# timweiland/DiffEqGMRFs.jl

Hardware: AMD Instinct MI355X
Metric: GMRF posterior solves/sec (mean+samples), 256^2 Darcy (higher is better)
Workload: dtype f64; 1 GPU; darcy256: n=65536, 64 blocks x 1024, nnz=1624084; 256 independent posterior(s) per GPU and step (4 stream(s) x batch 64), each factor + mean + 64 samples; mode=problems, samples_per_problem_per_rank=64, l_blocks_kept=False

## Files before the change

### diffeqgmrfs.jl_amd/_cabi.py

```python
from __future__ import annotations

import ctypes as C
import os
from typing import Optional

_HERE = os.path.dirname(os.path.abspath(__file__))
LIB_PATH = os.environ.get("GMRF_HIP_LIBRARY") or os.path.join(_HERE, "csrc", "libgmrf_hip.so")

GMRF_OK = 0
ERR_NOT_SPD, ERR_BAD_SHAPE, ERR_BAND, ERR_HIP, ERR_NO_FACTOR, ERR_NO_DEVICE, ERR_ALLOC, ERR_RCCL = -1, -2, -3, -4, -5, -6, -7, -8
SOLVE_FULL, SOLVE_FORWARD, SOLVE_BACKWARD = 0, 1, 2
VAR_EXACT, VAR_RBMC, VAR_MC = 0, 1, 2
BLOCK_L, BLOCK_C, BLOCK_LINV = 0, 1, 2
ORDER_REFERENCE, ORDER_TWISTED = 0, 1

EXPORTS = [
    "gmrf_bt_create", "gmrf_bt_destroy", "gmrf_last_error", "gmrf_version",
    "gmrf_bt_factor_csc", "gmrf_bt_factor_blocks", "gmrf_bt_refactor_values",
    "gmrf_bt_solve", "gmrf_bt_sample", "gmrf_bt_posterior", "gmrf_bt_normals", "gmrf_bt_marginal_var",
    "gmrf_bt_var_accumulate", "gmrf_bt_logdet", "gmrf_bt_get_block", "gmrf_bt_factor_buffer",
    "gmrf_bt_adopt_shape", "gmrf_bt_adopt_commit", "gmrf_bt_adopt_layout", "gmrf_bt_get_layout", "gmrf_bt_block_range",
    "gmrf_bt_set_keep_l", "gmrf_bt_storage_bytes", "gmrf_bt_set_storage", "gmrf_bt_factor_begin_csc",
    "gmrf_bt_factor_step_async", "gmrf_bt_factor_end", "gmrf_bt_stats",
    "gmrf_bt_set_profiling", "gmrf_bt_set_eager", "gmrf_bt_synchronize", "gmrf_bt_set_batch", "gmrf_bt_select_problem",
    "gmrf_bt_marginal_var_batch", "gmrf_bt_selinv", "gmrf_bt_trace_inv", "gmrf_bt_set_order", "gmrf_bt_get_order", "gmrf_bt_half_stats", "gmrf_bt_export_size", "gmrf_bt_export_factor", "gmrf_bt_import_factor",
    "gmrf_comm_unique_id", "gmrf_comm_create", "gmrf_comm_destroy", "gmrf_comm_bcast_host", "gmrf_comm_allreduce_sum",
    "gmrf_bt_bcast_blocks_async", "gmrf_bt_allgather_blocks_async", "gmrf_comm_wait", "gmrf_comm_bytes", "gmrf_streams_create", "gmrf_streams_destroy",
    "gmrf_bt_packed_size", "gmrf_bt_pack_blocks_async", "gmrf_bt_unpack_blocks_async",
    "gmrf_csr_create", "gmrf_csr_destroy", "gmrf_spmm", "gmrf_spmm_rows", "gmrf_spmm_async", "gmrf_spmm_rows_async",
    "gmrf_darcy_p1_create", "gmrf_darcy_p2_create", "gmrf_darcy_p1_destroy", "gmrf_darcy_p1_pattern", "gmrf_darcy_p1_assemble",
    "gmrf_burgers_p1_create", "gmrf_burgers_p2_create", "gmrf_burgers_p1_destroy", "gmrf_burgers_p1_pattern", "gmrf_burgers_p1_tangent",
    "gmrf_shallow_water_p1_create", "gmrf_shallow_water_p1_destroy", "gmrf_shallow_water_p1_pattern", "gmrf_shallow_water_p1_qpoints",
    "gmrf_shallow_water_p1_assemble", "gmrf_shallow_water_p1_operators",
    "gmrf_assemble_create", "gmrf_assemble_destroy", "gmrf_assemble_pattern", "gmrf_assemble_precision", "gmrf_assemble_rhs",
    "gmrf_test_gemm", "gmrf_test_gemm_rate", "gmrf_test_gemm_shapes", "gmrf_test_potrf_tile", "gmrf_test_potrf_block", "gmrf_test_tile_timing", "gmrf_test_persist_stamps", "gmrf_test_persist_aborts", "gmrf_test_persist_budget", "gmrf_test_clock_probe_start", "gmrf_test_clock_probe_finish",
    "gmrf_test_mfma_f64_rate", "gmrf_test_hbm_rate", "gmrf_test_microbench", "gmrf_test_symbolic_csc",
]


class SparseBlock(C.Structure):
    _fields_ = [("nnz", C.c_int64), ("ptr", C.c_void_p), ("idx", C.c_void_p), ("val", C.c_void_p)]


class Stats(C.Structure):
    _fields_ = [
        ("factor_ms", C.c_double), ("solve_ms", C.c_double), ("sample_ms", C.c_double),
        ("factor_flops", C.c_double), ("sweep_bytes", C.c_double), ("sweep_ms", C.c_double),
        ("n", C.c_int64), ("n_blocks", C.c_int64), ("block_size", C.c_int64),
        ("block_size_padded", C.c_int64), ("factor_bytes", C.c_int64),
        ("kernel_ms", C.c_double * 24), ("kernel_work", C.c_double * 24), ("kernel_launches", C.c_int64 * 24),
        ("sweep_bytes_streamed", C.c_double),
        ("persist_route", C.c_int32), ("persist_aborts", C.c_int32), ("persist_cus", C.c_int32), ("persist_refused", C.c_int32),
        ("sweep_persist", C.c_int32), ("sweep_persist_launches", C.c_int32),
    ]


class GmrfError(RuntimeError):
    def __init__(self, status: int, msg: str, info: int = 0):
        super().__init__(f"libgmrf_hip status {status}: {msg}")
        self.status = status
        self.info = info


class NotPositiveDefinite(GmrfError):
    """Julia's PosDefException(info): `.info` is the failing block (1-based)."""


_lib: Optional[C.CDLL] = None


def load() -> C.CDLL:
    global _lib
    if _lib is not None:
        return _lib
    if not os.path.exists(LIB_PATH):
        raise ImportError(
            f"{LIB_PATH} is missing: build it with `python -c 'import __graft_entry__ as g; g.build()'` "
            "or `make -C diffeqgmrfs.jl_amd/csrc` (the HIP library is the only compute path)")
    try:
        import torch
    except Exception:
        pass
    lib = C.CDLL(LIB_PATH)
    vp, i32, i64, u64, dbl = C.c_void_p, C.c_int32, C.c_int64, C.c_uint64, C.c_double
    P = C.POINTER
    sigs = {
        "gmrf_bt_create": [i32, vp, P(vp)],
        "gmrf_bt_destroy": [vp],
        "gmrf_version": [],
        "gmrf_bt_factor_csc": [vp, i64, i64, vp, vp, vp, i32, P(i32)],
        "gmrf_bt_factor_blocks": [vp, i64, i64, vp, vp, i32, i32, P(i32)],
        "gmrf_bt_refactor_values": [vp, vp, P(i32)],
        "gmrf_bt_solve": [vp, vp, vp, i64, i64, i64, i32],
        "gmrf_bt_sample": [vp, u64, i64, i64, vp, vp, vp, i64],
        "gmrf_bt_posterior": [vp, vp, u64, i64, i64, vp, vp, i64],
        "gmrf_bt_normals": [vp, u64, i64, i64, vp, i64],
        "gmrf_bt_marginal_var": [vp, i32, i64, u64, vp, vp],
        "gmrf_bt_var_accumulate": [vp, i32, i64, i64, u64, vp, vp],
        "gmrf_bt_logdet": [vp, P(dbl)],
        "gmrf_bt_get_block": [vp, i32, i64, vp, i64],
        "gmrf_bt_factor_buffer": [vp, i32, P(vp), P(i64)],
        "gmrf_bt_adopt_shape": [vp, i64, i64],
        "gmrf_bt_storage_bytes": [i64, i64, i64, P(i64), P(i64), P(i64)],
        "gmrf_bt_set_storage": [vp, i64, i64, i64, vp, vp, vp],
        "gmrf_bt_adopt_commit": [vp, i32],
        "gmrf_bt_adopt_layout": [vp, i64, i64, vp, i64],
        "gmrf_bt_get_layout": [vp, vp, i64, P(i64)],
        "gmrf_bt_block_range": [vp, i32, i64, i64, P(i64), P(i64), P(i64)],
        "gmrf_bt_set_keep_l": [vp, i32],
        "gmrf_comm_unique_id": [vp],
        "gmrf_comm_create": [i32, i32, i32, vp, P(vp)],
        "gmrf_comm_destroy": [vp],
        "gmrf_comm_bcast_host": [vp, vp, i64, i32],
        "gmrf_comm_allreduce_sum": [vp, vp, vp, i64],
        "gmrf_bt_bcast_blocks_async": [vp, vp, i32, i64, i64, i32],
        "gmrf_bt_allgather_blocks_async": [vp, vp, vp, i64, i64],
        "gmrf_comm_wait": [vp, vp],
        "gmrf_comm_bytes": [vp, i32, P(dbl)],
        "gmrf_bt_packed_size": [vp, i64, i64, P(i64)],
        "gmrf_bt_pack_blocks_async": [vp, i64, i64, vp],
        "gmrf_bt_unpack_blocks_async": [vp, i64, i64, vp],
        "gmrf_streams_create": [i32, i32, vp, vp],
        "gmrf_streams_destroy": [i32, i32, vp],
        "gmrf_bt_factor_begin_csc": [vp, i64, i64, vp, vp, vp, i32],
        "gmrf_bt_factor_step_async": [vp, i64, i64],
        "gmrf_bt_factor_end": [vp, P(i32)],
        "gmrf_bt_stats": [vp, P(Stats)],
        "gmrf_bt_set_order": [vp, i32, i64],
        "gmrf_bt_get_order": [vp, P(i32), P(i64)],
        "gmrf_bt_half_stats": [vp, i32, P(Stats)],
        "gmrf_bt_set_profiling": [vp, i32],
        "gmrf_bt_set_eager": [vp, i32],
        "gmrf_bt_synchronize": [vp],
        "gmrf_bt_set_batch": [vp, i64],
        "gmrf_bt_select_problem": [vp, i64],
        "gmrf_csr_create": [i32, vp, i64, i64, vp, vp, vp, i32, i32, P(vp)],
        "gmrf_bt_marginal_var_batch": [vp, i32, i64, u64, vp, vp, vp],
        "gmrf_bt_selinv": [vp, vp, vp],
        "gmrf_bt_trace_inv": [vp, vp, vp, i64, vp],
        "gmrf_bt_export_size": [vp, P(i64)],
        "gmrf_bt_export_factor": [vp, vp, i64],
        "gmrf_bt_import_factor": [vp, vp, i64],
        "gmrf_csr_destroy": [vp],
        "gmrf_assemble_create": [i32, vp, i64, vp, vp, i64, vp, vp, i32, P(vp)],
        "gmrf_assemble_destroy": [vp],
        "gmrf_assemble_pattern": [vp, P(i64), P(i64), vp, vp, i32],
        "gmrf_assemble_precision": [vp, vp, vp, dbl, vp],
        "gmrf_assemble_rhs": [vp, vp, vp, vp, vp, dbl, vp],
        "gmrf_darcy_p1_create": [i32, vp, i64, i64, P(vp)],
        "gmrf_darcy_p2_create": [i32, vp, i64, i64, P(vp)],
        "gmrf_darcy_p1_destroy": [vp],
        "gmrf_darcy_p1_pattern": [vp, P(i64), vp, vp, i32],
        "gmrf_darcy_p1_assemble": [vp, vp, i64, dbl, vp, vp],
        "gmrf_burgers_p1_create": [i32, vp, i64, i64, dbl, dbl, P(vp)],
        "gmrf_burgers_p2_create": [i32, vp, i64, i64, dbl, dbl, P(vp)],
        "gmrf_burgers_p1_destroy": [vp],
        "gmrf_burgers_p1_pattern": [vp, P(i64), vp, vp, i32],
        "gmrf_burgers_p1_tangent": [vp, vp, vp, vp],
        "gmrf_shallow_water_p1_create": [i32, vp, i64, i64, P(vp)],
        "gmrf_shallow_water_p1_destroy": [vp],
        "gmrf_shallow_water_p1_pattern": [vp, i32, P(i64), vp, vp, i32],
        "gmrf_shallow_water_p1_qpoints": [vp, vp],
        "gmrf_shallow_water_p1_assemble": [vp, vp, dbl, dbl, dbl, vp, vp, vp, vp],
        "gmrf_shallow_water_p1_operators": [vp, vp, vp, vp, vp, dbl, dbl, dbl, vp, vp, vp, vp],
        "gmrf_spmm": [vp, vp, vp, i64, i64, i64],
        "gmrf_spmm_async": [vp, vp, vp, i64, i64, i64],
        "gmrf_spmm_rows_async": [vp, vp, vp, i64, i64, i64],
        "gmrf_spmm_rows": [vp, vp, vp, i64, i64, i64],
        "gmrf_test_gemm": [i32, i64, i64, i64, i32, i32, i32, i32, dbl, vp, i64, vp, i64, dbl, vp, i64],
        "gmrf_test_gemm_shapes": [vp, P(dbl), i64, P(i64)],
        "gmrf_test_gemm_rate": [i32, i64, i64, i64, i32, i32, i32, i32, i32, i32, P(dbl)],
        "gmrf_test_potrf_tile": [i32, vp, vp, P(i32)],
        "gmrf_test_potrf_block": [i32, i64, vp, vp, P(i32)],
        "gmrf_test_tile_timing": [vp, i32],
        "gmrf_test_persist_stamps": [vp, i32],
        "gmrf_test_persist_aborts": [vp, vp],
        "gmrf_test_persist_budget": [i32, i32, vp, vp],
        "gmrf_test_clock_probe_start": [i32, i32, i32, P(vp)],
        "gmrf_test_clock_probe_finish": [vp, vp, vp],
        "gmrf_test_mfma_f64_rate": [i32, P(dbl)],
        "gmrf_test_hbm_rate": [i32, i64, P(dbl)],
        "gmrf_test_microbench": [i32, vp, i32],
        "gmrf_test_symbolic_csc": [i64, i64, vp, vp, i32, vp],
    }
    for name, args in sigs.items():
        fn = getattr(lib, name)
        fn.argtypes = args
        fn.restype = i32
    lib.gmrf_last_error.argtypes = []
    lib.gmrf_last_error.restype = C.c_char_p
    _lib = lib
    return lib


def check(status: int, info: int = 0):
    if status == GMRF_OK:
        return
    msg = load().gmrf_last_error().decode(errors="replace")
    if status == ERR_NOT_SPD:
        raise NotPositiveDefinite(status, msg, info)
    raise GmrfError(status, msg, info)


def ptr(a) -> C.c_void_p:
    if a is None:
        return C.c_void_p(0)
    if isinstance(a, int):
        return C.c_void_p(a)
    if hasattr(a, "data_ptr"):
        return C.c_void_p(a.data_ptr())
    return C.c_void_p(a.ctypes.data)
```

### diffeqgmrfs.jl_amd/api.py

```python
from __future__ import annotations

import ctypes as C
from typing import List, Optional, Sequence, Tuple

import numpy as np
import scipy.sparse as sp

from . import _cabi
from ._cabi import GmrfError, NotPositiveDefinite


def _is_torch(x) -> bool:
    return hasattr(x, "data_ptr") and hasattr(x, "device")


def _colmajor(b, n: int):
    if _is_torch(b):
        import torch
        if b.dtype != torch.float64:
            raise TypeError("float64 required")
        if b.dim() == 1:
            if b.shape[0] != n:
                raise ValueError("dimension mismatch")
            return b.contiguous(), 1, n, True
# ... 568 lines not shown
        return out

    def logdet(self) -> float:
        v = C.c_double(0.0)
        _cabi.check(self._lib.gmrf_bt_logdet(self._h, C.byref(v)))
        return v.value

    def normals(self, k: int, seed: int = 0x5EED, first_id: int = 0, like=None):
        if self.batch != 1:
            raise ValueError("a batched handle draws (batch, k, n) normals: normals_batch")
        store, view = _alloc_like(like if like is not None else np.empty(0), self.N, k, False)
        _cabi.check(self._lib.gmrf_bt_normals(self._h, seed, first_id, k, _cabi.ptr(store), self.N))
        return view

    def normals_batch(self, k: int, seed: int = 0x5EED, first_id: int = 0):
        out = np.empty((self.batch, k, self.N), dtype=np.float64)
        _cabi.check(self._lib.gmrf_bt_normals(self._h, seed, first_id, k, _cabi.ptr(out), self.N))
        return out

    def sample(self, k: int, mean=None, z=None, seed: int = 0x5EED, first_id: int = 0, like=None):
        ref = like if like is not None else (z if z is not None else (mean if mean is not None else np.empty(0)))
        za = None
        if z is not None:
            za, kz, _, _ = _colmajor(z, self.N)
            k = kz
        if mean is not None and not _is_torch(mean):
            mean = np.ascontiguousarray(mean, dtype=np.float64)
        store, view = _alloc_like(ref if _is_torch(ref) else np.empty(0), self.N, k, False)
        _cabi.check(self._lib.gmrf_bt_sample(self._h, seed, first_id, k, _cabi.ptr(mean), _cabi.ptr(za),
                                             _cabi.ptr(store), self.N))
        return view

    def posterior(self, b, k: int, seed: int = 0x5EED, first_id: int = 0):
        if self.batch != 1:
            raise ValueError("posterior(): one problem per handle (use solve_batch / sample_batch for batches)")
        xa, kb, ld, one_d = _colmajor(b, self.N)
        if kb != 1:
            raise ValueError("posterior(): one right-hand side")
        mstore, mview = _alloc_like(xa, self.N, 1, True)
        sstore, sview = _alloc_like(xa, self.N, k, False)
        _cabi.check(self._lib.gmrf_bt_posterior(self._h, _cabi.ptr(xa), seed, first_id, k, _cabi.ptr(mstore), _cabi.ptr(sstore),
                                                self.N))
        return mview, sview

    def posterior_batch(self, b, k: int, seed: int = 0x5EED, first_id: int = 0):
        import torch
        B, n = self.batch, self.N
        b = b.reshape(B, n).contiguous()
        mean = torch.empty((B, n), dtype=torch.float64, device=b.device)
        out = torch.empty((B, k, n), dtype=torch.float64, device=b.device)
        _cabi.check(self._lib.gmrf_bt_posterior(self._h, _cabi.ptr(b), seed, first_id, k, _cabi.ptr(mean), _cabi.ptr(out), n))
        return mean, out

    def marginal_var(self, method: str = "exact", k: int = 50, seed: int = 0x5EED, Q: Optional[CsrMatrix] = None,
                     q_values=None, out=None):
        m = {"exact": _cabi.VAR_EXACT, "rbmc": _cabi.VAR_RBMC, "mc": _cabi.VAR_MC}[method]
        shape = (self.N,) if self.batch == 1 else (self.batch, self.N)
        if out is None:
            out = np.empty(shape, dtype=np.float64)
        else:
            ok = tuple(out.shape) == shape and (out.is_contiguous() and str(out.dtype) == "torch.float64" if _is_torch(out)
                                                else out.flags.c_contiguous and out.dtype == np.float64)
            if not ok:
                raise ValueError(f"out must be a contiguous float64 array of shape {shape}")
        if self.batch > 1 and m != _cabi.VAR_EXACT:
            qv = None
            if q_values is not None:
                qv = q_values.contiguous() if _is_torch(q_values) else np.ascontiguousarray(q_values, dtype=np.float64)
            _cabi.check(self._lib.gmrf_bt_marginal_var_batch(self._h, m, k, seed, Q._h if Q is not None else None,
                                                             _cabi.ptr(qv) if qv is not None else None, _cabi.ptr(out)))
            return out
        _cabi.check(self._lib.gmrf_bt_marginal_var(self._h, m, k, seed, Q._h if Q is not None else None,
                                                   _cabi.ptr(out)))
        return out

    def selected_inverse(self, S: CsrMatrix, out=None):
        shape = (S.nnz,) if self.batch == 1 else (self.batch, S.nnz)
        given = out is not None
        out = self._out_array(out, shape)
        _cabi.check(self._lib.gmrf_bt_selinv(self._h, S._h, _cabi.ptr(out)))
        if given or self.batch > 1:
            return out
        return sp.csr_matrix((out, S.indices.copy(), S.indptr.copy()), shape=S.shape)

    def trace_inv(self, S: CsrMatrix, dvals):
        nd = 2 if self.batch == 1 else 3
        if dvals.ndim != nd or dvals.shape[-1] != S.nnz or (nd == 3 and dvals.shape[0] != self.batch):
            want = "(m, nnz)" if nd == 2 else "(batch, m, nnz)"
            raise ValueError(f"dvals must be {want} with nnz = {S.nnz}")
        m = int(dvals.shape[-2])
        if _is_torch(dvals):
            import torch
            if dvals.dtype != torch.float64:
                raise TypeError("float64 required")
            dvals = dvals.contiguous()
            out = torch.empty(dvals.shape[:-1], dtype=torch.float64, device=dvals.device)
        else:
            dvals = np.ascontiguousarray(dvals, dtype=np.float64)
            out = np.empty(dvals.shape[:-1], dtype=np.float64)
        _cabi.check(self._lib.gmrf_bt_trace_inv(self._h, S._h, _cabi.ptr(dvals), m, _cabi.ptr(out)))
        return out

    @staticmethod
    def _out_array(out, shape):
        if out is None:
            return np.empty(shape, dtype=np.float64)
# ... 261 lines not shown
```

### diffeqgmrfs.jl_amd/csrc/gemm_f64.hpp

```cpp
#pragma once
#include <hip/hip_runtime.h>
#include <hip/hip_ext.h>
#include <stdint.h>
#include <stdlib.h>
#include <algorithm>
#include <array>
#include <map>
#include <mutex>
#include <vector>

namespace gmrf {

typedef double v4d __attribute__((ext_vector_type(4)));
typedef double v2d __attribute__((ext_vector_type(2)));

enum : int {
    TRI_A_LOWER = 1,
    TRI_A_UPPER = 2,
    TRI_B_LOWER = 4,
    TRI_B_UPPER = 8
};

struct GemmArgs {
    const double* A;
    const double* B;
    double* C;
    int64_t lda, ldb, ldc;
    int64_t strideA, strideB, strideC;
    int64_t pA, pB, pC;
    int nb1;
    int M, N, K;
    int tri;
    int lower_only;
    double alpha, beta;
    const double* D;
    int64_t ldd, pD;
    unsigned long long* stamps;
    const int* kb_m = nullptr;
    const int* kb_n = nullptr;
    const int* ke_n = nullptr;
};

constexpr int GEMM_BM = 64;
constexpr int GEMM_BN = 64;

template <bool ROWS_CONTIG, int BK>
__device__ __forceinline__ void gemm_load_tile(const double* __restrict__ P, int64_t ld, int row0, int k0,
                                               int t, v2d (&rg)[BK / 8]) {
    if (!ROWS_CONTIG) {
        constexpr int TPR = BK / 2, RPP = 256 / TPR;
        const int r = t / TPR, kk = (t % TPR) * 2;
        const double* p = P + (int64_t)(row0 + r) * ld + k0 + kk;
#pragma unroll
        for (int i = 0; i < BK / 8; ++i) rg[i] = *reinterpret_cast<const v2d*>(p + (int64_t)(i * RPP) * ld);
    } else {
        const int kk = t >> 5, r = (t & 31) * 2;
        const double* p = P + (int64_t)(k0 + kk) * ld + row0 + r;
#pragma unroll
        for (int i = 0; i < BK / 8; ++i) rg[i] = *reinterpret_cast<const v2d*>(p + (int64_t)(i * 8) * ld);
    }
}

template <bool ROWS_CONTIG, int BK>
__device__ __forceinline__ void gemm_tile_offsets(int64_t ld, int row0, int t, uint32_t (&off)[BK / 8]) {
    if (!ROWS_CONTIG) {
        constexpr int TPR = BK / 2, RPP = 256 / TPR;
        const int r = t / TPR, kk = (t % TPR) * 2;
#pragma unroll
        for (int i = 0; i < BK / 8; ++i) off[i] = (uint32_t)(((int64_t)(row0 + r + i * RPP) * ld + kk) * 8);
    } else {
        const int kk = t >> 5, r = (t & 31) * 2;
#pragma unroll
        for (int i = 0; i < BK / 8; ++i) off[i] = (uint32_t)(((int64_t)(kk + i * 8) * ld + row0 + r) * 8);
    }
}
template <bool ROWS_CONTIG>
__device__ __forceinline__ const char* gemm_tile_base(const double* P, int64_t ld, int k0) {
    return reinterpret_cast<const char*>(ROWS_CONTIG ? P + (int64_t)k0 * ld : P + k0);
}
template <int BK>
__device__ __forceinline__ void gemm_load_tile_off(const char* base, uint32_t (&off)[BK / 8], v2d (&rg)[BK / 8]) {
#pragma unroll
    for (int i = 0; i < BK / 8; ++i) {
        asm volatile("" : "+v"(off[i]));
        rg[i] = *reinterpret_cast<const v2d*>(base + off[i]);
    }
}

template <int BK>
__device__ __forceinline__ void gemm_store_tile_natural(double* sm, int t, const v2d (&rg)[BK / 8]) {
    const int kk = t >> 5, r = (t & 31) * 2;
#pragma unroll
    for (int i = 0; i < BK / 8; ++i) *reinterpret_cast<v2d*>(sm + (kk + 8 * i) * 64 + r) = rg[i];
// ... 624 lines not shown
```

### diffeqgmrfs.jl_amd/csrc/gemm_f64_dma.hpp

```cpp
#pragma once
#include "gemm_f64.hpp"

namespace gmrf {

constexpr int DMA_BK = 16;
constexpr int DMA_ROWS_ASCENDING = 1024;
#ifndef GMRF_DMA_READS_FIRST
#define GMRF_DMA_READS_FIRST 0
#endif

template <int BM, int BN>
constexpr size_t gemm_dma_lds_bytes(int stages) { return (size_t)stages * (BM + BN) * DMA_BK * sizeof(double); }

#define GMRF_LDS_PTR(p) ((__attribute__((address_space(3))) void*)(p))
#define GMRF_GLB_PTR(p) ((const __attribute__((address_space(1))) void*)(p))

template <int BM, int BN>
__device__ __forceinline__ void gemm_dma_tile_order(const GemmArgs& g, int& bm, int& bn, int& z) {
    const int nx = g.N / BN, ny = g.M / BM;
    int tpp;
    if (g.lower_only == 1) {
        if (BM >= BN) tpp = (BM / BN) * ny * (ny + 1) / 2;
        else tpp = 0;
    } else tpp = nx * ny;
    const int nz = (int)gridDim.x / tpp;
    const int groups = (nz % 8 == 0) ? 8 : 1;
    const int xg = (int)blockIdx.x % groups, q = (int)blockIdx.x / groups, nzg = nz / groups;
    int zq;
    if (g.lower_only == 1) {
        constexpr int R = BM / BN > 0 ? BM / BN : 1;
        const int tile = q % tpp;
        zq = q / tpp;
        const int tr = (g.tri & DMA_ROWS_ASCENDING) ? tile : tpp - 1 - tile;
        int b = (int)((sqrtf(8.0f * (float)(tr / R) + 1.0f) - 1.0f) * 0.5f);
        while (R * b * (b + 1) / 2 > tr) --b;
        while (R * (b + 1) * (b + 2) / 2 <= tr) ++b;
        bm = b;
        bn = tr - R * b * (b + 1) / 2;
    } else {
        const bool cls_n = (g.tri & (TRI_B_LOWER | TRI_B_UPPER)) || !(g.tri & (TRI_A_LOWER | TRI_A_UPPER));
        const bool desc = cls_n ? ((g.tri & TRI_B_UPPER) != 0 || (g.ke_n && !g.kb_n)) : (g.tri & TRI_A_LOWER) != 0;
        const int ncls = cls_n ? nx : ny, other = cls_n ? ny : nx;
        int c = q / (other * nzg);
        const int rem = q % (other * nzg);
        const int o = rem % other;
        zq = rem / other;
        if (desc) c = ncls - 1 - c;
        bn = cls_n ? c : o;
        bm = cls_n ? o : c;
    }
    z = xg + groups * zq;
}

template <int BM, int BN, bool B_N, int STAGES, bool A_T = false, bool TAIL = false>
__global__ __launch_bounds__(256, (BM + BN > 128) ? 3 : 4) void gemm_f64_dma(GemmArgs g) {
    constexpr int BK = DMA_BK;
    constexpr int MI = BM / 32, NJ = BN / 32;
    constexpr int NA = BM / 32, NB = BN / 32;
    constexpr int A_ST = BM * BK, B_ST = BN * BK, T_ST = TAIL ? BK : 0, ST = A_ST + B_ST + T_ST;
    static_assert(NJ % 2 == 0 || !B_N, "the [k][n] image pairs neighbouring column tiles");
    static_assert(MI % 2 == 0 || !A_T, "the [k][m] image pairs neighbouring row tiles");
    static_assert(!TAIL || (BM == 64 && BN == 64 && B_N && !A_T), "the tail row: 64 x 64 tiles, B stored [k][n]");
    int bm, bn, z;
    gemm_dma_tile_order<BM, BN>(g, bm, bn, z);
    const bool tail = TAIL && bm == g.M / BM - 1;
    const int m0 = bm * BM, n0 = bn * BN;
    if (g.lower_only == 2 && n0 > m0 + BM - 1) return;
    const int zi = z % g.nb1, zp = z / g.nb1;
    const double* __restrict__ A = g.A + (int64_t)zi * g.strideA + (int64_t)zp * g.pA;
    const double* __restrict__ B = g.B + (int64_t)zi * g.strideB + (int64_t)zp * g.pB;
    double* C = g.C + (int64_t)zi * g.strideC + (int64_t)zp * g.pC;
    const double* Dm = g.D ? g.D + (int64_t)zp * g.pD : C;
    const int64_t ldd = g.D ? g.ldd : g.ldc;

    int kb = 0, ke = g.K;
    if (g.tri & TRI_A_LOWER) ke = min(ke, m0 + BM);
    if (g.tri & TRI_A_UPPER) kb = max(kb, m0);
    if (g.tri & TRI_B_LOWER) kb = max(kb, n0);
    if (g.tri & TRI_B_UPPER) ke = min(ke, n0 + BN);
    if (g.kb_m) kb = max(kb, g.kb_m[bm * (BM / 64)]);
    if (g.kb_n) kb = max(kb, g.kb_n[bn * (BN / 64)]);
    if (g.ke_n) ke = min(ke, g.ke_n[bn * (BN / 64) + BN / 64 - 1]);
    const int nkt = (ke > kb) ? (ke - kb) / BK : 0;

    extern __shared__ __attribute__((aligned(16))) double gsm[];
    const int t = threadIdx.x;
    const int lane = t & 63, w = __builtin_amdgcn_readfirstlane(t >> 6);
    const int wm = (w >> 1) * (BM / 2), wn = (w & 1) * (BN / 2);
    const int li = lane & 15, lq = lane >> 4;
    const bool idle = g.lower_only != 0 && ((n0 + wn) / 64 > (m0 + wm + BM / 2 - 1) / 64);

    uint32_t offa[NA], offb[NB];
#pragma unroll
    for (int i = 0; i < NA; ++i) {
        const int q = w + 4 * i;
        if (A_T) {
            constexpr int LPR = BM / 2;
            const int k = q * (64 / LPR) + lane / LPR, col = (lane % LPR) * 2;
            offa[i] = (uint32_t)(((int64_t)k * g.lda + m0 + col) * 8);
        } else {
            const int row = 8 * q + (lane >> 3), ch = (lane & 7) ^ ((row >> 1) & 7);
            offa[i] = (uint32_t)(((int64_t)(m0 + row) * g.lda + 2 * ch) * 8);
        }
    }
#pragma unroll
    for (int i = 0; i < NB; ++i) {
        const int q = w + 4 * i;
        if (B_N) {
            constexpr int LPR = BN / 2;
            const int k = q * (64 / LPR) + lane / LPR, col = (lane % LPR) * 2;
            offb[i] = (uint32_t)(((int64_t)k * g.ldb + n0 + col) * 8);
        } else {
            const int row = 8 * q + (lane >> 3), ch = (lane & 7) ^ ((row >> 1) & 7);
            offb[i] = (uint32_t)(((int64_t)(n0 + row) * g.ldb + 2 * ch) * 8);
        }
    }
    const double* arow = A + (int64_t)g.M * g.lda;
    auto issue = [&](int kt, int stage) {
        const int k0 = kb + kt * BK;
        const char* abase = reinterpret_cast<const char*>(A_T ? A + (int64_t)k0 * g.lda : A + k0);
        const char* bbase = reinterpret_cast<const char*>(B_N ? B + (int64_t)k0 * g.ldb : B + k0);
        double* as = gsm + stage * ST;
        double* bs = as + A_ST;
        if constexpr (TAIL)
            if (tail && w == 0 && lane < 8)
                __builtin_amdgcn_global_load_lds(GMRF_GLB_PTR(arow + k0 + 2 * lane), GMRF_LDS_PTR(bs + B_ST), 16, 0, 0);
#pragma unroll
        for (int i = 0; i < NA; ++i) {
            asm volatile("" : "+v"(offa[i]));
            __builtin_amdgcn_global_load_lds(GMRF_GLB_PTR(abase + offa[i]), GMRF_LDS_PTR(as + (w + 4 * i) * 128), 16, 0, 0);
        }
#pragma unroll
        for (int i = 0; i < NB; ++i) {
            asm volatile("" : "+v"(offb[i]));
            __builtin_amdgcn_global_load_lds(GMRF_GLB_PTR(bbase + offb[i]), GMRF_LDS_PTR(bs + (w + 4 * i) * 128), 16, 0, 0);
        }
    };

    v4d acc[MI][NJ];
#pragma unroll
    for (int i = 0; i < MI; ++i)
#pragma unroll
        for (int j = 0; j < NJ; ++j) acc[i][j] = (v4d){0.0, 0.0, 0.0, 0.0};
    v2d tacc = (v2d){0.0, 0.0};
    const int tkg = w >> 1;

    int fa[MI], fb[NJ];
#pragma unroll
    for (int i = 0; i < MI; ++i) {
        const int row = wm + 16 * i + li;
        fa[i] = A_T ? (2 * lq + (i & 1)) * BM + wm + 32 * (i >> 1) + 2 * li : row * 16 + 2 * (lq ^ ((row >> 1) & 3));
    }
    int sa2[MI], sb2[NJ];
#pragma unroll
    for (int i = 0; i < MI; ++i) { const int row = wm + 16 * i + li; sa2[i] = (!A_T && ((row >> 1) & 4)) ? 8 : 0; }
    if (!B_N) {
#pragma unroll
        for (int j = 0; j < NJ; ++j) {
            const int row = wn + 16 * j + li;
            fb[j] = A_ST + row * 16 + 2 * (lq ^ ((row >> 1) & 3));
            sb2[j] = ((row >> 1) & 4) ? 8 : 0;
        }
    } else {
#pragma unroll
        for (int j = 0; j < NJ; ++j) { fb[j] = A_ST + (2 * lq + (j & 1)) * BN + wn + 32 * (j >> 1) + 2 * li; sb2[j] = 0; }
    }

    constexpr int DEPTH = STAGES - 1;
#pragma unroll
    for (int s = 0; s < DEPTH; ++s)
        if (s < nkt) issue(s, s);
    for (int kt = 0; kt < nkt; ++kt) {
        const int ahead = min(DEPTH - 1, nkt - 1 - kt);
        if (ahead <= 0) asm volatile("s_waitcnt vmcnt(0)" ::: "memory");
        else if (ahead == 1) asm volatile("s_waitcnt vmcnt(%0)" ::"n"(NA + NB) : "memory");
        else asm volatile("s_waitcnt vmcnt(%0)" ::"n"(2 * (NA + NB)) : "memory");
        __builtin_amdgcn_s_barrier();
        __builtin_amdgcn_sched_barrier(0);
        if (!GMRF_DMA_READS_FIRST && kt + DEPTH < nkt) issue(kt + DEPTH, (kt + DEPTH) % STAGES);
        if (!idle) {
            const double* sm = gsm + (kt % STAGES) * ST;
            v2d a[BK / 8][MI], b[BK / 8][NJ];
#pragma unroll
            for (int kg = 0; kg < BK / 8; ++kg) {
#pragma unroll
                for (int i = 0; i < MI; ++i) a[kg][i] = *reinterpret_cast<const v2d*>(sm + fa[i] + (A_T ? kg * 8 * BM : ((kg * 8) ^ sa2[i])));
#pragma unroll
                for (int j = 0; j < NJ; ++j)
                    b[kg][j] = *reinterpret_cast<const v2d*>(sm + fb[j] + (B_N ? kg * 8 * BN : ((kg * 8) ^ sb2[j])));
            }
            v2d ta = (v2d){0.0, 0.0};
            if constexpr (TAIL)
                if (tail) ta = *reinterpret_cast<const v2d*>(sm + A_ST + B_ST + tkg * 8 + 2 * lq);
            __builtin_amdgcn_sched_barrier(0);
            if (GMRF_DMA_READS_FIRST && kt + DEPTH < nkt) issue(kt + DEPTH, (kt + DEPTH) % STAGES);
            __builtin_amdgcn_sched_barrier(0);
#pragma unroll
            for (int kg = 0; kg < BK / 8; ++kg)
#pragma unroll
                for (int p = 0; p < 2; ++p)
#pragma unroll
                    for (int i = 0; i < MI; ++i)
#pragma unroll
                        for (int j = 0; j < NJ; ++j) {
                            double av;
                            if (A_T) av = (i & 1) ? a[kg][2 * (i >> 1) + p].y : a[kg][2 * (i >> 1) + p].x;
                            else av = p ? a[kg][i].y : a[kg][i].x;
                            double bv;
                            if (B_N) bv = (j & 1) ? b[kg][2 * (j >> 1) + p].y : b[kg][2 * (j >> 1) + p].x;
                            else bv = p ? b[kg][j].y : b[kg][j].x;
                            acc[i][j] = __builtin_amdgcn_mfma_f64_16x16x4f64(av, bv, acc[i][j], 0, 0, 0);
                        }
            if constexpr (TAIL) {
                if (tail) {
                    const v2d b0 = tkg ? b[1][0] : b[0][0], b1 = tkg ? b[1][1] : b[0][1];
                    tacc.x = fma(ta.x, b0.x, tacc.x); tacc.x = fma(ta.y, b1.x, tacc.x);
                    tacc.y = fma(ta.x, b0.y, tacc.y); tacc.y = fma(ta.y, b1.y, tacc.y);
                }
            }
            __builtin_amdgcn_sched_barrier(0);
        } else if (GMRF_DMA_READS_FIRST && kt + DEPTH < nkt) issue(kt + DEPTH, (kt + DEPTH) % STAGES);
    }
    if (idle) return;

    const double alpha = g.alpha, beta = g.beta;
    auto orow = [&](int i, int r) -> int64_t {
        return A_T ? m0 + wm + 32 * (i >> 1) + 2 * (lq + 4 * r) + (i & 1) : m0 + wm + i * 16 + lq + 4 * r;
    };
    if (B_N) {
        v2d d[MI][4][NJ / 2 > 0 ? NJ / 2 : 1];
        if (beta != 0.0) {
#pragma unroll
            for (int i = 0; i < MI; ++i)
#pragma unroll
                for (int r = 0; r < 4; ++r)
#pragma unroll
                    for (int jp = 0; jp < NJ / 2; ++jp)
                        d[i][r][jp] = *reinterpret_cast<const v2d*>(Dm + orow(i, r) * ldd + n0 + wn + jp * 32 + 2 * li);
        }
#pragma unroll
        for (int i = 0; i < MI; ++i)
#pragma unroll
            for (int r = 0; r < 4; ++r)
#pragma unroll
                for (int jp = 0; jp < NJ / 2; ++jp) {
                    v2d v = (v2d){alpha * acc[i][2 * jp][r], alpha * acc[i][2 * jp + 1][r]};
                    if (beta != 0.0) { v.x += beta * d[i][r][jp].x; v.y += beta * d[i][r][jp].y; }
                    *reinterpret_cast<v2d*>(C + orow(i, r) * g.ldc + n0 + wn + jp * 32 + 2 * li) = v;
                }
    } else {
        double d[MI][4][NJ];
        if (beta != 0.0) {
#pragma unroll
            for (int i = 0; i < MI; ++i)
#pragma unroll
                for (int r = 0; r < 4; ++r)
#pragma unroll
                    for (int j = 0; j < NJ; ++j)
                        d[i][r][j] = Dm[orow(i, r) * ldd + n0 + wn + j * 16 + li];
        }
#pragma unroll
        for (int i = 0; i < MI; ++i)
#pragma unroll
            for (int r = 0; r < 4; ++r)
#pragma unroll
                for (int j = 0; j < NJ; ++j) {
                    double v = alpha * acc[i][j][r];
                    if (beta != 0.0) v += beta * d[i][r][j];
                    C[orow(i, r) * g.ldc + n0 + wn + j * 16 + li] = v;
                }
    }
    if constexpr (TAIL) {
        if (tail) {
            __syncthreads();
            *reinterpret_cast<v2d*>(gsm + (tkg * 4 + lq) * BN + wn + 2 * li) = tacc;
            __syncthreads();
            if (w == 0) {
                double s = 0.0;
#pragma unroll
                for (int q = 0; q < 8; ++q) s += gsm[q * BN + lane];
                double v = alpha * s;
                if (beta != 0.0) v += beta * Dm[(int64_t)g.M * ldd + n0 + lane];
                C[(int64_t)g.M * g.ldc + n0 + lane] = v;
            }
        }
    }
}

inline int& gemm_dma_policy() {
    static int v = [] { const char* e = getenv("GMRF_GEMM_DMA"); return e ? atoi(e) : 2; }();
    return v;
}
inline int& gemm_dma_force() {
    static int v = 0;
    return v;
}
inline int gemm_dma_stages() {
    static const int v = [] { const char* e = getenv("GMRF_GEMM_DMA_STAGES"); const int s = e ? atoi(e) : 2; return s == 3 ? 3 : 2; }();
    return v;
}

inline int gemm_dma_shape(bool a_t, const GemmArgs& g, int batch) {
    const int policy = gemm_dma_force() ? 2 : gemm_dma_policy();
    if (policy == 0 || g.stamps || (g.tri & ~15) || g.K % DMA_BK || g.M % 64 || g.N % 64) return 0;
    if ((g.lda & 1) || (g.ldb & 1) || ((uintptr_t)g.A & 15) || ((uintptr_t)g.B & 15) || ((g.strideA | g.strideB | g.pA | g.pB) & 1)) return 0;
    if (((uintptr_t)g.C & 15) || (g.ldc & 1) || ((g.strideC | g.pC) & 1)) return 0;
    if (g.D && (((uintptr_t)g.D & 15) || (g.ldd & 1) || (g.pD & 1))) return 0;
    if ((int64_t)g.M * g.ldc * 8 >= ((int64_t)1 << 32) || (g.D && (int64_t)g.M * g.ldd * 8 >= ((int64_t)1 << 32))) return 0;
    if ((int64_t)(a_t ? g.K : g.M) * g.lda * 8 >= ((int64_t)1 << 32) || (int64_t)std::max(g.N, g.K) * g.ldb * 8 >= ((int64_t)1 << 32)) return 0;
    if (a_t) return 1;
    const int force = gemm_dma_force();
    if (force == 2 && g.M % 128 == 0) return 2;
    if (force == 3 && g.N % 128 == 0 && !g.lower_only) return 3;
    if (force) return 1;
    if (policy == 1) return 1;
    const bool plain = !g.lower_only && !g.tri && !g.kb_m && !g.kb_n && !g.ke_n;
    const int64_t t64 = (int64_t)(g.M / 64) * (g.N / 64) * batch;
    if (policy >= 3 || (plain && t64 >= 2048)) {
        if (g.M % 128 == 0) return 2;
        if (g.N % 128 == 0 && !g.lower_only) return 3;
    }
    return 1;
}
inline bool gemm_uses_dma(bool a_t, const GemmArgs& g, int batch) { return gemm_dma_shape(a_t, g, batch) != 0; }

inline hipError_t gemm_dma_init() {
    hipError_t e = hipSuccess;
#define GMRF_DMA_ATTR(BM, BN, BNAT, ST)                                                                          \
    if (e == hipSuccess)                                                                                          \
        e = hipFuncSetAttribute((const void*)gemm_f64_dma<BM, BN, BNAT, ST>, hipFuncAttributeMaxDynamicSharedMemorySize, \
                                (int)gemm_dma_lds_bytes<BM, BN>(ST) + 64 * 1024);
    GMRF_DMA_ATTR(64, 64, false, 2) GMRF_DMA_ATTR(64, 64, true, 2) GMRF_DMA_ATTR(64, 64, false, 3) GMRF_DMA_ATTR(64, 64, true, 3)
    GMRF_DMA_ATTR(128, 64, false, 2) GMRF_DMA_ATTR(128, 64, true, 2) GMRF_DMA_ATTR(128, 64, false, 3) GMRF_DMA_ATTR(128, 64, true, 3)
    GMRF_DMA_ATTR(64, 128, false, 2) GMRF_DMA_ATTR(64, 128, true, 2) GMRF_DMA_ATTR(64, 128, false, 3) GMRF_DMA_ATTR(64, 128, true, 3)
#undef GMRF_DMA_ATTR
    return e;
}

inline bool gemm_tail_ok(bool a_t, bool b_n, const GemmArgs& g, int batch) {
    if (a_t || !b_n || g.lower_only || gemm_uses_ll(g, batch) || gemm_dma_shape(false, g, batch) != 1) return false;
    return (int64_t)(g.M + 1) * g.ldc * 8 < ((int64_t)1 << 32) && (!g.D || (int64_t)(g.M + 1) * g.ldd * 8 < ((int64_t)1 << 32));
}
inline bool gemm_try_dma_tail(hipStream_t st, bool a_t, bool b_n, const GemmArgs& g, int batch, hipEvent_t ev_start, hipEvent_t ev_stop,
                              hipError_t* err) {
    if (!gemm_tail_ok(a_t, b_n, g, batch)) return false;
    GemmArgs gs = g;
    gs.lower_only = 0;
    const dim3 grid((unsigned)((int64_t)(g.N / 64) * (g.M / 64) * batch)), block(256);
    const size_t lds = (size_t)gemm_dma_stages() * (64 + 64 + DMA_BK) * DMA_BK * sizeof(double);
    if (gemm_dma_stages() == 3) {
        if (ev_start) hipExtLaunchKernelGGL((gemm_f64_dma<64, 64, true, 3, false, true>), grid, block, lds, st, ev_start, ev_stop, 0, gs);
        else hipLaunchKernelGGL((gemm_f64_dma<64, 64, true, 3, false, true>), grid, block, lds, st, gs);
    } else {
        if (ev_start) hipExtLaunchKernelGGL((gemm_f64_dma<64, 64, true, 2, false, true>), grid, block, lds, st, ev_start, ev_stop, 0, gs);
        else hipLaunchKernelGGL((gemm_f64_dma<64, 64, true, 2, false, true>), grid, block, lds, st, gs);
    }
    *err = hipGetLastError();
    return true;
}

inline bool gemm_try_dma(hipStream_t st, bool a_t, bool b_n, const GemmArgs& g, int batch, hipEvent_t ev_start, hipEvent_t ev_stop,
                         hipError_t* err) {
    const int shape = gemm_dma_shape(a_t, g, batch);
    if (shape == 0) return false;
    const bool tri_grid = g.lower_only && g.M == g.N;
    GemmArgs gs = g;
    gs.lower_only = tri_grid ? 1 : (g.lower_only ? 2 : 0);
    static const bool asc_off = [] { const char* e = getenv("GMRF_GEMM_G2_ORDER"); return e && atoi(e) == 0; }();
    if (tri_grid && (g.kb_m || g.kb_n) && !asc_off) gs.tri |= DMA_ROWS_ASCENDING;
    const int stages = gemm_dma_stages();
    const dim3 block(256);
#define GMRF_DMA_GO(BM, BN)                                                                                       \
    do {                                                                                                          \
        const int64_t nx = g.N / BN, ny = g.M / BM;                                                               \
        const int64_t tiles = tri_grid ? (int64_t)(BM / BN > 0 ? BM / BN : 1) * ny * (ny + 1) / 2 : nx * ny;      \
        const dim3 grid((unsigned)(tiles * batch));                                                               \
        static const size_t lds_pad = [] { const char* e = getenv("GMRF_GEMM_DMA_LDS_PAD_KB"); return (size_t)(e ? atoi(e) : 0) * 1024; }();    \
        const size_t lds = gemm_dma_lds_bytes<BM, BN>(stages) + lds_pad;                                          \
        if (a_t && BM == 64 && BN == 64) {                                                                        \
            if (b_n) GMRF_DMA_K((gemm_f64_dma<64, 64, true, 2, true>)); else GMRF_DMA_K((gemm_f64_dma<64, 64, false, 2, true>)); \
        } else if (stages == 3) {                                                                                 \
            if (b_n) GMRF_DMA_K((gemm_f64_dma<BM, BN, true, 3>)); else GMRF_DMA_K((gemm_f64_dma<BM, BN, false, 3>)); \
        } else {                                                                                                  \
            if (b_n) GMRF_DMA_K((gemm_f64_dma<BM, BN, true, 2>)); else GMRF_DMA_K((gemm_f64_dma<BM, BN, false, 2>)); \
        }                                                                                                         \
    } while (0)
#define GMRF_DMA_K(KERNEL)                                                                                        \
    do {                                                                                                          \
        if (ev_start) hipExtLaunchKernelGGL(KERNEL, grid, block, lds, st, ev_start, ev_stop, 0, gs);              \
        else hipLaunchKernelGGL(KERNEL, grid, block, lds, st, gs);                                                \
    } while (0)
    if (shape == 2) GMRF_DMA_GO(128, 64);
    else if (shape == 3) GMRF_DMA_GO(64, 128);
    else GMRF_DMA_GO(64, 64);
#undef GMRF_DMA_K
#undef GMRF_DMA_GO
    *err = hipGetLastError();
    return true;
}

}
```

### diffeqgmrfs.jl_amd/csrc/gmrf_hip.hip

```cpp
#include <hip/hip_runtime.h>
#include <dlfcn.h>
#include <stdint.h>
#include <stdlib.h>
#include <string.h>
#include <time.h>

#include <algorithm>
#include <atomic>
#include <iterator>
#include <cmath>
#include <map>
#include <memory>
#include <chrono>
#include <functional>
#include <initializer_list>
#include <mutex>
#include <string>
#include <type_traits>
#include <vector>

#include "../../include/gmrf_hip.h"
#include "assemble.hpp"
#include "fem_assemble.hpp"
#include "gemm_f64.hpp"
// ... 122 lines not shown
    int* d_mend = nullptr;
    int* d_kbx = nullptr;
    int kst_cap = 0;
    double c_streamed = 0.0;
    double g2_tile_k = 0.0;
    bool c_dirty = false;
    int* d_lo_rowptr = nullptr;
    int* d_dg_rowptr = nullptr;
    int* d_bxt_uptr = nullptr; int* d_bxt_ucols = nullptr; uint16_t* d_bxt_lidx = nullptr; int* d_bxt_gtiles = nullptr;
    std::vector<int> bxt_ng;
    int bxt_ecap = 0; int bxt_nrt = 0; bool bxt_plan_ok = false;
    int64_t lo_row_max = 0;
    bool sparse_b = false;
    bool dense_g1 = false;
    double *d_L = nullptr, *d_C = nullptr, *d_Linv = nullptr;
    bool external_storage = false;
    bool keep_l = true;
    bool l_valid = false;
    bool logdet_valid = false;
    std::vector<char> got_block;
    int64_t alloc_rm = 0, alloc_wc = 0;
    bool alloc_keep_l = true;
    double *d_S = nullptr, *d_B = nullptr, *d_T = nullptr, *d_W = nullptr;
    double* d_V = nullptr;
    int64_t v_elems = 0;
    uint64_t layout_gen = 0;
    uint64_t sel_csr = 0, sel_gen = ~0ull;
    int64_t sel_nnz = 0;
    std::vector<int64_t> sel_off, sel_nd;
    int64_t* d_sel_src = nullptr;
    int64_t* d_sel_slot = nullptr;
    int64_t sel_cap = 0;
    double* d_sig = nullptr;
    int64_t sig_elems = 0;
    double* d_dv = nullptr;
    int64_t dv_elems = 0;
    int* d_info = nullptr;
    double* d_logdet = nullptr;
    int64_t alloc_N = 0, alloc_bsp = 0;
    bool factored = false;
    double *d_P = nullptr, *d_Y = nullptr, *d_Tp = nullptr;
    int64_t kp_cap = 0;
    double* d_stage = nullptr;
    int64_t stage_cap = 0;
    double* d_mean = nullptr;
    double* d_acc = nullptr;
    int64_t acc_B = 0;
    bool eager = false;
    bool split_step = false;
    bool sweep_no_gemm = false;
    bool no_fused_posterior = false;
    bool tail_probe = false;
    bool tail_refused = false;
    unsigned long long* dbg_stamps = nullptr;
    bool fork_graph = false;
    bool no_staircase = false;
    bool doubling_x = false;
    int xsplit = 0;
    int adopt_xsplit = 0;
    bool no_xsplit = false;
    bool no_lookahead = false;
    bool no_persist = false;
    bool persist_gave_up = false;
    bool persist_launched = false;
    int persist_cus = 0;
    int info_checked = 0;
    int factor_graph_route = 0;
    int persist_aborts = 0;
    int cu_count = 0;
    unsigned* d_pflags = nullptr;
    int64_t pflags_words = 0;
    bool no_sweep_persist = false;
    bool no_scatter_fold = false;
    bool sweep_persist_planned = false;
    bool sweep_persist_launched = false;
    unsigned* d_sweep_flags = nullptr;
    double* d_Tsw = nullptr;
    int64_t t_elems = 0;
    unsigned* h_sweep_abort = nullptr;
    int sweep_nw = 0;
    double *d_P2 = nullptr, *d_Y2 = nullptr, *d_T2 = nullptr;
    int64_t p2_elems = 0;
    bool sweep_persist_hold = false;
    bool no_persist_panels = false;
    hipStream_t aux = nullptr;
    bool aux_distinct = false;
    hipStream_t gemm_stream = nullptr;
    bool capturing = false;
    std::vector<hipEvent_t> fork_events;
    size_t fork_next = 0;
    hipGraphExec_t factor_graph = nullptr;
    int64_t factor_graph_i0 = -1, factor_graph_i1 = -1;
    std::map<int64_t, hipGraphExec_t> sweep_graphs;
    int profiling = 0;
    std::vector<EvPair> events;
    std::vector<hipEvent_t> ev_pool;
    std::vector<GemmShapeStat> gemm_shapes;
    gmrf_stats stats;
    hipEvent_t ev0 = nullptr, ev1 = nullptr;
    int order = GMRF_ORDER_REFERENCE;
    int64_t meet_req = -1;
    int32_t eager_bits = 0;
    TwistState* tw = nullptr;
    int64_t tw_blk = -1;
    const double* tw_hj = nullptr;
    double* tw_w = nullptr;
// ... 25 lines not shown
    if (!h || h->order != GMRF_ORDER_TWISTED) return GMRF_OK;
    g_last_error = std::string(what) + ": not supported on a handle in the twisted elimination order (gmrf_bt_set_order)";
    return GMRF_ERR_BAD_SHAPE;
}

static void destroy_graphs(gmrf_handle* h) {
    if (h->factor_graph) { (void)hipGraphExecDestroy(h->factor_graph); h->factor_graph = nullptr; }
    for (auto& kv : h->sweep_graphs) (void)hipGraphExecDestroy(kv.second);
    h->sweep_graphs.clear();
}

static hipEvent_t ev_get(gmrf_handle* h) {
    if (!h->ev_pool.empty()) {
        hipEvent_t e = h->ev_pool.back();
        h->ev_pool.pop_back();
        return e;
    }
    hipEvent_t e;
    (void)hipEventCreate(&e);
    return e;
}

struct ProfScope {
    gmrf_handle* h;
    EvPair p;
    bool on;
    ProfScope(gmrf_handle* hh, int kind, double work) : h(hh), on(hh->profiling > 0) {
        if (on) {
            p.kind = kind; p.work = work;
            p.a = ev_get(h); p.b = ev_get(h);
            (void)hipEventRecord(p.a, h->stream);
        }
    }
    ~ProfScope() {
        if (on) {
            (void)hipEventRecord(p.b, h->stream);
            h->events.push_back(p);
        }
    }
};

static void prof_collect(gmrf_handle* h) {
    for (auto& p : h->events) {
        float ms = 0.f;
        (void)hipEventElapsedTime(&ms, p.a, p.b);
        h->stats.kernel_ms[p.kind] += ms; h->stats.kernel_work[p.kind] += p.work; h->stats.kernel_launches[p.kind]++;
        if (p.shape >= 0) { auto& g = h->gemm_shapes[(size_t)p.shape]; g.launches += 1; g.ms += ms; g.work += p.work; }
        h->ev_pool.push_back(p.a);
        h->ev_pool.push_back(p.b);
    }
    h->events.clear();
}

static gmrf_status gemm(gmrf_handle* h, bool a_t, bool b_n, int M, int N, int K, int tri, int lower_only,
                        double alpha, const double* A, int64_t lda, const double* B, int64_t ldb,
                        double beta, double* C, int64_t ldc, int64_t pA, int64_t pB, int64_t pC,
                        int batch = 1, int64_t sA = 0, int64_t sB = 0, int64_t sC = 0, const double* D = nullptr,
                        int64_t ldd = 0, int64_t pD = 0, int pclass = 0, double pwork = -1.0,
                        const int* kb_m = nullptr, const int* kb_n = nullptr, const int* ke_n = nullptr, bool tail = false) {
    GemmArgs g;
    g.kb_m = kb_m; g.kb_n = kb_n; g.ke_n = ke_n;
    g.D = D; g.ldd = ldd; g.pD = pD;
    g.A = A; g.B = B; g.C = C;
    g.lda = lda; g.ldb = ldb; g.ldc = ldc;
    g.strideA = sA; g.strideB = sB; g.strideC = sC;
    g.pA = pA; g.pB = pB; g.pC = pC; g.nb1 = batch;
    g.M = M; g.N = N; g.K = K; g.tri = tri; g.lower_only = lower_only;
    g.alpha = alpha; g.beta = beta; g.stamps = nullptr;
    double flops = 2.0 * M * N * (double)K * batch * (double)h->B;
    if (lower_only) flops *= 0.5 * (1.0 + 64.0 / std::max(M, 64));
    if (tri) flops *= 0.5 * (1.0 + 64.0 / std::max(K, 64));
    if (tail) {
        if (!gemm_tail_ok(a_t, b_n, g, batch * (int)h->B)) {
            h->tail_refused = true;
            return h->tail_probe ? GMRF_OK : bad_shape("internal: a product of the fused sweep does not qualify for the tail-row GEMM");
        }
        if (h->tail_probe) return GMRF_OK;
        flops *= (M + 1.0) / M;
        if (pwork >= 0.0) pwork *= (M + 1.0) / M;
        pclass = b_n ? 15 : 14;
        hipError_t e = hipSuccess;
        if (h->profiling > 0) {
            EvPair p;
            p.kind = pclass; p.work = pwork >= 0.0 ? pwork : flops;
            p.a = ev_get(h); p.b = ev_get(h);
            const int64_t key[8] = {pclass, M + 1, N, K, tri, lower_only, batch * h->B, (kb_m || kb_n || ke_n) ? 1 : 0};
            for (size_t i = 0; i < h->gemm_shapes.size() && p.shape < 0; ++i)
                if (!memcmp(h->gemm_shapes[i].key, key, sizeof(key))) p.shape = (int)i;
            if (p.shape < 0) {
                GemmShapeStat st; memcpy(st.key, key, sizeof(key));
                h->gemm_shapes.push_back(st); p.shape = (int)h->gemm_shapes.size() - 1;
            }
            (void)gemm_try_dma_tail(h->gemm_stream ? h->gemm_stream : h->stream, a_t, b_n, g, batch * (int)h->B, p.a, p.b, &e);
            HIPCHK(e);
            h->events.push_back(p);
            return GMRF_OK;
        }
        (void)gemm_try_dma_tail(h->gemm_stream ? h->gemm_stream : h->stream, a_t, b_n, g, batch * (int)h->B, nullptr, nullptr, &e);
        HIPCHK(e);
        return GMRF_OK;
    }
    if (gemm_uses_big(a_t, g, batch * (int)h->B)) { pclass = b_n ? 7 : 6; pwork = -1.0; }
    else if (pclass == 0) {
        if (gemm_uses_ll(g, batch * (int)h->B)) pclass = 13;
        else if (gemm_uses_dma(a_t, g, batch * (int)h->B)) pclass = a_t ? 18 : (b_n ? 15 : 14);
        else pclass = a_t ? 12 : (b_n ? 11 : 0);
    }
    if (h->profiling > 0) {
        EvPair p;
        p.kind = pclass; p.work = pwork >= 0.0 ? pwork : flops;
        p.a = ev_get(h); p.b = ev_get(h);
        const int64_t key[8] = {pclass, M, N, K, tri, lower_only, batch * h->B, (kb_m || kb_n || ke_n) ? 1 : 0};
        for (size_t i = 0; i < h->gemm_shapes.size() && p.shape < 0; ++i)
            if (!memcmp(h->gemm_shapes[i].key, key, sizeof(key))) p.shape = (int)i;
        if (p.shape < 0) {
            GemmShapeStat st; memcpy(st.key, key, sizeof(key));
            h->gemm_shapes.push_back(st); p.shape = (int)h->gemm_shapes.size() - 1;
        }
        HIPCHK(launch_gemm(h->gemm_stream ? h->gemm_stream : h->stream, a_t, b_n, g, batch * (int)h->B, p.a, p.b));
        h->events.push_back(p);
        return GMRF_OK;
    }
    HIPCHK(launch_gemm(h->gemm_stream ? h->gemm_stream : h->stream, a_t, b_n, g, batch * (int)h->B));
    return GMRF_OK;
}

static void free_dev(void* p) {
    if (p) (void)hipFree(p);
// ... 74 lines not shown
        }
        h->alloc_rm = h->rmax; h->alloc_wc = c_ld(h);
        h->l_valid = false;
        return GMRF_OK;
    }
    free_dev(h->d_L); free_dev(h->d_C); free_dev(h->d_Linv);
    free_dev(h->d_S); free_dev(h->d_B); free_dev(h->d_T); free_dev(h->d_W);
    free_dev(h->d_logdet);
    h->d_L = h->d_C = h->d_Linv = h->d_S = h->d_B = h->d_T = h->d_W = h->d_logdet = nullptr;
    h->l_valid = false;
    const size_t blk = (size_t)blk_elems(h) * sizeof(double) * (size_t)h->B;
    HIPCHK(hipMalloc(&h->d_L, blk * (h->keep_l ? h->N : 1)));
    HIPCHK(hipMalloc(&h->d_Linv, blk * h->N));
    HIPCHK(hipMalloc(&h->d_C, (size_t)stride_pC(h) * sizeof(double) * (size_t)h->B));
    HIPCHK(hipMemsetAsync(h->d_L, 0, blk * (h->keep_l ? h->N : 1), h->stream));
    HIPCHK(hipMemsetAsync(h->d_Linv, 0, blk * h->N, h->stream));
    HIPCHK(hipMemsetAsync(h->d_C, 0, (size_t)stride_pC(h) * sizeof(double) * (size_t)h->B, h->stream));
    h->c_dirty = false;
    GCHK(alloc_work(h));
    h->alloc_rm = h->rmax; h->alloc_wc = c_ld(h); h->alloc_keep_l = h->keep_l;
    return GMRF_OK;
}

static gmrf_status alloc_work(gmrf_handle* h) {
    const size_t blk = (size_t)blk_elems(h) * sizeof(double) * (size_t)h->B;
    HIPCHK(hipMalloc(&h->d_S, blk));
    HIPCHK(hipMalloc(&h->d_B, blk));
    HIPCHK(hipMalloc(&h->d_T, blk));
    HIPCHK(hipMalloc(&h->d_W, blk));
    HIPCHK(hipMalloc(&h->d_logdet, sizeof(double) * h->N * h->B));
    {
        const int64_t words = (int64_t)persist_flag_words((int)(h->bsp / 64)) * h->B;
        if (!h->d_pflags || h->pflags_words < words) {
            free_dev(h->d_pflags); h->d_pflags = nullptr; h->pflags_words = 0;
            HIPCHK(hipMalloc(&h->d_pflags, sizeof(unsigned) * (size_t)words));
            HIPCHK(hipMemsetAsync(h->d_pflags, 0, sizeof(unsigned) * (size_t)words, h->stream));
            HIPCHK(hipStreamSynchronize(h->stream));
            h->pflags_words = words;
        }
    }
    h->alloc_N = h->N; h->alloc_bsp = h->bsp; h->alloc_B = h->B;
    h->stats.factor_bytes = (int64_t)(blk * ((h->keep_l ? 2 : 1) * h->N) + (size_t)stride_pC(h) * sizeof(double) * (size_t)h->B);
    return GMRF_OK;
}

static void release_shape_buffers(gmrf_handle* h) {
    for (auto& kv : h->sweep_graphs) (void)hipGraphExecDestroy(kv.second);
    h->sweep_graphs.clear();
    free_dev(h->d_P); free_dev(h->d_Y); free_dev(h->d_Tp);
    h->d_P = h->d_Y = h->d_Tp = nullptr; h->kp_cap = 0;
    free_dev(h->d_mean); h->d_mean = nullptr;
    free_dev(h->d_acc); h->d_acc = nullptr; h->acc_B = 0;
    free_dev(h->d_stage); h->d_stage = nullptr; h->stage_cap = 0;
}

static gmrf_status set_shape(gmrf_handle* h, int64_t n, int64_t N) {
    if (n <= 0 || N <= 0 || n % N != 0) return bad_shape("n must be a positive multiple of N_blocks");
    const int64_t bs = n / N;
    if (bs > (1 << 20)) return bad_shape("block size too large");
    if (h->n != n || h->N != N) {
        (void)hipStreamSynchronize(h->stream);
        destroy_graphs(h);
        release_shape_buffers(h);
        h->factored = false;
        h->analyzed = false;
    }
    h->n = n; h->N = N; h->bs = bs;
    h->layout_gen++;
    h->bsp = 64 * next_pow2((bs + 63) / 64);
    h->n_pad = h->bsp * N;
    h->stats.n = n; h->stats.n_blocks = N; h->stats.block_size = bs; h->stats.block_size_padded = h->bsp;
    h->stats.factor_flops = ((double)N * bs * bs * bs / 3.0 + (double)(N - 1) * 2.0 * bs * bs * bs) * (double)h->B;
    return GMRF_OK;
}

static gmrf_status ensure_panels(gmrf_handle* h, int64_t kp) {
    if (kp <= h->kp_cap && h->d_P) return GMRF_OK;
    for (auto& kv : h->sweep_graphs) (void)hipGraphExecDestroy(kv.second);
    h->sweep_graphs.clear();
    free_dev(h->d_P); free_dev(h->d_Y); free_dev(h->d_Tp);
    h->d_P = h->d_Y = h->d_Tp = nullptr;
    HIPCHK(hipMalloc(&h->d_P, sizeof(double) * kp * h->n_pad * h->B));
    HIPCHK(hipMalloc(&h->d_Y, sizeof(double) * kp * h->n_pad * h->B));
    HIPCHK(hipMalloc(&h->d_Tp, sizeof(double) * kp * h->bsp * h->B));
    h->kp_cap = kp;
    return GMRF_OK;
}

static gmrf_status ensure_stage(gmrf_handle* h, int64_t elems) {
    if (elems <= h->stage_cap && h->d_stage) return GMRF_OK;
    free_dev(h->d_stage);
    h->d_stage = nullptr;
    HIPCHK(hipMalloc(&h->d_stage, sizeof(double) * elems));
    h->stage_cap = elems;
    return GMRF_OK;
}

struct HostEntry { uint64_t key; int64_t src; };

struct SymbolicPlan {
    std::vector<int64_t> diag_first, diag_count, low_first, low_count;
    std::vector<uint64_t> keys;
    std::vector<int64_t> src;
    int64_t cmin = 0, rmax = 0;
    std::vector<int64_t> first;
    std::vector<int> rowptr;
// ... 364 lines not shown
        }
    }
    h->sweep_persist_planned = ok && want_s > 0 && want >= want_s;
    const int got = ok ? want : 0;
    if (got != h->persist_cus) destroy_graphs(h);
    h->persist_cus = got;
    h->stats.persist_cus = got;
    h->stats.persist_refused = (want > 0 && !ok) ? 1 : 0;
}
static void persist_release(gmrf_handle* h) {
    std::lock_guard<std::mutex> lock(g_persist_mu);
    auto it = g_persist_claims.find(h->device);
    if (it != g_persist_claims.end()) it->second.erase(h);
    h->persist_cus = 0;
    h->stats.persist_cus = 0;
    h->sweep_persist_planned = false;
}

static void persist_give_up(gmrf_handle* h) {
    h->persist_gave_up = true; h->persist_aborts++;
    h->stats.persist_aborts = h->persist_aborts;
    persist_release(h);
    destroy_graphs(h);
}

static bool persist_fits(const gmrf_handle* h, int nt, int j0, int j1, int xrows) {
    if (h->no_persist || h->persist_gave_up || h->persist_cus <= 0) return false;
    return (int64_t)(1 + persist_tiles(nt, j0, j1, xrows)) * h->B <= h->persist_cus;
}

static gmrf_status launch_persist(gmrf_handle* h, double* S, double* L, double* X, int nt, int j0, int j1, int xrows, int blk_id,
                                  double flops) {
    const int words = persist_flag_words(nt);
    if (!h->d_pflags || h->pflags_words < (int64_t)words * h->B) return bad_shape("internal: flag words of the persistent launches not allocated");
    PersistArgs pa;
    pa.S = S; pa.L = L; pa.X = X; pa.ld = h->bsp; pa.nt = nt; pa.j0 = j0; pa.j1 = j1; pa.xrows = xrows;
    pa.tail_panel = (!xrows && j1 < nt) ? 1 : 0;
    pa.info = h->d_info; pa.blk = blk_id;
    pa.pS = h->bsp * h->bsp; pa.pL = stride_pL(h); pa.pX = stride_pX(h); pa.blk_per_problem = (int)h->N;
    pa.flags = h->d_pflags; pa.flag_stride = words;
    pa.abort_word = reinterpret_cast<unsigned*>(h->d_info + 1);
    static const int limit_ms = [] { const char* e = getenv("GMRF_PERSIST_SPIN_MS"); return e ? atoi(e) : -1; }();
    pa.spin_limit = (unsigned)(limit_ms >= 0 ? limit_ms : (h->B > 1 ? 200 : 2000)) * 100000u;
    pa.stamps = h->dbg_stamps;
    h->persist_launched = true;
    h->stats.persist_route = xrows == 1 ? 1 : (xrows == 0 ? 2 : 3);
    ProfScope ps(h, 17, flops);
    hipLaunchKernelGGL(potrf_persist<false>, dim3(1 + persist_tiles(nt, j0, j1, xrows), (unsigned)h->B), dim3(POTRF_PERSIST_THREADS), POTRF_PERSIST_LDS,
                       h->stream, pa);
    HIPCHK(hipGetLastError());
    return GMRF_OK;
}

static gmrf_status potrf_block(gmrf_handle* h, double* S, double* L, double* X, double* T, int blk_id) {
    const int bsp = (int)h->bsp;
    const int64_t ld = bsp;
    const int nt = bsp / 64;
    const int route = potrf_route(h);
    const bool fused = route == ROUTE_FUSED;
    if (h->xsplit > 0 && route != ROUTE_PANELS256) return bad_shape("internal: split inverse planned off the 256-column panel route");
    static const int pw_env = [] { const char* e = getenv("GMRF_PANEL_TILES"); return e ? atoi(e) : 4; }();
    const int pw = (!fused && nt >= 8) ? ((pw_env == 2 || pw_env == 8) ? pw_env : 4) : nt;
    const bool fused_in_panel = route == ROUTE_BIG_ONE;
    const bool overlap = h->capturing && h->fork_graph && nt >= 8;
    if (overlap && !h->aux) HIPCHK(hipStreamCreateWithFlags(&h->aux, hipStreamNonBlocking));
    hipEvent_t ev_fork = nullptr, ev_join = nullptr;
    if (overlap) { GCHK(fork_event(h, &ev_fork)); GCHK(fork_event(h, &ev_join)); }
    if (fused && !h->no_lookahead && !h->doubling_x && !overlap && nt >= 2 && persist_fits(h, nt, 0, nt, 1)) {
        const double t3 = 64.0 * 64.0 * 64.0;
        double fl = t3 / 3.0 * nt;
        for (int j = 0; j + 1 < nt; ++j) {
            const int m = nt - j - 1;
            fl += (double)m * t3 + 2.0 * t3 * (m * (m + 1) / 2) + 2.0 * t3 * (0.5 * (double)(j + 1) * (j + 2) + 0.625 * (j + 1));
        }
        return launch_persist(h, S, L, X, nt, 0, nt, 1, blk_id, fl);
    }
    if (fused && !h->no_lookahead && !h->doubling_x && !overlap && nt >= 2) {
        StepArgs sa;
        sa.S = S; sa.L = L; sa.X = X; sa.ld = ld; sa.nt = nt; sa.cend = nt;
        sa.info = h->d_info; sa.blk = blk_id; sa.dbg = nullptr;
        sa.pS = (int64_t)bsp * bsp; sa.pL = stride_pL(h); sa.pX = stride_pX(h); sa.blk_per_problem = (int)h->N;
        const double t3 = 64.0 * 64.0 * 64.0;
        {
            sa.j = 0; sa.lookahead = 0; sa.xrow = -1;
            ProfScope ps(h, 1, t3 / 3.0);
            hipLaunchKernelGGL(potrf_step<false>, dim3(1, 1), dim3(256), POTRF_TILE_LDS, h->stream, sa);
        }
        for (int j = 0; j + 1 < nt; ++j) {
            const int m = nt - j - 1, ntile_wg = m * (m + 1) / 2;
            sa.j = j; sa.lookahead = 1;
            sa.xrow = (j >= 1) ? j : -1; sa.xrow_first = ntile_wg;
            const int nx_wg = (j >= 1) ? 4 * j : 0;
            const double f_x = (j >= 1) ? 2.0 * t3 * (0.5 * (double)j * (j + 1) + 0.625 * j) : 0.0;
            ProfScope ps(h, 1, t3 / 3.0 + (double)m * t3 + 2.0 * t3 * ntile_wg + f_x);
            hipLaunchKernelGGL(potrf_step<false>, dim3(ntile_wg + nx_wg, 1), dim3(256), POTRF_STEP_LDS, h->stream, sa);
        }
        {
            sa.j = nt - 1; sa.lookahead = 0; sa.xrow = nt - 1; sa.xrow_first = 0;
            ProfScope ps(h, 1, 2.0 * t3 * (0.5 * (double)(nt - 1) * nt + 0.625 * (nt - 1)));
            hipLaunchKernelGGL(potrf_step<false>, dim3(4 * (nt - 1), 1), dim3(256), 64 * 18 * sizeof(double), h->stream, sa);
        }
        HIPCHK(hipGetLastError());
        return GMRF_OK;
    }
    if (route == ROUTE_PANELS256 && !overlap) {
        StepArgs sa;
        sa.S = S; sa.L = L; sa.X = X; sa.ld = ld; sa.nt = nt; sa.cend = nt;
        sa.info = h->d_info; sa.blk = blk_id; sa.dbg = nullptr;
        sa.pS = (int64_t)bsp * bsp; sa.pL = stride_pL(h); sa.pX = stride_pX(h); sa.blk_per_problem = (int)h->N;
        const int64_t pW = (int64_t)bsp * bsp;
        const double t3 = 64.0 * 64.0 * 64.0, nb = (double)h->B;
        auto diag128 = [&](int j) -> gmrf_status {
            sa.j = j;
            ProfScope ps(h, 16, (2.0 * t3 / 3.0 + 4.0 * 2.0 * t3 * 0.625) * nb);
            static const size_t lds_pad = [] { const char* e = getenv("GMRF_DIAG128_LDS_PAD_KB"); return (size_t)(e ? atoi(e) : 0) * 1024; }();
            static const bool fat = [] { const char* e = getenv("GMRF_DIAG128_FAT"); return e && atoi(e) != 0; }();
            if (fat) hipLaunchKernelGGL(potrf_diag128, dim3(1, (unsigned)h->B), dim3(256), POTRF_DIAG128_LDS + lds_pad, h->stream, sa);
            else hipLaunchKernelGGL(potrf_diag128_slim, dim3(1, (unsigned)h->B), dim3(256), POTRF_DIAG128_SLIM_LDS + lds_pad, h->stream, sa);
            HIPCHK(hipGetLastError());
            return GMRF_OK;
        };
        static const bool no_small = [] { const char* e = getenv("GMRF_PERSIST_PANELS"); return e && atoi(e) == 0; }();
        const bool persist_panels = !no_small && !h->no_persist_panels && persist_fits(h, 4, 0, 4, 2);
        for (int j = 0; j < nt; j += 4) {
            const int64_t oa = (int64_t)j * 64, ob = oa + 128, oc = oa + 256;
            if (persist_panels) {
                const double fl = (4.0 * t3 / 3.0 + 2.0 * t3 * (6.0 * 0.625 + 10.0 + 10.0 + 6.0 * 0.625)) * nb;
                GCHK(launch_persist(h, S + oa * ld + oa, L + oa * ld + oa, X + oa * ld + oa, 4, 0, 4, 2, blk_id, fl));
            } else {
                GCHK(diag128(j));
                GCHK(gemm(h, false, false, 128, 128, 128, TRI_B_UPPER, 0, 1.0, S + ob * ld + oa, ld, X + oa * ld + oa, ld, 0.0, L + ob * ld + oa, ld,
                          sa.pS, sa.pX, sa.pL, 1, 0, 0, 0, nullptr, 0, 0, 0, 2.0 * t3 * 3.0 * 2.0 * nb));
                GCHK(gemm(h, false, false, 128, 128, 128, 0, 1, -1.0, L + ob * ld + oa, ld, L + ob * ld + oa, ld, 1.0, S + ob * ld + ob, ld,
                          sa.pL, sa.pL, sa.pS, 1, 0, 0, 0, nullptr, 0, 0, 0, 2.0 * t3 * 2.0 * 3.0 * nb));
                GCHK(diag128(j + 2));
                GCHK(gemm(h, false, true, 128, 128, 128, TRI_B_LOWER, 0, 1.0, L + ob * ld + oa, ld, X + oa * ld + oa, ld, 0.0, T + ob * ld + oa, ld,
                          sa.pL, sa.pX, pW));
                GCHK(gemm(h, false, true, 128, 128, 128, TRI_A_LOWER, 0, -1.0, X + ob * ld + ob, ld, T + ob * ld + oa, ld, 0.0, X + ob * ld + oa, ld,
                          sa.pX, pW, sa.pX));
            }
            const int m3 = nt - j - 4;
            if (m3 <= 0) continue;
            const bool in_slot = (j == 0 && h->xsplit == 256 && !h->keep_l);
            double* Lb = in_slot ? X + oc * ld + oa : L + oc * ld + oa;
            const int64_t pLb = in_slot ? sa.pX : sa.pL;
            GCHK(gemm(h, false, false, 64 * m3, 256, 256, TRI_B_UPPER, 0, 1.0, S + oc * ld + oa, ld, X + oa * ld + oa, ld, 0.0, Lb, ld,
                      sa.pS, sa.pX, pLb, 1, 0, 0, 0, nullptr, 0, 0, 0, 2.0 * t3 * 10.0 * m3 * nb));
            GCHK(gemm(h, false, false, m3 * 64, m3 * 64, 256, 0, 1, -1.0, Lb, ld, Lb, ld, 1.0, S + oc * ld + oc, ld, pLb, pLb, sa.pS,
                      1, 0, 0, 0, nullptr, 0, 0, 0, 2.0 * t3 * 4.0 * (m3 * (m3 + 1) / 2) * nb));
        }
        const int p = h->xsplit;
        GCHK(doubling_levels(h, L, X, T, 256, bsp / 2, -1, p));
        if (p > 0 && !(p == 256 && !h->keep_l)) {
            hipLaunchKernelGGL(copy_rect, dim3((unsigned)((bsp - p) / 4), (unsigned)h->B), dim3(256), 0, h->stream,
                               L + (int64_t)p * ld, ld, sa.pL, X + (int64_t)p * ld, ld, sa.pX, bsp - p, p);
            HIPCHK(hipGetLastError());
        }
        return GMRF_OK;
    }
    if (h->xsplit > 0) return bad_shape("internal: split inverse planned off the 256-column panel route");
    for (int j = 0; j < nt; ++j) {
        StepArgs sa;
        sa.S = S; sa.L = L; sa.X = X; sa.ld = ld; sa.j = j; sa.nt = nt;
        sa.info = h->d_info; sa.blk = blk_id; sa.dbg = h->dbg_stamps;
        sa.pS = (int64_t)bsp * bsp; sa.pL = stride_pL(h); sa.pX = stride_pX(h); sa.blk_per_problem = (int)h->N;
        const int m = nt - j - 1;
        const int cend = std::min(nt, (j / pw + 1) * pw);
        sa.cend = cend;
        int utiles = 0;
        for (int c = j + 1; c < cend; ++c) utiles += nt - c;
        const double rem = 64.0 * m, nb = (double)h->B;
        const double f_tile = 64.0 * 64.0 * 64.0 / 3.0 * nb, f_panel = rem * 64.0 * 64.0 * nb;
        const double f_upd = 2.0 * 64.0 * 64.0 * 64.0 * utiles * nb;
        if (fused_in_panel && !h->no_lookahead && !overlap && j % pw == 0 && cend - j >= 2 && persist_fits(h, nt, j, cend, 0)) {
            const int npc = cend - j;
            double fl = 64.0 * 64.0 * 64.0 / 3.0 * npc;
            for (int jj = j; jj + 1 < cend; ++jj) {
                int ut = 0;
                for (int c = jj + 1; c < cend; ++c) ut += nt - c;
                fl += 64.0 * (nt - jj - 1) * 64.0 * 64.0 + 2.0 * 64.0 * 64.0 * 64.0 * ut;
            }
            fl += 64.0 * (nt - cend) * 64.0 * 64.0;
            GCHK(launch_persist(h, S, L, X, nt, j, cend, 0, blk_id, fl));
            j = cend - 1;
            sa.j = j;
        } else if (fused || m == 0) {
            const bool xrows = fused && !h->doubling_x && !overlap && j >= 2;
            const int ntile_wg = 1 + m * (m + 1) / 2;
            sa.xrow = xrows ? j - 1 : -1; sa.xrow_first = ntile_wg;
            const int nx_wg = xrows ? 4 * (j - 1) : 0;
            const double f_x = xrows ? 2.0 * 64.0 * 64.0 * 64.0 * (0.5 * (double)(j - 1) * j + 0.625 * (j - 1)) : 0.0;
            ProfScope ps(h, 1, f_tile + f_panel + f_upd + f_x);
            hipLaunchKernelGGL(potrf_step<false>, dim3(ntile_wg + nx_wg, (unsigned)h->B), dim3(256),
                               m == 0 ? POTRF_TILE_LDS : POTRF_STEP_LDS, h->stream, sa);
            sa.xrow = -1;
        } else if (fused_in_panel && utiles > 0) {
            ProfScope ps(h, 1, f_tile + f_panel + f_upd);
            hipLaunchKernelGGL(potrf_step<false>, dim3(1 + utiles, 1), dim3(256), POTRF_STEP_LDS, h->stream, sa);
        } else {
            {
                ProfScope ps(h, 1, f_tile);
                hipLaunchKernelGGL(potrf_step<false>, dim3(1, (unsigned)h->B), dim3(256), POTRF_TILE_LDS, h->stream, sa);
// ... 12 lines not shown
            const int j0 = cend - pw, mr = nt - cend;
            const double* Lp = L + (int64_t)cend * 64 * ld + (int64_t)j0 * 64;
            double* Sr = S + (int64_t)cend * 64 * ld + (int64_t)cend * 64;
            GCHK(gemm(h, false, false, mr * 64, mr * 64, pw * 64, 0, 1, -1.0, Lp, ld, Lp, ld, 1.0, Sr, ld, sa.pL, sa.pL,
                      sa.pS, 1, 0, 0, 0, nullptr, 0, 0, 0, 2.0 * 64.0 * 64.0 * (pw * 64.0) * (mr * (mr + 1) / 2) * (double)h->B));
        }
        if (overlap && j + 1 == nt / 2) {
            HIPCHK(hipEventRecord(ev_fork, h->stream));
            HIPCHK(hipStreamWaitEvent(h->aux, ev_fork, 0));
            h->gemm_stream = h->aux;
            gmrf_status st = doubling_levels(h, L, X, T, 64, bsp / 4, 0);
            if (st == GMRF_OK) st = doubling_top(h, L, X, T, true, false);
            h->gemm_stream = nullptr;
            GCHK(st);
        }
    }
    if (fused && !h->doubling_x && !overlap) {
        if (nt >= 2) {
            StepArgs sa;
            sa.S = S; sa.L = L; sa.X = X; sa.ld = ld; sa.j = nt - 1; sa.nt = nt;
            sa.info = h->d_info; sa.blk = blk_id; sa.dbg = nullptr;
            sa.pS = (int64_t)bsp * bsp; sa.pL = stride_pL(h); sa.pX = stride_pX(h); sa.blk_per_problem = (int)h->N;
            sa.cend = nt; sa.xrow = nt - 1; sa.xrow_first = 0;
            ProfScope ps(h, 1, 2.0 * 64.0 * 64.0 * 64.0 * (0.5 * (double)(nt - 1) * nt + 0.625 * (nt - 1)));
            hipLaunchKernelGGL(potrf_step<false>, dim3(4 * (nt - 1), 1), dim3(256), 64 * 18 * sizeof(double), h->stream, sa);
            HIPCHK(hipGetLastError());
        }
        return GMRF_OK;
    }
    if (overlap) {
        GCHK(doubling_levels(h, L, X, T, 64, bsp / 4, 1));
        HIPCHK(hipEventRecord(ev_join, h->aux));
        HIPCHK(hipStreamWaitEvent(h->stream, ev_join, 0));
        GCHK(doubling_top(h, L, X, T, false, true));
    } else {
        GCHK(doubling_levels(h, L, X, T, 64, bsp / 2, -1));
    }
    return GMRF_OK;
}

static gmrf_status factor_blocks_range(gmrf_handle* h, int64_t i0, int64_t i1) {
    const int bsp = (int)h->bsp;
    h->xsplit = planned_xsplit(h);
    const int64_t ld = bsp;
    const size_t blk_bytes = (size_t)bsp * bsp * sizeof(double) * (size_t)h->B;
    const int64_t bstride = (int64_t)bsp * bsp;
    const int64_t pX = stride_pX(h), pC = stride_pC(h);
    const int64_t ldc = c_ld(h), cstride = c_blk(h);
    const unsigned nb = (unsigned)h->B;
    for (int64_t i = i0; i < i1; ++i) {
        double* L = l_block(h, i);
        double* X = h->d_Linv + i * bstride;
        const int rm_s = (i > 0) ? (int)h->rmax : 0;
        static const bool no_tiles_z = [] { const char* e = getenv("GMRF_BXT_TILES"); return e && atoi(e) == 0; }();
        const bool scatter_in_bxt = i > 0 && nb == 1 && h->sparse_b && !h->dense_g1 && h->bxt_plan_ok && !no_tiles_z && h->bxt_nrt == (int)h->rmax / 64
                                    && h->d_dg_rowptr && h->bsp == h->bs && !h->no_scatter_fold;
        const bool zero_in_bxt = scatter_in_bxt || (i > 0 && h->sparse_b && !h->dense_g1 && h->bxt_plan_ok && !no_tiles_z && h->bxt_nrt == (int)h->rmax / 64
                                                    && ((int64_t)(bsp - rm_s) * bsp) % 2 == 0);
        if (rm_s < bsp && !zero_in_bxt) {
            const int64_t cnt = (int64_t)(bsp - rm_s) * bsp;
            hipLaunchKernelGGL(zero_rows, dim3((unsigned)((cnt / 2 + 255) / 256), nb), dim3(256), 0, h->stream,
                               h->d_S + (int64_t)rm_s * ld, cnt, bstride);
            HIPCHK(hipGetLastError());
        }
        if (i > 0) {
            double* C = h->d_C + (i - 1) * cstride;
            const double* Xp = h->d_Linv + (i - 1) * bstride;
            const bool sparse_g1 = h->sparse_b && !h->dense_g1;
            if (!sparse_g1) {
                HIPCHK(hipMemsetAsync(h->d_B, 0, blk_bytes, h->stream));
                if (h->low_count[i] > 0) {
                    hipLaunchKernelGGL(scatter_block, dim3((unsigned)((h->low_count[i] + 255) / 256), nb), dim3(256), 0,
                                       h->stream, h->d_keys, h->d_vals, h->low_first[i], h->low_count[i], h->d_B, ld,
                                       h->n_entries, bstride, 0);
                    HIPCHK(hipGetLastError());
                }
            }
            const int cm = (int)h->cmin, rm = (int)h->rmax;
            const int W = bsp - cm;
            if (sparse_g1) {
                BxtArgs ba;
                ba.rowptr = h->d_lo_rowptr + i * (h->bsp + 1); ba.keys = h->d_keys;
                ba.vals = h->d_vals; ba.n_entries = h->n_entries;
                ba.X = Xp; ba.C = C; ba.ld = ld; ba.ldc = ldc; ba.pX = pX; ba.pC = pC; ba.cm = cm; ba.rm = rm;
                ba.kst = h->d_kst;
                const int rch = (rm + 255) / 256;
                ba.cw = ((int64_t)(W / 64) * rch * nb >= 512) ? 64 : (((int64_t)(W / 32) * rch * nb >= 512) ? 32 : 16);
                ba.bsp = bsp;
                const dim3 grid((unsigned)((W / ba.cw) * rch * (int)nb));
                ProfScope ps(h, 10, 8.0 * (h->c_streamed + 0.5 * (double)W * W) * (double)h->B);
                static const bool no_tiles = [] { const char* e = getenv("GMRF_BXT_TILES"); return e && atoi(e) == 0; }();
                if (h->bxt_plan_ok && !no_tiles && h->bxt_nrt == rm / 64) {
                    BxtTileArgs ta;
                    ta.rowptr = ba.rowptr; ta.lidx = h->d_bxt_lidx; ta.vals = h->d_vals; ta.n_entries = h->n_entries;
                    ta.uptr = h->d_bxt_uptr + i * (h->bxt_nrt + 1); ta.ucols = h->d_bxt_ucols;
                    ta.gtiles = h->d_bxt_gtiles + i * h->bxt_nrt * 3; ta.ng = h->bxt_ng[(size_t)i];
                    ta.X = Xp; ta.C = C; ta.ld = ld; ta.ldc = ldc; ta.pX = pX; ta.pC = pC; ta.kst = h->d_kst;
                    ta.cm = cm; ta.rm = rm; ta.bsp = bsp; ta.ecap = h->bxt_ecap;
                    static const bool live_skip = [] { const char* e = getenv("GMRF_BXT_LIVE"); return e && atoi(e) != 0; }();
                    ta.skip_dead = live_skip ? 1 : 0;
                    const int chunks = W / 16, ng = ta.ng;
                    static const int nch_env = [] { const char* e = getenv("GMRF_BXT_NCH"); return e ? atoi(e) : 0; }();
                    {
                        const int64_t slots = 3 * (int64_t)std::max(h->cu_count, 1);
                        int best = 1; int64_t best_cost = INT64_MAX;
                        for (int c : {1, 2, 3, 4, 6, 8, 12, 16, 24, 48}) {
                            if (c > chunks) break;
                            const int64_t wgs = (int64_t)((chunks + c - 1) / c) * ng * nb;
                            const int64_t cost = ((wgs + slots - 1) / slots) * (c + 2);
                            if (cost < best_cost || (cost == best_cost && c < best)) { best = c; best_cost = cost; }
                        }
                        ta.nch = nch_env > 0 ? std::min(nch_env, chunks) : best;
                    }
                    const int ncg = (chunks + ta.nch - 1) / ta.nch;
                    ta.nprob = (int)nb;
                    ta.zdst = nullptr; ta.zcount = 0; ta.zpdst = 0; ta.zwgs = 0;
                    ta.srowptr = nullptr; ta.skeys = nullptr; ta.svals = nullptr;
                    if (scatter_in_bxt) {
                        ta.zdst = h->d_S; ta.zcount = (int64_t)bsp * bsp; ta.zpdst = bstride; ta.zwgs = 64;
                        ta.srowptr = h->d_dg_rowptr + i * (h->bsp + 1); ta.skeys = h->d_keys; ta.svals = h->d_vals;
                    } else if (zero_in_bxt && rm_s < bsp) {
                        ta.zdst = h->d_S + (int64_t)rm_s * ld; ta.zcount = (int64_t)(bsp - rm_s) * bsp; ta.zpdst = bstride;
                        ta.zwgs = (int)std::min<int64_t>(32, std::max<int64_t>(1, ta.zcount / 16384));
                    }
                    hipLaunchKernelGGL(spmm_bxt_tiles, dim3((unsigned)((ncg * ng + ta.zwgs) * (int)nb)), dim3(256), bxt_tile_lds_bytes(h->bxt_ecap),
                                       h->stream, ta);
                }
                else if (h->lo_row_max <= 8) hipLaunchKernelGGL(spmm_bxt<8>, grid, dim3(256), 0, h->stream, ba);
                else if (h->lo_row_max <= 16) hipLaunchKernelGGL(spmm_bxt<16>, grid, dim3(256), 0, h->stream, ba);
                else hipLaunchKernelGGL(spmm_bxt<32>, grid, dim3(256), 0, h->stream, ba);
                HIPCHK(hipGetLastError());
            } else {
                GCHK(gemm(h, false, false, rm, W, W, TRI_B_UPPER, 0, 1.0, h->d_B + cm, ld,
                          Xp + (int64_t)cm * ld + cm, ld, 0.0, C, ldc, bstride, pX, pC, 1, 0, 0, 0, nullptr, 0, 0, 0, -1.0,
                          h->d_kst, nullptr, nullptr));
            }
            GCHK(gemm(h, false, false, rm, rm, W, 0, 1, -1.0, C, ldc, C, ldc, scatter_in_bxt ? 1.0 : 0.0, h->d_S, ld, pC, pC,
                      bstride, 1, 0, 0, 0, nullptr, 0, 0, 0, 2.0 * 64.0 * 64.0 * h->g2_tile_k * (double)h->B,
                      h->d_kst, h->d_kst, nullptr));
        }
        if (h->diag_count[i] > 0 && !scatter_in_bxt) {
            hipLaunchKernelGGL(scatter_block, dim3((unsigned)((h->diag_count[i] + 255) / 256), nb), dim3(256), 0,
                               h->stream, h->d_keys, h->d_vals, h->diag_first[i], h->diag_count[i], h->d_S, ld,
                               h->n_entries, bstride, 1);
            HIPCHK(hipGetLastError());
        }
        if (i == h->tw_blk && h->tw_hj)
            GCHK(gemm(h, false, false, bsp, bsp, bsp, 0, 1, -1.0, h->tw_hj, ld, h->tw_hj, ld, 1.0, h->d_S, ld, 0, 0, 0));
        if (h->bsp > h->bs) {
            hipLaunchKernelGGL(pad_identity, dim3((unsigned)((h->bsp - h->bs + 255) / 256), nb), dim3(256), 0,
                               h->stream, h->d_S, ld, (int)h->bs, bsp, bstride);
            HIPCHK(hipGetLastError());
        }
        GCHK(potrf_block(h, h->d_S, L, X, h->d_T, (int)(i + 1)));
        if (i == h->tw_blk && h->tw_w)
            GCHK(gemm(h, false, true, bsp, bsp, bsp, 0, 0, 1.0, X, ld, h->tw_hj, ld, 0.0, h->tw_w, ld, 0, 0, 0));
        if (!h->keep_l) {
            hipLaunchKernelGGL(logdet_blocks, dim3(1, nb), dim3(256), 0, h->stream, L, bstride, ld, (int)h->bs,
                               h->d_logdet + i, stride_pL(h), h->N);
            HIPCHK(hipGetLastError());
        }
    }
    return GMRF_OK;
}

static gmrf_status ensure_full_inverse(gmrf_handle* h) {
    if (h->xsplit <= 0) return GMRF_OK;
    const int bsp = (int)h->bsp, p = h->xsplit, q = bsp - p;
    const int64_t ld = bsp, bstride = (int64_t)bsp * bsp, pX = stride_pX(h), pW = bstride;
    for (int64_t i = 0; i < h->N; ++i) {
        double* X = h->d_Linv + i * bstride;
        double* T = h->d_T + (int64_t)p * ld;
        GCHK(gemm(h, false, true, q, p, p, TRI_B_LOWER, 0, 1.0, X + (int64_t)p * ld, ld, X, ld, 0.0, T, ld, pX, pX, pW));
        GCHK(gemm(h, false, true, q, p, q, TRI_A_LOWER, 0, -1.0, X + (int64_t)p * ld + p, ld, T, ld, 0.0, X + (int64_t)p * ld, ld, pX, pW, pX));
    }
    h->xsplit = 0;
    return GMRF_OK;
}

static std::mutex g_capture_mu;

static gmrf_status run_factor(gmrf_handle* h, int64_t i0, int64_t i1) {
    if (h->eager || h->profiling) { h->stats.persist_route = 0; return factor_blocks_range(h, i0, i1); }
    if (!h->factor_graph || h->factor_graph_i0 != i0 || h->factor_graph_i1 != i1) {
        std::lock_guard<std::mutex> capture_lock(g_capture_mu);
        if (h->factor_graph) { (void)hipGraphExecDestroy(h->factor_graph); h->factor_graph = nullptr; }
        hipGraph_t graph = nullptr;
        HIPCHK(hipStreamBeginCapture(h->stream, hipStreamCaptureModeThreadLocal));
        h->capturing = true; h->fork_next = 0;
        h->stats.persist_route = 0;
        gmrf_status s = factor_blocks_range(h, i0, i1);
        h->capturing = false;
        h->factor_graph_route = h->stats.persist_route;
        hipError_t e = hipStreamEndCapture(h->stream, &graph);
        if (s != GMRF_OK) { if (graph) (void)hipGraphDestroy(graph); return s; }
        HIPCHK(e);
        HIPCHK(hipGraphInstantiate(&h->factor_graph, graph, nullptr, nullptr, 0));
        (void)hipGraphDestroy(graph);
        h->factor_graph_i0 = i0; h->factor_graph_i1 = i1;
    }
    h->xsplit = planned_xsplit(h);
    h->stats.persist_route = h->factor_graph_route;
    if (h->factor_graph_route) h->persist_launched = true;
    HIPCHK(hipGraphLaunch(h->factor_graph, h->stream));
    return GMRF_OK;
}

static gmrf_status persist_check_range(gmrf_handle* h, int64_t i0, int64_t i1, int* hinfo_out) {
    int hinfo2[2] = {0, 0};
    HIPCHK(hipMemcpyAsync(hinfo2, h->d_info, 2 * sizeof(int), hipMemcpyDeviceToHost, h->stream));
    HIPCHK(hipStreamSynchronize(h->stream));
    h->persist_launched = false;
    if (hinfo2[1] != 0) {
        persist_give_up(h);
        const int restore[4] = {h->info_checked, 0, 0, 0};
        HIPCHK(hipMemcpyAsync(h->d_info, restore, 4 * sizeof(int), hipMemcpyHostToDevice, h->stream));
        if (h->d_pflags) HIPCHK(hipMemsetAsync(h->d_pflags, 0, sizeof(unsigned) * (size_t)h->pflags_words, h->stream));
        h->stats.persist_route = 0;
        GCHK(factor_blocks_range(h, i0, i1));
        HIPCHK(hipMemcpyAsync(hinfo2, h->d_info, 2 * sizeof(int), hipMemcpyDeviceToHost, h->stream));
        HIPCHK(hipStreamSynchronize(h->stream));
        h->persist_launched = false;
    }
    h->info_checked = hinfo2[0];
    if (hinfo_out) *hinfo_out = hinfo2[0];
    return GMRF_OK;
}

static gmrf_status factor_finish(gmrf_handle* h, int32_t* info) {
    int hinfo = 0;
    GCHK(persist_check_range(h, 0, h->N, &hinfo));
    if (info) *info = hinfo;
    if (hinfo != 0) {
        h->factored = false;
        g_last_error = "matrix is not positive definite; failed block " + std::to_string((hinfo - 1) % h->N + 1) +
                       " of problem " + std::to_string((hinfo - 1) / h->N);
        if (info) *info = (hinfo - 1) % (int)h->N + 1;
        return GMRF_ERR_NOT_SPD;
    }
    h->factored = true;
    h->l_valid = h->keep_l;
    h->logdet_valid = !h->keep_l;
    return GMRF_OK;
}

static gmrf_status numeric_factor(gmrf_handle* h, const double* nzval, int32_t* info) {
    if (!h->analyzed) { g_last_error = "no sparsity pattern analysed"; return GMRF_ERR_NO_FACTOR; }
    GCHK(alloc_factor(h));
    if (h->c_dirty) {
        HIPCHK(hipMemsetAsync(h->d_C, 0, sizeof(double) * stride_pC(h) * h->B, h->stream));
        h->c_dirty = false;
    }
    persist_plan(h);
    HIPCHK(hipEventRecord(h->ev0, h->stream));
    GCHK(load_values(h, nzval));
    HIPCHK(hipMemsetAsync(h->d_info, 0, 4 * sizeof(int), h->stream));
    h->info_checked = 0; h->persist_launched = false;
    GCHK(run_factor(h, 0, h->N));
    HIPCHK(hipEventRecord(h->ev1, h->stream));
    gmrf_status s = factor_finish(h, info);
    float ms = 0.f;
    (void)hipEventElapsedTime(&ms, h->ev0, h->ev1);
    h->stats.factor_ms = ms;
    if (h->profiling) prof_collect(h);
    return s;
}

__global__ void gmrf_spin_kernel(unsigned long long ticks) {
    const unsigned long long t0 = __builtin_amdgcn_s_memrealtime();
    while (__builtin_amdgcn_s_memrealtime() - t0 < ticks) {}
}

static double spin_pair_ms(hipStream_t a, hipStream_t b, unsigned long long ticks) {
    (void)hipDeviceSynchronize();
    const auto t0 = std::chrono::steady_clock::now();
    hipLaunchKernelGGL(gmrf_spin_kernel, dim3(1), dim3(64), 0, a, ticks);
    if (b) hipLaunchKernelGGL(gmrf_spin_kernel, dim3(1), dim3(64), 0, b, ticks);
    (void)hipStreamSynchronize(a);
    if (b) (void)hipStreamSynchronize(b);
    return std::chrono::duration<double, std::milli>(std::chrono::steady_clock::now() - t0).count();
}

gmrf_status gmrf_streams_create(int32_t device, int32_t n, void** streams, int32_t* n_distinct) {
    if (n <= 0 || n > 32 || !streams) return bad_shape("gmrf_streams_create: 1 <= n <= 32 streams");
    HIPCHK(hipSetDevice(device));
    const int ncand = std::min(3 * n + 4, 48);
    std::vector<hipStream_t> cand((size_t)ncand, nullptr);
    for (int i = 0; i < ncand; ++i) {
        if (hipStreamCreateWithFlags(&cand[(size_t)i], hipStreamNonBlocking) != hipSuccess) {
            for (int j = 0; j < i; ++j) (void)hipStreamDestroy(cand[(size_t)j]);
            g_last_error = "hipStreamCreateWithFlags failed"; return GMRF_ERR_HIP;
        }
        hipLaunchKernelGGL(gmrf_spin_kernel, dim3(1), dim3(64), 0, cand[(size_t)i], 1ull);
    }
    HIPCHK(hipDeviceSynchronize());
    const unsigned long long ticks = 100000ull;
    double one = 1e30;
    for (int r = 0; r < 3; ++r) one = std::min(one, spin_pair_ms(cand[0], nullptr, ticks));
    std::vector<int> chosen;
    for (int i = 0; i < ncand && (int)chosen.size() < n; ++i) {
        bool ok = true;
        for (int c : chosen) {
            const double t = std::min(spin_pair_ms(cand[(size_t)c], cand[(size_t)i], ticks), spin_pair_ms(cand[(size_t)c], cand[(size_t)i], ticks));
            if (t > 1.5 * one) { ok = false; break; }
        }
        if (ok) chosen.push_back(i);
    }
    const int nd = (int)chosen.size();
    std::vector<char> used((size_t)ncand, 0);
    for (int c : chosen) used[(size_t)c] = 1;
    for (int i = 0; i < ncand && (int)chosen.size() < n; ++i)
        if (!used[(size_t)i]) { chosen.push_back(i); used[(size_t)i] = 1; }
    for (int k = 0; k < n; ++k) streams[k] = (void*)cand[(size_t)chosen[(size_t)k]];
// ... 299 lines not shown
int32_t gmrf_version(void) { return 100; }
const char* gmrf_last_error(void) { return g_last_error.c_str(); }

gmrf_status gmrf_bt_create(int32_t device, void* stream, gmrf_handle** out) {
    if (!out) return bad_shape("null out pointer");
    int count = 0;
    if (hipGetDeviceCount(&count) != hipSuccess || count <= 0 || device < 0 || device >= count) {
        (void)hipGetLastError();
        g_last_error = "no HIP device visible (libgmrf_hip needs an MI355X / gfx950 GPU)";
        return GMRF_ERR_NO_DEVICE;
    }
    HIPCHK(hipSetDevice(device));
    gmrf_handle* h = new gmrf_handle();
    memset(&h->stats, 0, sizeof(h->stats));
    h->device = device;
    if (stream) { h->stream = (hipStream_t)stream; h->own_stream = false; }
    else { HIPCHK(hipStreamCreateWithFlags(&h->stream, hipStreamNonBlocking)); h->own_stream = true; }
    HIPCHK(hipMalloc(&h->d_info, 4 * sizeof(int)));
    HIPCHK(hipMemsetAsync(h->d_info, 0, 4 * sizeof(int), h->stream));
    HIPCHK(hipStreamSynchronize(h->stream));
    HIPCHK(hipEventCreate(&h->ev0));
    HIPCHK(hipEventCreate(&h->ev1));
    HIPCHK(hipFuncSetAttribute((const void*)potrf_step<false>, hipFuncAttributeMaxDynamicSharedMemorySize, (int)POTRF_STEP_LDS));
    HIPCHK(hipFuncSetAttribute((const void*)potrf_diag128, hipFuncAttributeMaxDynamicSharedMemorySize, 160 * 1024));
    HIPCHK(hipFuncSetAttribute((const void*)potrf_persist<false>, hipFuncAttributeMaxDynamicSharedMemorySize, (int)POTRF_PERSIST_LDS));
    HIPCHK(hipDeviceGetAttribute(&h->cu_count, hipDeviceAttributeMultiprocessorCount, device));
    { const char* e = getenv("GMRF_PERSIST"); if (e && atoi(e) == 0) h->no_persist = true; }
    { const char* e = getenv("GMRF_SWEEP_PERSIST"); if (e && atoi(e) == 0) h->no_sweep_persist = true; }
    HIPCHK(hipFuncSetAttribute((const void*)potrf_diag128_slim, hipFuncAttributeMaxDynamicSharedMemorySize, 160 * 1024));
    HIPCHK(gemm_init());
    HIPCHK(gemm_dma_init());
    *out = h;
    return GMRF_OK;
}

gmrf_status gmrf_bt_destroy(gmrf_handle* h) {
    if (!h) return GMRF_OK;
    (void)hipSetDevice(h->device);
    tw_free(h);
    (void)hipStreamSynchronize(h->stream);
    persist_release(h);
    destroy_graphs(h);
    free_dev(h->d_keys); free_dev(h->d_vals); free_dev(h->d_src); free_dev(h->d_nz_stage);
    free_dev(h->d_lo_rowptr); free_dev(h->d_dg_rowptr); free_dev(h->d_kst); free_dev(h->d_mend);
    free_dev(h->d_bxt_uptr); free_dev(h->d_bxt_ucols); free_dev(h->d_bxt_lidx); free_dev(h->d_bxt_gtiles);
    if (!h->external_storage) { free_dev(h->d_L); free_dev(h->d_C); free_dev(h->d_Linv); }
    else if (!h->keep_l) free_dev(h->d_L);
    free_dev(h->d_S); free_dev(h->d_B); free_dev(h->d_T); free_dev(h->d_W);
    free_dev(h->d_sweep_flags); free_dev(h->d_Tsw); free_dev(h->d_P2); free_dev(h->d_Y2); free_dev(h->d_T2);
    if (h->h_sweep_abort) { (void)hipHostFree(h->h_sweep_abort); h->h_sweep_abort = nullptr; }
    free_dev(h->d_info); free_dev(h->d_logdet); free_dev(h->d_pflags); free_dev(h->d_kbx); free_dev(h->d_V);
    free_dev(h->d_P); free_dev(h->d_Y); free_dev(h->d_Tp);
    free_dev(h->d_stage); free_dev(h->d_mean); free_dev(h->d_acc);
    free_dev(h->d_sel_src); free_dev(h->d_sel_slot); free_dev(h->d_sig); free_dev(h->d_dv);
    for (auto e : h->ev_pool) (void)hipEventDestroy(e);
    if (h->ev0) (void)hipEventDestroy(h->ev0);
    if (h->ev1) (void)hipEventDestroy(h->ev1);
    for (auto e : h->fork_events) (void)hipEventDestroy(e);
    if (h->aux) (void)hipStreamDestroy(h->aux);
    if (h->own_stream) (void)hipStreamDestroy(h->stream);
    delete h;
    return GMRF_OK;
}

gmrf_status gmrf_bt_set_batch(gmrf_handle* h, int64_t batch) {
    if (!h || batch < 1 || batch > 4096) return bad_shape("batch must be in [1, 4096]");
    if (batch != 1) GCHK(tw_refuse(h, "gmrf_bt_set_batch (batch > 1)"));
    if (batch != h->B) {
        HIPCHK(hipSetDevice(h->device));
        HIPCHK(hipStreamSynchronize(h->stream));
        destroy_graphs(h);
        h->B = batch;
        h->sel = 0;
        h->factored = false;
        release_shape_buffers(h);
        if (h->n > 0) (void)set_shape(h, h->n, h->N);
    }
    return GMRF_OK;
}

gmrf_status gmrf_bt_select_problem(gmrf_handle* h, int64_t p) {
    if (!h || p < 0 || p >= h->B) return bad_shape("problem index out of range");
    h->sel = p;
    return GMRF_OK;
}

gmrf_status gmrf_bt_set_profiling(gmrf_handle* h, int32_t level) {
    if (!h) return bad_shape("null handle");
    h->profiling = level;
    if (h->tw)
        for (gmrf_handle* s : {h->tw->top, h->tw->bot}) if (s) GCHK(gmrf_bt_set_profiling(s, level));
    if (level > 0 && h->events.empty()) h->gemm_shapes.clear();
    for (int i = 0; i < GMRF_KERNEL_CLASSES; ++i) { h->stats.kernel_ms[i] = h->stats.kernel_work[i] = 0; h->stats.kernel_launches[i] = 0; }
    return GMRF_OK;
}

gmrf_status gmrf_bt_set_eager(gmrf_handle* h, int32_t eager) {
    if (!h) return bad_shape("null handle");
    if (((eager & 2) != 0) != h->split_step) { destroy_graphs(h); h->split_step = (eager & 2) != 0; }
    if (((eager & 4) != 0) != h->sweep_no_gemm) { destroy_graphs(h); h->sweep_no_gemm = (eager & 4) != 0; }
    if (((eager & 8) != 0) != h->dense_g1) { destroy_graphs(h); h->dense_g1 = (eager & 8) != 0; }
    if (((eager & 16) != 0) != h->fork_graph) { destroy_graphs(h); h->fork_graph = (eager & 16) != 0; }
    h->no_staircase = (eager & 32) != 0;
    if (((eager & 128) != 0) != h->doubling_x) { destroy_graphs(h); h->doubling_x = (eager & 128) != 0; }
    if (((eager & 256) != 0) != h->no_lookahead) { destroy_graphs(h); h->no_lookahead = (eager & 256) != 0; }
    if (((eager & 4096) != 0) != h->no_xsplit) { destroy_graphs(h); h->no_xsplit = (eager & 4096) != 0; }
    if (((eager & 8192) != 0) != h->no_persist) { destroy_graphs(h); h->no_persist = (eager & 8192) != 0; }
    if (((eager & 32768) != 0) != h->no_persist_panels) { destroy_graphs(h); h->no_persist_panels = (eager & 32768) != 0; }
    if (((eager & 65536) != 0) != h->no_sweep_persist) { destroy_graphs(h); h->no_sweep_persist = (eager & 65536) != 0; }
    if (((eager & 131072) != 0) != h->no_scatter_fold) { destroy_graphs(h); h->no_scatter_fold = (eager & 131072) != 0; }
    h->no_fused_posterior = (eager & 262144) != 0;
    h->eager = (eager & 1) != 0;
    h->eager_bits = eager;
    if (h->tw)
        for (gmrf_handle* s : {h->tw->top, h->tw->bot})
            if (s) {
                GCHK(gmrf_bt_set_eager(s, eager));
                if (h->tw->bot) s->no_sweep_persist = true;
            }
    return GMRF_OK;
}

gmrf_status gmrf_bt_synchronize(gmrf_handle* h) {
    if (!h) return bad_shape("null handle");
    HIPCHK(hipStreamSynchronize(h->stream));
    if (tw_on(h)) HIPCHK(hipStreamSynchronize(h->tw->bot->stream));
    return GMRF_OK;
}

gmrf_status gmrf_bt_stats(gmrf_handle* h, gmrf_stats* out) {
    if (!h || !out) return bad_shape("null pointer");
    if (tw_on(h)) {
        const gmrf_stats &a = h->tw->top->stats, &b = h->tw->bot->stats;
        *out = h->stats;
        out->persist_route = a.persist_route;
        out->persist_aborts = a.persist_aborts + b.persist_aborts;
        out->persist_cus = a.persist_cus + b.persist_cus;
        out->persist_refused = a.persist_refused | b.persist_refused;
        out->factor_bytes = a.factor_bytes + b.factor_bytes;
        return GMRF_OK;
    }
    h = tw_route(h);
    *out = h->stats;
    return GMRF_OK;
}

gmrf_status gmrf_bt_factor_csc(gmrf_handle* h, int64_t n, int64_t n_blocks, const int64_t* colptr,
                               const int64_t* rowval, const double* nzval, int32_t index_base,
                               int32_t* info) {
    if (!h) return bad_shape("null handle");
    HIPCHK(hipSetDevice(h->device));
    if (info) *info = 0;
    if (h->order == GMRF_ORDER_TWISTED) {
        GCHK(tw_analyze(h, n, n_blocks, colptr, rowval, index_base));
        return tw_numeric(h, nzval, info);
    }
    GCHK(analyze_csc(h, n, n_blocks, colptr, rowval, index_base));
    return numeric_factor(h, nzval, info);
}

gmrf_status gmrf_bt_factor_begin_csc(gmrf_handle* h, int64_t n, int64_t n_blocks, const int64_t* colptr,
                                     const int64_t* rowval, const double* nzval, int32_t index_base) {
    GCHK(tw_refuse(h, "gmrf_bt_factor_begin_csc"));
    if (!h) return bad_shape("null handle");
    HIPCHK(hipSetDevice(h->device));
    if (colptr) GCHK(analyze_csc(h, n, n_blocks, colptr, rowval, index_base));
    if (!h->analyzed) { g_last_error = "no sparsity pattern analysed"; return GMRF_ERR_NO_FACTOR; }
    GCHK(alloc_factor(h));
    if (h->c_dirty) {
        HIPCHK(hipMemsetAsync(h->d_C, 0, sizeof(double) * stride_pC(h) * h->B, h->stream));
        h->c_dirty = false;
    }
    persist_plan(h);
    GCHK(load_values(h, nzval));
    HIPCHK(hipMemsetAsync(h->d_info, 0, 4 * sizeof(int), h->stream));
    h->info_checked = 0; h->persist_launched = false; h->stats.persist_route = 0;
    h->factored = false;
    return GMRF_OK;
}

gmrf_status gmrf_bt_factor_step_async(gmrf_handle* h, int64_t i0, int64_t i1) {
    GCHK(tw_refuse(h, "gmrf_bt_factor_step_async"));
    if (!h) return bad_shape("null handle");
    if (i0 < 0 || i1 > h->N || i0 > i1) return bad_shape("bad block range");
    HIPCHK(hipSetDevice(h->device));
    GCHK(factor_blocks_range(h, i0, i1));
    if (h->persist_launched) GCHK(persist_check_range(h, i0, i1, nullptr));
    return GMRF_OK;
}

gmrf_status gmrf_bt_factor_end(gmrf_handle* h, int32_t* info) {
    GCHK(tw_refuse(h, "gmrf_bt_factor_end"));
    if (!h) return bad_shape("null handle");
    HIPCHK(hipSetDevice(h->device));
    gmrf_status s = factor_finish(h, info);
    if (h->profiling) prof_collect(h);
    return s;
}

gmrf_status gmrf_bt_refactor_values(gmrf_handle* h, const double* nzval, int32_t* info) {
    if (!h) return bad_shape("null handle");
    HIPCHK(hipSetDevice(h->device));
    if (info) *info = 0;
    if (h->order == GMRF_ORDER_TWISTED) return tw_numeric(h, nzval, info);
    return numeric_factor(h, nzval, info);
}

gmrf_status gmrf_bt_factor_blocks(gmrf_handle* h, int64_t n, int64_t n_blocks, const gmrf_sparse_block* diag,
                                  const gmrf_sparse_block* lower, int32_t index_base,
                                  int32_t compressed_by_column, int32_t* info) {
    GCHK(tw_refuse(h, "gmrf_bt_factor_blocks"));
    if (!h || !diag || (n_blocks > 1 && !lower)) return bad_shape("null pointer");
    HIPCHK(hipSetDevice(h->device));
    if (info) *info = 0;
    GCHK(set_shape(h, n, n_blocks));
    const int64_t bs = h->bs;
    std::vector<std::vector<HostEntry>> dg(n_blocks), lo(n_blocks);
    std::vector<double> vals;
    auto add_block = [&](const gmrf_sparse_block& b, std::vector<HostEntry>& dst, bool lower_tri_only) -> bool {
        for (int64_t o = 0; o < bs; ++o) {
            for (int64_t p = b.ptr[o] - index_base; p < b.ptr[o + 1] - index_base; ++p) {
                const int64_t in = b.idx[p] - index_base;
                if (in < 0 || in >= bs) return false;
                const int64_t r = compressed_by_column ? in : o, c = compressed_by_column ? o : in;
                if (lower_tri_only && r < c) continue;
                dst.push_back({((uint64_t)r << 32) | (uint64_t)c, (int64_t)vals.size()});
                vals.push_back(b.val[p]);
            }
        }
        return true;
// ... 75 lines not shown
    for (int64_t t = 0; t < nrt; ++t) out[3 + t] = h->kst[(size_t)t];
    out[3 + nrt] = h->factored ? h->xsplit : planned_xsplit(h);
    return GMRF_OK;
}

gmrf_status gmrf_bt_adopt_layout(gmrf_handle* h, int64_t n, int64_t n_blocks, const int64_t* layout, int64_t count) {
    GCHK(tw_refuse(h, "gmrf_bt_adopt_layout"));
    if (!h) return bad_shape("null handle");
    HIPCHK(hipSetDevice(h->device));
    GCHK(set_shape(h, n, n_blocks));
    h->analyzed = false;
    if (layout) {
        if (count < 3 || layout[2] < 1 || count < 3 + layout[2] || layout[1] != 64 * layout[2]) return bad_shape("bad layout record");
        std::vector<int64_t> first((size_t)layout[2]);
        for (int64_t t = 0; t < layout[2]; ++t) first[(size_t)t] = layout[0] + layout[3 + t];
        GCHK(set_layout(h, layout[0], layout[1], first));
        h->adopt_xsplit = 0;
        if (count >= 4 + layout[2]) {
            const int64_t xs = layout[3 + layout[2]];
            if (xs < 0 || xs >= h->bsp || xs % 64) return bad_shape("bad layout record (split)");
            h->adopt_xsplit = (int)xs;
        }
    } else {
        GCHK(set_layout_dense(h));
        h->adopt_xsplit = 0;
    }
    GCHK(alloc_factor(h));
    if (h->c_dirty) {
        HIPCHK(hipMemsetAsync(h->d_C, 0, sizeof(double) * stride_pC(h) * h->B, h->stream));
        h->c_dirty = false;
    }
    h->factored = false; h->l_valid = false; h->logdet_valid = false;
    h->got_block.assign((size_t)h->N, 0);
    HIPCHK(hipStreamSynchronize(h->stream));
    return GMRF_OK;
}

gmrf_status gmrf_bt_adopt_shape(gmrf_handle* h, int64_t n, int64_t n_blocks) {
    GCHK(tw_refuse(h, "gmrf_bt_adopt_shape"));
    return gmrf_bt_adopt_layout(h, n, n_blocks, nullptr, 0);
}

gmrf_status gmrf_bt_adopt_commit(gmrf_handle* h, int32_t l_blocks_valid) {
    GCHK(tw_refuse(h, "gmrf_bt_adopt_commit"));
    if (!h || !h->d_Linv) return bad_shape("no factor storage");
    HIPCHK(hipSetDevice(h->device));
    int seen = 0;
    HIPCHK(hipMemcpyAsync(&seen, h->d_info + 2, sizeof(int), hipMemcpyDeviceToHost, h->stream));
    HIPCHK(hipStreamSynchronize(h->stream));
    if (seen != 0) HIPCHK(hipMemsetAsync(h->d_info + 2, 0, sizeof(int), h->stream));
    if (seen < 0) { g_last_error = "the packed ranges of this factor carry different (or no) representation tags"; return GMRF_ERR_BAD_SHAPE; }
    const int xs = seen > 0 ? seen - 1 : h->adopt_xsplit;
    if (xs < 0 || xs >= h->bsp || xs % 64) { g_last_error = "bad representation tag in the packed image"; return GMRF_ERR_BAD_SHAPE; }
    h->factored = true;
    h->xsplit = xs;
    h->l_valid = l_blocks_valid != 0 && h->keep_l;
    bool all = !h->got_block.empty();
    for (char g : h->got_block) all = all && g;
    h->logdet_valid = all;
    h->got_block.assign((size_t)h->N, 0);
    persist_plan(h);
    return GMRF_OK;
}

gmrf_status gmrf_bt_factor_buffer(gmrf_handle* h, int32_t kind, void** dev_ptr, int64_t* bytes) {
    GCHK(tw_refuse(h, "gmrf_bt_factor_buffer"));
    if (!h || !dev_ptr || !bytes) return bad_shape("null pointer");
    if (!h->d_Linv) { g_last_error = "no factor storage"; return GMRF_ERR_NO_FACTOR; }
    const int64_t blk = blk_elems(h) * (int64_t)sizeof(double) * h->B;
    if (kind == GMRF_BLOCK_L) {
        if (!h->keep_l) { g_last_error = "L blocks are not kept (gmrf_bt_set_keep_l)"; return GMRF_ERR_NO_FACTOR; }
        *dev_ptr = h->d_L; *bytes = blk * h->N;
    }
    else if (kind == GMRF_BLOCK_C) { *dev_ptr = h->d_C; *bytes = stride_pC(h) * (int64_t)sizeof(double) * h->B; }
    else if (kind == GMRF_BLOCK_LINV) { *dev_ptr = h->d_Linv; *bytes = blk * h->N; }
    else return bad_shape("bad block kind");
    return GMRF_OK;
}

gmrf_status gmrf_bt_block_range(gmrf_handle* h, int32_t kind, int64_t i0, int64_t i1, int64_t* first_elem,
                                int64_t* n_elems, int64_t* problem_stride) {
    GCHK(tw_refuse(h, "gmrf_bt_block_range"));
    if (!h || !first_elem || !n_elems || !problem_stride) return bad_shape("null pointer");
    if (h->N <= 0 || i0 < 0 || i1 > h->N || i0 > i1) return bad_shape("bad block range");
    if (kind == GMRF_BLOCK_C) {
        const int64_t c0 = std::max<int64_t>(i0 - 1, 0), c1 = std::max<int64_t>(i1 - 1, 0);
        *first_elem = c0 * c_blk(h); *n_elems = (c1 - c0) * c_blk(h); *problem_stride = stride_pC(h);
    } else if (kind == GMRF_BLOCK_LINV || kind == GMRF_BLOCK_L) {
        if (kind == GMRF_BLOCK_L && !h->keep_l) { g_last_error = "L blocks are not kept"; return GMRF_ERR_NO_FACTOR; }
        *first_elem = i0 * blk_elems(h); *n_elems = (i1 - i0) * blk_elems(h);
        *problem_stride = kind == GMRF_BLOCK_L ? stride_pL(h) : stride_pX(h);
    } else return bad_shape("bad block kind");
    return GMRF_OK;
}

static void packed_counts(const gmrf_handle* h, int64_t i0, int64_t i1, int64_t* x_elems, int64_t* c_elems, int64_t* ld_elems,
                          int64_t* c0_out) {
    const int64_t nt = h->bsp / 64, ntri = nt * (nt + 1) / 2;
    const int64_t c0 = std::max<int64_t>(i0 - 1, 0), c1 = std::max<int64_t>(i1 - 1, 0);
    *x_elems = (i1 - i0) * ntri * 4096;
    *c_elems = (c1 - c0) * c_blk(h);
    *ld_elems = 2 + ((i1 - i0) + 1) / 2 * 2;
    if (c0_out) *c0_out = c0;
}

gmrf_status gmrf_bt_packed_size(gmrf_handle* h, int64_t i0, int64_t i1, int64_t* elems_per_problem) {
    GCHK(tw_refuse(h, "gmrf_bt_packed_size"));
// ... 133 lines not shown
    for (int64_t i = 0; i < h->N; ++i) GCHK(gmrf_bt_get_block(h, GMRF_BLOCK_LINV, i, out + i * be, h->bs));
    return GMRF_OK;
}

gmrf_status gmrf_bt_import_factor(gmrf_handle* h, const void* buf, int64_t bytes) {
    GCHK(tw_refuse(h, "gmrf_bt_import_factor"));
    if (!h || !buf) return bad_shape("null pointer");
    if (is_device_ptr(buf)) return bad_shape("import buffer must be host memory");
    if (bytes < 64) return bad_shape("import buffer too small");
    const int64_t* hdr = (const int64_t*)buf;
    if (hdr[0] != EXPORT_MAGIC || hdr[1] != 1 || hdr[5] != 1) return bad_shape("not a factor image");
    const int64_t n = hdr[2], N = hdr[3], bs = hdr[4];
    if (N <= 0 || bs <= 0 || n != N * bs) return bad_shape("bad shape in factor image");
    if (bytes < 64 + (int64_t)sizeof(double) * bs * bs * (3 * N - 1)) return bad_shape("factor image truncated");
    HIPCHK(hipSetDevice(h->device));
    if (!h->keep_l) return bad_shape("import needs the L blocks kept (gmrf_bt_set_keep_l(h, 1))");
    if ((h->n != n || h->N != N) && h->B != 1) return bad_shape("a batched handle imports into an existing shape only");
    const bool relayout = (h->n != n || h->N != N || h->cmin != 0 || h->rmax != 64 * next_pow2((bs + 63) / 64) || !h->d_Linv);
    if (relayout && h->B != 1 && h->factored) return bad_shape("a batched handle imports only into a dense-layout factor");
    GCHK(set_shape(h, n, N));
    h->analyzed = false;
    if (relayout) {
        GCHK(set_layout_dense(h));
        GCHK(alloc_factor(h));
        if (h->c_dirty) {
            HIPCHK(hipMemsetAsync(h->d_C, 0, sizeof(double) * stride_pC(h) * h->B, h->stream));
            h->c_dirty = false;
        }
    } else {
        std::vector<int64_t> z((size_t)(h->bsp / 64), 0);
        bool dense_ks = true;
        for (int v : h->kst) if (v != 0) dense_ks = false;
        if (!dense_ks) GCHK(set_layout(h, 0, h->bsp, z));
        h->c_dirty = false;
    }
    const int64_t bsp = h->bsp, be = bs * bs;
    std::vector<double> tmp((size_t)bsp * bsp);
    auto put = [&](const double* src, double* dst, bool unit_pad) -> gmrf_status {
        std::fill(tmp.begin(), tmp.end(), 0.0);
        for (int64_t r = 0; r < bs; ++r)
            for (int64_t c = 0; c < bs; ++c) tmp[(size_t)r * bsp + c] = src[c * bs + r];
        if (unit_pad)
            for (int64_t r = bs; r < bsp; ++r) tmp[(size_t)r * bsp + r] = 1.0;
        HIPCHK(hipMemcpyAsync(dst, tmp.data(), tmp.size() * sizeof(double), hipMemcpyHostToDevice, h->stream));
        HIPCHK(hipStreamSynchronize(h->stream));
        return GMRF_OK;
    };
    const double* in = (const double*)((const char*)buf + 64);
    for (int64_t i = 0; i < N; ++i) GCHK(put(in + i * be, h->d_L + h->sel * stride_pL(h) + i * blk_elems(h), true));
    in += N * be;
    for (int64_t i = 0; i + 1 < N; ++i) GCHK(put(in + i * be, h->d_C + h->sel * stride_pC(h) + i * c_blk(h), false));
    in += (N - 1) * be;
    for (int64_t i = 0; i < N; ++i) GCHK(put(in + i * be, h->d_Linv + h->sel * stride_pX(h) + i * blk_elems(h), true));
    h->factored = true; h->l_valid = true;
    persist_plan(h);
    h->xsplit = 0;
    return GMRF_OK;
}

struct NcclUid { char b[128]; };
struct RcclApi {
    void* lib = nullptr;
    int (*GetUniqueId)(NcclUid*) = nullptr;
    int (*CommInitRank)(void**, int, NcclUid, int) = nullptr;
    int (*CommDestroy)(void*) = nullptr;
    int (*Broadcast)(const void*, void*, size_t, int, int, void*, hipStream_t) = nullptr;
    int (*AllReduce)(const void*, void*, size_t, int, int, void*, hipStream_t) = nullptr;
    int (*AllGather)(const void*, void*, size_t, int, void*, hipStream_t) = nullptr;
    int (*GroupStart)() = nullptr;
    int (*GroupEnd)() = nullptr;
    const char* (*GetErrorString)(int) = nullptr;
};
static RcclApi g_rccl;
static std::mutex g_rccl_mu;

static gmrf_status rccl_load() {
    std::lock_guard<std::mutex> lock(g_rccl_mu);
    if (g_rccl.lib) return GMRF_OK;
    const char* env = getenv("GMRF_RCCL_PATH");
    const char* names[] = {env, "librccl.so.1", "librccl.so", "/opt/rocm/lib/librccl.so.1", "/opt/rocm/lib/librccl.so"};
    void* lib = nullptr;
    for (int pass = 0; pass < 2 && !lib; ++pass)
        for (const char* nm : names) {
            if (!nm) continue;
            lib = dlopen(nm, RTLD_NOW | RTLD_LOCAL | (pass == 0 ? RTLD_NOLOAD : 0));
            if (lib) break;
        }
    if (!lib) { g_last_error = std::string("librccl not found (set GMRF_RCCL_PATH): ") + (dlerror() ? dlerror() : ""); return GMRF_ERR_RCCL; }
#define GMRF_RCCL_SYM(field, name)                                                           \
    g_rccl.field = reinterpret_cast<decltype(g_rccl.field)>(dlsym(lib, name));               \
    if (!g_rccl.field) { g_last_error = std::string("librccl lacks ") + name; return GMRF_ERR_RCCL; }
    GMRF_RCCL_SYM(GetUniqueId, "ncclGetUniqueId") GMRF_RCCL_SYM(CommInitRank, "ncclCommInitRank")
    GMRF_RCCL_SYM(CommDestroy, "ncclCommDestroy") GMRF_RCCL_SYM(Broadcast, "ncclBroadcast")
    GMRF_RCCL_SYM(AllReduce, "ncclAllReduce") GMRF_RCCL_SYM(AllGather, "ncclAllGather") GMRF_RCCL_SYM(GroupStart, "ncclGroupStart")
    GMRF_RCCL_SYM(GroupEnd, "ncclGroupEnd") GMRF_RCCL_SYM(GetErrorString, "ncclGetErrorString")
#undef GMRF_RCCL_SYM
    g_rccl.lib = lib;
    return GMRF_OK;
}

#define NCCLCHK(expr)                                                                       \
    do {                                                                                    \
        int _r = (expr);                                                                    \
        if (_r != 0) {                                                                      \
            g_last_error = std::string(#expr) + ": " + g_rccl.GetErrorString(_r);           \
            return GMRF_ERR_RCCL;                                                           \
        }                                                                                   \
// ... 309 lines not shown
        free_dev(h->d_P2); free_dev(h->d_Y2); free_dev(h->d_T2);
        h->d_P2 = h->d_Y2 = h->d_T2 = nullptr; h->p2_elems = 0;
        HIPCHK(hipMalloc(&h->d_P2, sizeof(double) * (size_t)elems));
        HIPCHK(hipMalloc(&h->d_Y2, sizeof(double) * (size_t)elems));
        HIPCHK(hipMalloc(&h->d_T2, sizeof(double) * (size_t)elems));
        h->p2_elems = elems;
    }
    GCHK(ensure_aux(h));
    h->fork_next = 0;
    hipEvent_t ev_fork = nullptr, ev_join = nullptr;
    GCHK(fork_event(h, &ev_fork)); GCHK(fork_event(h, &ev_join));
    h->sweep_persist_launched = true;
    h->stats.sweep_persist = 1;
    h->stats.sweep_persist_launches += 3;
    HIPCHK(hipEventRecord(h->ev0, h->stream));
    HIPCHK(hipEventRecord(ev_fork, h->stream));
    HIPCHK(hipStreamWaitEvent(h->aux, ev_fork, 0));
    {
        const int64_t total = (int64_t)kp * h->n_pad;
        hipLaunchKernelGGL(fill_normals_panel, dim3((unsigned)((total + 255) / 256), 1), dim3(256), 0, h->aux, h->d_P2, h->n_pad,
                           (int)h->bs, (int)h->bsp, (int)k, kp, seed, first_id, k, nullptr, (int64_t)0);
        HIPCHK(hipGetLastError());
        GCHK(launch_sweep_persist(h, true, kp, h->d_P2, h->d_Y2, h->aux, h->d_T2));
        HIPCHK(hipEventRecord(ev_join, h->aux));
    }
    GCHK(launch_pack(h, b, h->n, 1, 1));
    GCHK(launch_sweep_persist(h, false, 1, h->d_P, h->d_Y));
    GCHK(launch_sweep_persist(h, true, 1, h->d_Y, h->d_P));
    GCHK(launch_unpack(h, h->d_P, mean, h->n, 1, nullptr));
    HIPCHK(hipStreamWaitEvent(h->stream, ev_join, 0));
    GCHK(launch_unpack(h, h->d_Y2, samples, ld, (int)k, mean));
    HIPCHK(hipEventRecord(h->ev1, h->stream));
    HIPCHK(hipStreamSynchronize(h->stream));
    return GMRF_OK;
}

static bool posterior_fused_ok(gmrf_handle* h, int64_t k, bool dev_all) {
    if (tw_on(h) || h->B <= 1 || !dev_all || h->no_fused_posterior || h->sweep_no_gemm || k <= 0 || k > KP_CHUNK) return false;
    const int kp = pad_k(k);
    if (kp % 64 != 0 || (int64_t)h->B * (h->bsp / 64) * (kp / 64) < 128) return false;
    if ((int64_t)(kp + 1) * h->n_pad * 8 >= ((int64_t)1 << 32)) return false;
    if (ensure_panels(h, kp + 1) != GMRF_OK) return false;
    h->tail_probe = true; h->tail_refused = false;
    const gmrf_status st = sweep_launches(h, true, kp, h->d_P, h->d_Y, true);
    h->tail_probe = false;
    return st == GMRF_OK && !h->tail_refused;
}

static gmrf_status posterior_fused(gmrf_handle* h, const double* b, uint64_t seed, int64_t first_id, int64_t k, double* mean,
                                   double* samples, int64_t ld) {
    const int kp = pad_k(k);
    GCHK(ensure_panels(h, kp + 1));
    HIPCHK(hipEventRecord(h->ev0, h->stream));
    GCHK(launch_pack(h, b, h->n, 1, 1));
    GCHK(run_sweeps(h, GMRF_SOLVE_FORWARD, 1));
    {
        const int64_t total = (int64_t)(kp + 1) * h->n_pad;
        hipLaunchKernelGGL(fill_normals_panel, dim3((unsigned)((total + 255) / 256), (unsigned)h->B), dim3(256), 0,
                           h->stream, h->d_P, h->n_pad, (int)h->bs, (int)h->bsp, (int)k, kp, seed, first_id, k, h->d_Y, h->n_pad);
        HIPCHK(hipGetLastError());
    }
    GCHK(run_sweeps(h, SWEEP_BACKWARD_TAIL, kp));
    {
        const int64_t total = h->n * (k + 1);
        hipLaunchKernelGGL(unpack_panel_mean, dim3((unsigned)((total + 255) / 256), (unsigned)h->B), dim3(256), 0, h->stream, h->d_Y,
                           h->n_pad, samples, ld, mean, (int)h->bs, (int)h->bsp, h->n, (int)k, kp);
        HIPCHK(hipGetLastError());
    }
    HIPCHK(hipEventRecord(h->ev1, h->stream));
    HIPCHK(hipStreamSynchronize(h->stream));
    if (h->profiling) prof_collect(h);
    return GMRF_OK;
}

gmrf_status gmrf_bt_posterior(gmrf_handle* h, const double* b, uint64_t seed, int64_t first_id, int64_t k, double* mean,
                              double* samples, int64_t ld) {
    h = tw_route(h);
    if (!h || !b || !mean || !samples) return bad_shape("null pointer");
    if (!h->factored) { g_last_error = "posterior before factor"; return GMRF_ERR_NO_FACTOR; }
    if (k <= 0 || ld < h->n) return bad_shape("bad k / ld");
    HIPCHK(hipSetDevice(h->device));
    const bool dev_all = is_device_ptr(b) && is_device_ptr(mean) && is_device_ptr(samples);
    const int64_t vec_bytes = h->n * h->B * (int64_t)sizeof(double), smp_bytes = cols_bytes(h->n, k * h->B, ld);
    bool beside = false, fused = false;
    GCHK(sweep_guarded(h, {{b, vec_bytes, mean, vec_bytes}, {b, vec_bytes, samples, smp_bytes}, {mean, vec_bytes, samples, smp_bytes}},
                       [&]() -> gmrf_status {
        beside = !tw_on(h) && h->B == 1 && k <= KP_CHUNK && k >= 2 && dev_all && !h->profiling && sweep_persist_ok(h, 1) &&
                 sweep_persist_ok(h, pad_k(k));
        if (beside) return posterior_beside(h, b, seed, first_id, k, mean, samples, ld);
        fused = !h->sweep_persist_hold && posterior_fused_ok(h, k, dev_all);
        return fused ? posterior_fused(h, b, seed, first_id, k, mean, samples, ld) : GMRF_OK;
    }, [&]() -> gmrf_status {
        if (h->aux) HIPCHK(hipStreamSynchronize(h->aux));
        return GMRF_OK;
    }));
    if (!beside && !fused) {
        GCHK(gmrf_bt_solve(h, b, mean, 1, h->n, h->n, GMRF_SOLVE_FULL));
        return gmrf_bt_sample(h, seed, first_id, k, mean, nullptr, samples, ld);
    }
    float ms = 0.f;
    (void)hipEventElapsedTime(&ms, h->ev0, h->ev1);
    h->stats.solve_ms = ms;
    h->stats.sample_ms = 0.0;
    return GMRF_OK;
}

gmrf_status gmrf_bt_normals(gmrf_handle* h, uint64_t seed, int64_t first_id, int64_t k, double* z, int64_t ld) {
    if (!h || !z) return bad_shape("null pointer");
    if (h->n <= 0) return bad_shape("no shape set");
    if (k <= 0 || ld < h->n) return bad_shape("bad k / ld");
    if (h->B > 1 && k > KP_CHUNK) return bad_shape("with a batch of problems k is limited to 128 per call");
    HIPCHK(hipSetDevice(h->device));
    const bool z_dev = is_device_ptr(z);
    for (int64_t c0 = 0; c0 < k; c0 += KP_CHUNK) {
        const int kc = (int)std::min<int64_t>(KP_CHUNK, k - c0);
        const int kp = pad_k(kc);
        GCHK(ensure_panels(h, kp));
        const int64_t total = (int64_t)kp * h->n_pad;
        hipLaunchKernelGGL(fill_normals_panel, dim3((unsigned)((total + 255) / 256), (unsigned)h->B), dim3(256), 0,
                           h->stream, h->d_P, h->n_pad, (int)h->bs, (int)h->bsp, kc, kp, seed, first_id + c0, k, nullptr, (int64_t)0);
        HIPCHK(hipGetLastError());
        GCHK(cols_out(h, h->d_P, kc, nullptr, z + c0 * ld, ld, z_dev));
        HIPCHK(hipStreamSynchronize(h->stream));
    }
    return GMRF_OK;
}

gmrf_status gmrf_bt_logdet(gmrf_handle* h, double* out) {
    h = tw_route(h);
    if (!h || !out) return bad_shape("null pointer");
    if (!h->factored) { g_last_error = "logdet before factor"; return GMRF_ERR_NO_FACTOR; }
    HIPCHK(hipSetDevice(h->device));
    if (tw_on(h)) return tw_logdet(h, out);
    if (h->keep_l && h->l_valid) {
        hipLaunchKernelGGL(logdet_blocks, dim3((unsigned)h->N, 1), dim3(256), 0, h->stream,
                           h->d_L + h->sel * stride_pL(h), blk_elems(h), h->bsp, (int)h->bs, h->d_logdet + h->sel * h->N,
                           (int64_t)0, (int64_t)0);
        HIPCHK(hipGetLastError());
    } else if (!h->logdet_valid) {
        g_last_error = "neither the L blocks nor the log-determinant parts of this factor are resident (adopted as raw buffers without L)";
        return GMRF_ERR_NO_FACTOR;
    }
    std::vector<double> part((size_t)h->N);
    HIPCHK(hipMemcpyAsync(part.data(), h->d_logdet + h->sel * h->N, sizeof(double) * h->N, hipMemcpyDeviceToHost, h->stream));
    HIPCHK(hipStreamSynchronize(h->stream));
    double s = 0.0;
    for (double v : part) s += v;
    *out = 2.0 * s;
    return GMRF_OK;
}

gmrf_status gmrf_csr_create(int32_t device, void* stream, int64_t n_rows, int64_t n_cols, const int64_t* rowptr,
                            const int64_t* colidx, const double* vals, int32_t index_base, int32_t values_f32,
                            gmrf_csr** out) {
    if (!out || !rowptr || !colidx || !vals || n_rows <= 0 || n_cols <= 0) return bad_shape("bad CSR arguments");
    int count = 0;
// ... 2067 lines not shown
    HIPCHK(hipMalloc(&dL, sizeof(double) * 4096));
    HIPCHK(hipMalloc(&dX, sizeof(double) * 4096));
    HIPCHK(hipMalloc(&dinfo, sizeof(int)));
    HIPCHK(hipMemset(dinfo, 0, sizeof(int)));
    HIPCHK(hipMemcpy(dS, tile64, sizeof(double) * 4096, hipMemcpyHostToDevice));
    auto kern = potrf_tile_kernel;
    const dim3 tpb(256);
    (void)hipFuncSetAttribute((const void*)kern, hipFuncAttributeMaxDynamicSharedMemorySize, (int)POTRF_TILE_LDS);
    unsigned long long* dstamps;
    HIPCHK(hipMalloc(&dstamps, 64 * sizeof(unsigned long long)));
    HIPCHK(hipMemset(dstamps, 0, 64 * sizeof(unsigned long long)));
    hipLaunchKernelGGL(kern, dim3(1), tpb, POTRF_TILE_LDS, nullptr, dS, dL, dX, dinfo, (unsigned long long*)nullptr);
    HIPCHK(hipDeviceSynchronize());
    {
        hipEvent_t e0, e1; HIPCHK(hipEventCreate(&e0)); HIPCHK(hipEventCreate(&e1));
        HIPCHK(hipEventRecord(e0, nullptr));
        for (int i = 0; i < 200; ++i)
            hipLaunchKernelGGL(kern, dim3(1), tpb, POTRF_TILE_LDS, nullptr, dS, dL, dX, dinfo, (unsigned long long*)nullptr);
        HIPCHK(hipEventRecord(e1, nullptr)); HIPCHK(hipEventSynchronize(e1));
        float ms = 0.f; HIPCHK(hipEventElapsedTime(&ms, e0, e1));
        g_tile_us = ms * 1e3 / 200.0;
        hipEventDestroy(e0); hipEventDestroy(e1);
    }
    hipLaunchKernelGGL(kern, dim3(1), tpb, POTRF_TILE_LDS, nullptr, dS, dL, dX, dinfo, dstamps);
    HIPCHK(hipDeviceSynchronize());
    HIPCHK(hipMemcpy(g_tile_stamps, dstamps, 64 * sizeof(unsigned long long), hipMemcpyDeviceToHost));
    hipFree(dstamps);
    HIPCHK(hipGetLastError());
    HIPCHK(hipDeviceSynchronize());
    HIPCHK(hipMemcpy(tile64, dL, sizeof(double) * 4096, hipMemcpyDeviceToHost));
    HIPCHK(hipMemcpy(inv64, dX, sizeof(double) * 4096, hipMemcpyDeviceToHost));
    int hi = 0;
    HIPCHK(hipMemcpy(&hi, dinfo, sizeof(int), hipMemcpyDeviceToHost));
    if (info) *info = hi;
    hipFree(dS); hipFree(dL); hipFree(dX); hipFree(dinfo);
    return GMRF_OK;
}

gmrf_status gmrf_test_tile_timing(double* out, int32_t n) {
    if (!out || n < 18) return bad_shape("need 18 outputs");
    out[0] = g_tile_us;
    for (int i = 0; i < 17; ++i) out[1 + i] = (double)(g_tile_stamps[i] - g_tile_stamps[15]);
    if (n >= 24) for (int i = 0; i < 3; ++i) out[18 + i] = (double)(g_tile_stamps[20 + i] - g_tile_stamps[15]);
    if (n >= 30) for (int i = 0; i < 6; ++i) out[24 + i] = (double)(g_tile_stamps[24 + i] - g_tile_stamps[24]);
    if (n >= 62) for (int i = 0; i < 8; ++i) out[54 + i] = g_tile_stamps[56 + i] ? (double)(g_tile_stamps[56 + i] - g_tile_stamps[15]) : -1.0;
    if (n >= 54) for (int i = 0; i < 24; ++i) out[30 + i] = g_tile_stamps[32 + i] ? (double)(g_tile_stamps[32 + i] - g_tile_stamps[15]) : -1.0;
    return GMRF_OK;
}

gmrf_status gmrf_test_persist_stamps(double* out, int32_t n) {
    if (!out || n < 1 || n > 128) return bad_shape("1 .. 128 outputs");
    for (int i = 0; i < n; ++i)
        out[i] = g_persist_stamps[i] ? (g_persist_stamps[i] < 64 ? (double)g_persist_stamps[i] : (double)(g_persist_stamps[i] - g_persist_stamps[0])) : -1.0;
    return GMRF_OK;
}

gmrf_status gmrf_test_persist_aborts(gmrf_handle* h, int32_t* n) {
    if (!h || !n) return bad_shape("null argument");
    *n = h->persist_aborts;
    return GMRF_OK;
}

gmrf_status gmrf_test_persist_budget(int32_t cus, int32_t n, const int32_t* demands, int32_t* granted) {
    if (n < 0 || (n > 0 && (!demands || !granted))) return bad_shape("null argument");
    std::map<const void*, int> claims;
    for (int i = 0; i < n; ++i) granted[i] = persist_budget_claim(claims, (const void*)(demands + i), demands[i], cus, 0) ? 1 : 0;
    return GMRF_OK;
}

gmrf_status gmrf_test_potrf_block(int32_t device, int64_t bs, double* S, double* Linv, int32_t* info) {
    if (bs % 64 || next_pow2(bs / 64) != bs / 64) return bad_shape("bs must be 64 * 2^p");
    gmrf_handle* h = nullptr;
    GCHK(gmrf_bt_create(device, nullptr, &h));
    h->N = 1; h->n = bs; h->bs = bs; h->bsp = bs; h->n_pad = bs; h->B = 1;
    gmrf_status s = set_layout_dense(h);
    if (s == GMRF_OK) s = alloc_factor(h);
    unsigned long long* dst = nullptr;
    if (s == GMRF_OK && hipMalloc(&dst, 128 * sizeof(unsigned long long)) == hipSuccess) {
        (void)hipMemset(dst, 0, 128 * sizeof(unsigned long long));
        h->dbg_stamps = dst;
    }
    if (s == GMRF_OK) {
        hipError_t e = hipMemcpyAsync(h->d_S, S, sizeof(double) * bs * bs, hipMemcpyHostToDevice, h->stream);
        persist_plan(h);
        if (e == hipSuccess) s = potrf_block(h, h->d_S, h->d_L, h->d_Linv, h->d_T, 1);
        if (s == GMRF_OK) {
            int hi = 0;
            (void)hipMemcpyAsync(&hi, h->d_info, sizeof(int), hipMemcpyDeviceToHost, h->stream);
            (void)hipMemcpyAsync(S, h->d_L, sizeof(double) * bs * bs, hipMemcpyDeviceToHost, h->stream);
            (void)hipMemcpyAsync(Linv, h->d_Linv, sizeof(double) * bs * bs, hipMemcpyDeviceToHost, h->stream);
            if (hipStreamSynchronize(h->stream) != hipSuccess) s = GMRF_ERR_HIP;
            if (info) *info = hi;
            if (dst) (void)hipMemcpy(g_tile_stamps + 24, dst, 6 * sizeof(unsigned long long), hipMemcpyDeviceToHost);
            if (dst) (void)hipMemcpy(g_persist_stamps, dst, 128 * sizeof(unsigned long long), hipMemcpyDeviceToHost);
        }
    }
    if (dst) (void)hipFree(dst);
    gmrf_bt_destroy(h);
    return s;
}

gmrf_status gmrf_test_mfma_f64_rate(int32_t device, double* tflops) {
    HIPCHK(hipSetDevice(device));
    double* d;
    HIPCHK(hipMalloc(&d, 64));
    hipEvent_t a, b;
// ... 132 lines not shown
```

### diffeqgmrfs.jl_amd/csrc/misc_kernels.hpp

```cpp
#pragma once
#include <hip/hip_runtime.h>
#include <stdint.h>

namespace gmrf {

__global__ void scatter_block(const uint64_t* __restrict__ keys, const double* __restrict__ vals,
                              int64_t first, int64_t count, double* __restrict__ dst, int64_t ld,
                              int64_t pvals, int64_t pdst, int add) {
    const int64_t i = (int64_t)blockIdx.x * blockDim.x + threadIdx.x;
    if (i >= count) return;
    const uint64_t key = keys[first + i];
    const int64_t r = (int64_t)(key >> 32), c = (int64_t)(key & 0xffffffffu);
    double* d = dst + (int64_t)blockIdx.y * pdst + r * ld + c;
    const double v = vals[(int64_t)blockIdx.y * pvals + first + i];
    *d = add ? *d + v : v;
}

__global__ void zero_rows(double* __restrict__ dst, int64_t count, int64_t pdst) {
    const int64_t i = ((int64_t)blockIdx.x * blockDim.x + threadIdx.x) * 2;
    if (i < count) *reinterpret_cast<v2d*>(dst + (int64_t)blockIdx.y * pdst + i) = (v2d){0.0, 0.0};
}

__global__ void pad_identity(double* __restrict__ dst, int64_t ld, int bs, int bsp, int64_t pdst) {
    const int i = bs + blockIdx.x * blockDim.x + threadIdx.x;
    if (i < bsp) dst[(int64_t)blockIdx.y * pdst + (int64_t)i * ld + i] = 1.0;
}

template <bool PACK>
__global__ __launch_bounds__(256) void linv_tiles_copy(double* __restrict__ X, int64_t ld, int64_t blk_stride,
                                                       int64_t pX, double* __restrict__ buf, int64_t pbuf, int ntri) {
    const int b = (int)blockIdx.x / ntri, tile = (int)blockIdx.x % ntri;
    int r = (int)((sqrtf(8.0f * (float)tile + 1.0f) - 1.0f) * 0.5f);
    while (r * (r + 1) / 2 > tile) --r;
    while ((r + 1) * (r + 2) / 2 <= tile) ++r;
    const int c = tile - r * (r + 1) / 2;
    double* x = X + (int64_t)blockIdx.y * pX + (int64_t)b * blk_stride + (int64_t)r * 64 * ld + (int64_t)c * 64;
    double* q = buf + (int64_t)blockIdx.y * pbuf + ((int64_t)b * ntri + tile) * 4096;
    const int t = threadIdx.x;
#pragma unroll
    for (int i = 0; i < 8; ++i) {
        const int e = (i * 256 + t) * 2, row = e >> 6, col = e & 63;
        if (PACK) *reinterpret_cast<v2d*>(q + e) = *reinterpret_cast<const v2d*>(x + (int64_t)row * ld + col);
        else *reinterpret_cast<v2d*>(x + (int64_t)row * ld + col) = *reinterpret_cast<const v2d*>(q + e);
    }
}

constexpr double PACK_TAG_MAGIC = 1196249670.0;
__global__ void pack_tag_write(double* __restrict__ buf, int64_t pbuf, double xsplit) {
    double* q = buf + (int64_t)threadIdx.x * pbuf;
    q[0] = xsplit; q[1] = PACK_TAG_MAGIC;
}
__global__ void pack_tag_read(const double* __restrict__ buf, int64_t pbuf, int nprob, int* __restrict__ seen) {
    int code = *seen;
    for (int p = 0; p < nprob; ++p) {
        const double* q = buf + (int64_t)p * pbuf;
        const double v = q[0];
        const int c = (q[1] == PACK_TAG_MAGIC && v >= 0.0 && v < 1.0e6 && v == (double)(int)v) ? (int)v + 1 : -1;
        code = (code == 0 || code == c) ? c : -1;
    }
    *seen = code;
}

__global__ void pack_panel(const double* __restrict__ src, int64_t ld, double* __restrict__ P,
                           int64_t n_pad, int bs, int bsp, int nblk, int k, int kp) {
    const int64_t idx = (int64_t)blockIdx.x * blockDim.x + threadIdx.x;
    const int64_t total = (int64_t)kp * n_pad;
    if (idx >= total) return;
    const int64_t r = idx / n_pad, j = idx % n_pad;
    const int64_t blk = j / bsp, off = j % bsp;
    double v = 0.0;
    if (r < k && off < bs) v = src[((int64_t)blockIdx.y * k + r) * ld + blk * bs + off];
    P[(int64_t)blockIdx.y * total + idx] = v;
}

__global__ void unpack_panel(const double* __restrict__ P, int64_t n_pad, double* __restrict__ dst,
                             int64_t ld, int bs, int bsp, int64_t n, int k, int kp,
                             const double* __restrict__ mean) {
    const int64_t idx = (int64_t)blockIdx.x * blockDim.x + threadIdx.x;
    if (idx >= n * (int64_t)k) return;
    const int64_t r = idx / n, j = idx % n;
    const int64_t blk = j / bs, off = j % bs;
    double v = P[(int64_t)blockIdx.y * kp * n_pad + r * n_pad + blk * bsp + off];
    if (mean) v += mean[(int64_t)blockIdx.y * n + j];
    dst[((int64_t)blockIdx.y * k + r) * ld + j] = v;
}

__device__ __host__ inline void philox4x32_10(uint32_t c[4], uint32_t k0, uint32_t k1) {
    for (int i = 0; i < 10; ++i) {
        const uint64_t p0 = (uint64_t)0xD2511F53u * c[0];
        const uint64_t p1 = (uint64_t)0xCD9E8D57u * c[2];
        const uint32_t n0 = (uint32_t)(p1 >> 32) ^ c[1] ^ k0;
        const uint32_t n1 = (uint32_t)p1;
        const uint32_t n2 = (uint32_t)(p0 >> 32) ^ c[3] ^ k1;
        const uint32_t n3 = (uint32_t)p0;
        c[0] = n0; c[1] = n1; c[2] = n2; c[3] = n3;
        k0 += 0x9E3779B9u; k1 += 0xBB67AE85u;
    }
}

__device__ __host__ inline double philox_normal(uint64_t seed, uint64_t dof, uint64_t sample) {
    uint32_t c[4] = {(uint32_t)dof, (uint32_t)(dof >> 32), (uint32_t)sample, (uint32_t)(sample >> 32)};
    philox4x32_10(c, (uint32_t)seed, (uint32_t)(seed >> 32));
    const uint64_t a = ((uint64_t)c[1] << 32) | c[0];
    const uint64_t b = ((uint64_t)c[3] << 32) | c[2];
    const double u1 = ((double)(a >> 11) + 0.5) * (1.0 / 9007199254740992.0);
    const double u2 = ((double)(b >> 11) + 0.5) * (1.0 / 9007199254740992.0);
    return sqrt(-2.0 * log(u1)) * cos(6.283185307179586476925 * u2);
}

__global__ void fill_normals_panel(double* __restrict__ P, int64_t n_pad, int bs, int bsp,
                                   int k, int kp, uint64_t seed, int64_t first_id, int64_t id_stride,
                                   const double* __restrict__ yrow, int64_t ystride) {
    const int64_t idx = (int64_t)blockIdx.x * blockDim.x + threadIdx.x;
// ... 961 lines not shown
```

### diffeqgmrfs.jl_amd/posterior.py

```python
from __future__ import annotations

from typing import List, Optional, Tuple

import numpy as np


def shard_range(total: int, world: int, rank: int) -> Tuple[int, int]:
    base, rem = divmod(total, world)
    first = rank * base + min(rank, rem)
    return first, base + (1 if rank < rem else 0)


def block_groups(n_blocks: int, group: int) -> List[Tuple[int, int]]:
    return [(i, min(n_blocks, i + group)) for i in range(0, n_blocks, group)]


class HipEngine:

    def __init__(self, pkg, workload, device_index: int = 0, batch: int = 1, values=None, rhs=None,
                 keep_l: bool = True, transport: str = "torch", comm=None):
        import torch
        self.torch = torch
        self.pkg = pkg
        self.w = workload
        self.batch = batch
        self.dev = torch.device("cuda", device_index)
        torch.cuda.set_device(self.dev)
        self.stream = torch.cuda.current_stream(self.dev)
        if self.stream.cuda_stream == 0:
            self.stream = torch.cuda.Stream(self.dev)
            torch.cuda.set_stream(self.stream)
        self.F = pkg.TridiagonalCholeskyFactor(device=device_index, stream=self.stream.cuda_stream, batch=batch)
        if not keep_l:
            self.F.set_keep_l(False)
        self.keep_l = keep_l
        self.transport, self.comm = transport, comm
        if transport == "cabi" and comm is None:
            raise ValueError('transport "cabi" needs an api.Comm')
        if values is None:
            values = np.tile(np.ascontiguousarray(workload.Q.data), (batch, 1))
        if rhs is None:
            rhs = np.tile(np.ascontiguousarray(workload.rhs), (batch, 1))
        self.values_host = np.ascontiguousarray(values, dtype=np.float64).reshape(batch, -1)
        self.nz = torch.from_numpy(self.values_host).to(self.dev)
        self.rhs = torch.from_numpy(np.ascontiguousarray(rhs, dtype=np.float64).reshape(batch, 1, -1)).to(self.dev)
        self._stage = {}
        self.bytes_moved = 0
        self._pending = []

    def prepare(self, is_root: bool, shared_storage: bool, dist=None):
        if not shared_storage:
            self.F.factor(self.w.Q, self.w.n_blocks, values=self.values_host)
            return
        if is_root:
            self.F.factor(self.w.Q, self.w.n_blocks, values=self.values_host)
            layout = self.F.get_layout()
        else:
            layout = None
        if self.transport == "cabi":
            cnt = np.array([0 if layout is None else layout.size], dtype=np.int64)
            self.comm.bcast_host(cnt, 0)
            if layout is None:
                layout = np.zeros(int(cnt[0]), dtype=np.int64)
            self.comm.bcast_host(layout, 0)
        else:
            box = [layout]
            dist.broadcast_object_list(box, src=0)
            layout = np.asarray(box[0], dtype=np.int64)
        if not is_root:
            self.F.adopt_layout(self.w.n, self.w.n_blocks, layout)

    def factor(self):
        self.F.refactor(self.nz)

    def factor_range_async(self, i0: int, i1: int, first: bool):
        if first:
            self.F.factor_begin_values(self.nz)
        self.F.factor_step_async(i0, i1)

    def factor_end(self):
        self.F.factor_end()

    def adopt_commit(self):
        self.F.adopt_commit(False)

    def _staging(self, i0: int, i1: int):
        key = (i0, i1)
        if key not in self._stage:
            t = self.torch
            self._stage[key] = t.empty((self.batch, self.F.packed_size(i0, i1)), dtype=t.float64, device=self.dev)
        return self._stage[key]

    def share_range(self, dist, i0: int, i1: int, is_root: bool = True):
        if self.transport == "cabi":
            self.comm.bcast_blocks_async(self.F, i0, i1, root=0, with_l=False)
            return
        buf = self._staging(i0, i1)
        if is_root:
# ... 200 lines not shown
```

### include/gmrf_hip.h

```cpp
#ifndef GMRF_HIP_H
#define GMRF_HIP_H

#include <stdint.h>

#ifdef __cplusplus
extern "C" {
#endif

typedef int32_t gmrf_status;

enum {
    GMRF_OK = 0,
    GMRF_ERR_NOT_SPD = -1,
    GMRF_ERR_BAD_SHAPE = -2,
    GMRF_ERR_BAND = -3,
    GMRF_ERR_HIP = -4,
    GMRF_ERR_NO_FACTOR = -5,
    GMRF_ERR_NO_DEVICE = -6,
    GMRF_ERR_ALLOC = -7,
    GMRF_ERR_RCCL = -8
};

enum { GMRF_SOLVE_FULL = 0, GMRF_SOLVE_FORWARD = 1, GMRF_SOLVE_BACKWARD = 2 };
enum { GMRF_VAR_EXACT = 0, GMRF_VAR_RBMC = 1, GMRF_VAR_MC = 2 };
// ... 9 lines not shown
    const int64_t* idx;
    const double* val;
} gmrf_sparse_block;

typedef struct {
    double factor_ms;
    double solve_ms;
    double sample_ms;
    double factor_flops;
    double sweep_bytes;
    double sweep_ms;
    int64_t n, n_blocks, block_size, block_size_padded;
    int64_t factor_bytes;
#define GMRF_KERNEL_CLASSES 24
    double kernel_ms[GMRF_KERNEL_CLASSES];
    double kernel_work[GMRF_KERNEL_CLASSES];
    int64_t kernel_launches[GMRF_KERNEL_CLASSES];
    double sweep_bytes_streamed;
    int32_t persist_route;
    int32_t persist_aborts;
    int32_t persist_cus;
    int32_t persist_refused;
    int32_t sweep_persist;
    int32_t sweep_persist_launches;
} gmrf_stats;


gmrf_status gmrf_bt_create(int32_t device, void* stream, gmrf_handle** out);
gmrf_status gmrf_bt_destroy(gmrf_handle* h);
const char* gmrf_last_error(void);
int32_t gmrf_version(void);

gmrf_status gmrf_bt_factor_csc(gmrf_handle* h, int64_t n, int64_t n_blocks,
                               const int64_t* colptr, const int64_t* rowval,
                               const double* nzval, int32_t index_base, int32_t* info);

gmrf_status gmrf_bt_factor_blocks(gmrf_handle* h, int64_t n, int64_t n_blocks,
                                  const gmrf_sparse_block* diag,
                                  const gmrf_sparse_block* lower,
                                  int32_t index_base, int32_t compressed_by_column,
                                  int32_t* info);

gmrf_status gmrf_bt_refactor_values(gmrf_handle* h, const double* nzval, int32_t* info);

gmrf_status gmrf_bt_solve(gmrf_handle* h, const double* b, double* y, int64_t k,
                          int64_t ldb, int64_t ldy, int32_t mode);

gmrf_status gmrf_bt_sample(gmrf_handle* h, uint64_t seed, int64_t first_id, int64_t k,
                           const double* mean, const double* z, double* out, int64_t ld);

gmrf_status gmrf_bt_posterior(gmrf_handle* h, const double* b, uint64_t seed, int64_t first_id, int64_t k,
                              double* mean, double* samples, int64_t ld);

gmrf_status gmrf_bt_normals(gmrf_handle* h, uint64_t seed, int64_t first_id, int64_t k,
                            double* z, int64_t ld);

gmrf_status gmrf_bt_marginal_var(gmrf_handle* h, int32_t method, int64_t k, uint64_t seed,
                                 const gmrf_csr* Q, double* var_out);

gmrf_status gmrf_bt_marginal_var_batch(gmrf_handle* h, int32_t method, int64_t k, uint64_t seed,
                                       const gmrf_csr* Q, const double* q_vals, double* var_out);

gmrf_status gmrf_bt_selinv(gmrf_handle* h, const gmrf_csr* S, double* vals_out);

gmrf_status gmrf_bt_trace_inv(gmrf_handle* h, const gmrf_csr* S, const double* dvals, int64_t m, double* out);

gmrf_status gmrf_bt_var_accumulate(gmrf_handle* h, int32_t method, int64_t first_id,
                                   int64_t k, uint64_t seed, const gmrf_csr* Q,
                                   double* acc);

gmrf_status gmrf_bt_logdet(gmrf_handle* h, double* out);

gmrf_status gmrf_bt_get_block(gmrf_handle* h, int32_t kind, int64_t i, double* out,
                              int64_t ld);

gmrf_status gmrf_bt_export_size(gmrf_handle* h, int64_t* bytes);
gmrf_status gmrf_bt_export_factor(gmrf_handle* h, void* host_buf, int64_t bytes);
gmrf_status gmrf_bt_import_factor(gmrf_handle* h, const void* host_buf, int64_t bytes);

gmrf_status gmrf_bt_factor_buffer(gmrf_handle* h, int32_t kind, void** dev_ptr,
                                  int64_t* bytes);
gmrf_status gmrf_bt_block_range(gmrf_handle* h, int32_t kind, int64_t i0, int64_t i1,
                                int64_t* first_elem, int64_t* n_elems, int64_t* problem_stride);
gmrf_status gmrf_bt_set_keep_l(gmrf_handle* h, int32_t keep);
gmrf_status gmrf_bt_get_layout(gmrf_handle* h, int64_t* out, int64_t cap, int64_t* count);

gmrf_status gmrf_bt_packed_size(gmrf_handle* h, int64_t i0, int64_t i1, int64_t* elems_per_problem);
gmrf_status gmrf_bt_pack_blocks_async(gmrf_handle* h, int64_t i0, int64_t i1, double* dev_buf);
gmrf_status gmrf_bt_unpack_blocks_async(gmrf_handle* h, int64_t i0, int64_t i1, const double* dev_buf);

gmrf_status gmrf_bt_storage_bytes(int64_t n, int64_t n_blocks, int64_t batch, int64_t* bytes_L,
                                  int64_t* bytes_C, int64_t* bytes_Linv);
gmrf_status gmrf_bt_set_storage(gmrf_handle* h, int64_t n, int64_t n_blocks, int64_t batch,
                                void* dev_L, void* dev_C, void* dev_Linv);

gmrf_status gmrf_bt_adopt_layout(gmrf_handle* h, int64_t n, int64_t n_blocks,
                                 const int64_t* layout, int64_t count);
gmrf_status gmrf_bt_adopt_shape(gmrf_handle* h, int64_t n, int64_t n_blocks);
gmrf_status gmrf_bt_adopt_commit(gmrf_handle* h, int32_t l_blocks_valid);

gmrf_status gmrf_comm_unique_id(void* id128);
gmrf_status gmrf_comm_create(int32_t device, int32_t rank, int32_t world, const void* id128,
                             gmrf_comm** out);
gmrf_status gmrf_comm_destroy(gmrf_comm* c);
gmrf_status gmrf_comm_bcast_host(gmrf_comm* c, void* host_buf, int64_t bytes, int32_t root);
gmrf_status gmrf_comm_allreduce_sum(gmrf_comm* c, gmrf_handle* stream_of, double* dev_buf,
// ... 46 lines not shown
gmrf_status gmrf_assemble_pattern(const gmrf_assembler* as, int64_t* nnz_out, int64_t* n_products,
                                  int64_t* colptr, int64_t* rowval, int32_t index_base);
gmrf_status gmrf_assemble_precision(gmrf_assembler* as, const double* q_nzval, const double* j_vals,
                                    double noise, double* out_nzval);
gmrf_status gmrf_assemble_rhs(gmrf_assembler* as, const double* base, const double* j_vals,
                              const double* x, const double* obs_diff, double noise, double* out);

typedef struct gmrf_darcy_p1 gmrf_darcy_p1;
gmrf_status gmrf_darcy_p1_create(int32_t device, void* stream, int64_t nx, int64_t ny, gmrf_darcy_p1** out);
gmrf_status gmrf_darcy_p2_create(int32_t device, void* stream, int64_t nx, int64_t ny, gmrf_darcy_p1** out);
gmrf_status gmrf_darcy_p1_destroy(gmrf_darcy_p1* d);
gmrf_status gmrf_darcy_p1_pattern(const gmrf_darcy_p1* d, int64_t* nnz_out, int64_t* rowptr, int64_t* colidx,
                                  int32_t index_base);
gmrf_status gmrf_darcy_p1_assemble(gmrf_darcy_p1* d, const double* coeff_table, int64_t ng, double beta,
                                   double* vals_out, double* f_out);

typedef struct gmrf_burgers_p1 gmrf_burgers_p1;
gmrf_status gmrf_burgers_p1_create(int32_t device, void* stream, int64_t ns, int64_t nt, double dt, double nu,
                                   gmrf_burgers_p1** out);
gmrf_status gmrf_burgers_p2_create(int32_t device, void* stream, int64_t ns, int64_t nt, double dt, double nu,
                                   gmrf_burgers_p1** out);
gmrf_status gmrf_burgers_p1_destroy(gmrf_burgers_p1* b);
gmrf_status gmrf_burgers_p1_pattern(const gmrf_burgers_p1* b, int64_t* nnz_out, int64_t* rowptr, int64_t* colidx,
                                    int32_t index_base);
gmrf_status gmrf_burgers_p1_tangent(gmrf_burgers_p1* b, const double* w, double* vals_out, double* f_out);

typedef struct gmrf_swe_p1 gmrf_swe_p1;
gmrf_status gmrf_shallow_water_p1_create(int32_t device, void* stream, int64_t nx, int64_t ny, gmrf_swe_p1** out);
gmrf_status gmrf_shallow_water_p1_destroy(gmrf_swe_p1* w);
gmrf_status gmrf_shallow_water_p1_pattern(const gmrf_swe_p1* w, int32_t which, int64_t* nnz_out, int64_t* rowptr, int64_t* colidx,
                                          int32_t index_base);
gmrf_status gmrf_shallow_water_p1_qpoints(const gmrf_swe_p1* w, double* xy);
gmrf_status gmrf_shallow_water_p1_assemble(gmrf_swe_p1* w, const double* H_q, double k, double f, double g, const uint8_t* prescribed,
                                           double* K_vals, double* M_lumped, double* S_vals);
gmrf_status gmrf_shallow_water_p1_operators(gmrf_swe_p1* w, const double* K_vals, const double* M_lumped, const double* S_vals,
                                            const uint8_t* prescribed, double kappa_matern, double tau, double dt, double* G_vals,
                                            double* J_vals, double* M_tilde, double* beta);

gmrf_status gmrf_test_gemm(int32_t device, int64_t M, int64_t N, int64_t K, int32_t transA,
                           int32_t transB, int32_t tri_flags, int32_t lower_only,
                           double alpha, const double* A, int64_t lda, const double* B,
                           int64_t ldb, double beta, double* C, int64_t ldc);
gmrf_status gmrf_test_gemm_rate(int32_t device, int64_t M, int64_t N, int64_t K, int32_t transB,
                                int32_t tri_flags, int32_t lower_only, int32_t batch,
                                int32_t big, int32_t reps, double* ms_per_launch);
gmrf_status gmrf_test_gemm_shapes(gmrf_handle* h, double* rows, int64_t cap_rows, int64_t* n_rows);
gmrf_status gmrf_test_potrf_tile(int32_t device, double* tile64 ,
                                 double* inv64, int32_t* info);
gmrf_status gmrf_test_tile_timing(double* out, int32_t n);
gmrf_status gmrf_test_potrf_block(int32_t device, int64_t bs, double* S ,
                                  double* Linv, int32_t* info);
gmrf_status gmrf_test_persist_stamps(double* out, int32_t n);
gmrf_status gmrf_test_persist_aborts(gmrf_handle* h, int32_t* n);
gmrf_status gmrf_test_persist_budget(int32_t cus, int32_t n, const int32_t* demands, int32_t* granted);
gmrf_status gmrf_test_mfma_f64_rate(int32_t device, double* tflops);
gmrf_status gmrf_test_clock_probe_start(int32_t device, int32_t n, int32_t sleeps, void** probe);
gmrf_status gmrf_test_clock_probe_finish(void* probe, double* ghz, double* t_ms);
gmrf_status gmrf_test_hbm_rate(int32_t device, int64_t bytes, double* gbps);
gmrf_status gmrf_test_microbench(int32_t device, double* out, int32_t n);
gmrf_status gmrf_test_symbolic_csc(int64_t n, int64_t n_blocks, const int64_t* colptr, const int64_t* rowval,
                                   int32_t index_base, int64_t* out8);

#ifdef __cplusplus
}
#endif
#endif
```

Before: 51390 solves/s.

## Fuse forward triangular solve into blocked Cholesky factorization via GEMM tail rows

```diff
diff --git a/diffeqgmrfs.jl_amd/_cabi.py b/diffeqgmrfs.jl_amd/_cabi.py
--- a/diffeqgmrfs.jl_amd/_cabi.py
+++ b/diffeqgmrfs.jl_amd/_cabi.py
@@ -17,7 +17,7 @@
 EXPORTS = [
     "gmrf_bt_create", "gmrf_bt_destroy", "gmrf_last_error", "gmrf_version",
     "gmrf_bt_factor_csc", "gmrf_bt_factor_blocks", "gmrf_bt_refactor_values",
-    "gmrf_bt_solve", "gmrf_bt_sample", "gmrf_bt_posterior", "gmrf_bt_normals", "gmrf_bt_marginal_var",
+    "gmrf_bt_solve", "gmrf_bt_sample", "gmrf_bt_posterior", "gmrf_bt_set_factor_rhs", "gmrf_bt_normals", "gmrf_bt_marginal_var",
     "gmrf_bt_var_accumulate", "gmrf_bt_logdet", "gmrf_bt_get_block", "gmrf_bt_factor_buffer",
     "gmrf_bt_adopt_shape", "gmrf_bt_adopt_commit", "gmrf_bt_adopt_layout", "gmrf_bt_get_layout", "gmrf_bt_block_range",
     "gmrf_bt_set_keep_l", "gmrf_bt_storage_bytes", "gmrf_bt_set_storage", "gmrf_bt_factor_begin_csc",
@@ -33,7 +33,7 @@
     "gmrf_shallow_water_p1_create", "gmrf_shallow_water_p1_destroy", "gmrf_shallow_water_p1_pattern", "gmrf_shallow_water_p1_qpoints",
     "gmrf_shallow_water_p1_assemble", "gmrf_shallow_water_p1_operators",
     "gmrf_assemble_create", "gmrf_assemble_destroy", "gmrf_assemble_pattern", "gmrf_assemble_precision", "gmrf_assemble_rhs",
-    "gmrf_test_gemm", "gmrf_test_gemm_rate", "gmrf_test_gemm_shapes", "gmrf_test_potrf_tile", "gmrf_test_potrf_block", "gmrf_test_tile_timing", "gmrf_test_persist_stamps", "gmrf_test_persist_aborts", "gmrf_test_persist_budget", "gmrf_test_clock_probe_start", "gmrf_test_clock_probe_finish",
+    "gmrf_test_gemm", "gmrf_test_gemm_rate", "gmrf_test_gemm_shapes", "gmrf_test_potrf_tile", "gmrf_test_potrf_block", "gmrf_test_tile_timing", "gmrf_test_persist_stamps", "gmrf_test_persist_aborts", "gmrf_test_factor_fwd", "gmrf_test_persist_budget", "gmrf_test_clock_probe_start", "gmrf_test_clock_probe_finish",
     "gmrf_test_mfma_f64_rate", "gmrf_test_hbm_rate", "gmrf_test_microbench", "gmrf_test_symbolic_csc",
 ]
 
@@ -94,6 +94,7 @@
         "gmrf_bt_solve": [vp, vp, vp, i64, i64, i64, i32],
         "gmrf_bt_sample": [vp, u64, i64, i64, vp, vp, vp, i64],
         "gmrf_bt_posterior": [vp, vp, u64, i64, i64, vp, vp, i64],
+        "gmrf_bt_set_factor_rhs": [vp, vp],
         "gmrf_bt_normals": [vp, u64, i64, i64, vp, i64],
         "gmrf_bt_marginal_var": [vp, i32, i64, u64, vp, vp],
         "gmrf_bt_var_accumulate": [vp, i32, i64, i64, u64, vp, vp],
@@ -175,6 +176,7 @@
         "gmrf_test_tile_timing": [vp, i32],
         "gmrf_test_persist_stamps": [vp, i32],
         "gmrf_test_persist_aborts": [vp, vp],
+        "gmrf_test_factor_fwd": [vp, vp, vp],
         "gmrf_test_persist_budget": [i32, i32, vp, vp],
         "gmrf_test_clock_probe_start": [i32, i32, i32, P(vp)],
         "gmrf_test_clock_probe_finish": [vp, vp, vp],
diff --git a/diffeqgmrfs.jl_amd/api.py b/diffeqgmrfs.jl_amd/api.py
--- a/diffeqgmrfs.jl_amd/api.py
+++ b/diffeqgmrfs.jl_amd/api.py
@@ -644,6 +644,16 @@
         _cabi.check(self._lib.gmrf_bt_posterior(self._h, _cabi.ptr(b), seed, first_id, k, _cabi.ptr(mean), _cabi.ptr(out), n))
         return mean, out
 
+    def set_factor_rhs(self, b):
+        if b is None:
+            self._factor_rhs = None
+            _cabi.check(self._lib.gmrf_bt_set_factor_rhs(self._h, None))
+            return
+        if not (_is_torch(b) and b.is_cuda and b.is_contiguous()) or (self.N and b.numel() != self.batch * self.N):
+            raise ValueError("set_factor_rhs(): a contiguous device tensor of batch x n values")
+        self._factor_rhs = b
+        _cabi.check(self._lib.gmrf_bt_set_factor_rhs(self._h, _cabi.ptr(b)))
+
     def marginal_var(self, method: str = "exact", k: int = 50, seed: int = 0x5EED, Q: Optional[CsrMatrix] = None,
                      q_values=None, out=None):
         m = {"exact": _cabi.VAR_EXACT, "rbmc": _cabi.VAR_RBMC, "mc": _cabi.VAR_MC}[method]
diff --git a/diffeqgmrfs.jl_amd/csrc/gemm_f64.hpp b/diffeqgmrfs.jl_amd/csrc/gemm_f64.hpp
--- a/diffeqgmrfs.jl_amd/csrc/gemm_f64.hpp
+++ b/diffeqgmrfs.jl_amd/csrc/gemm_f64.hpp
@@ -39,6 +39,11 @@
     const int* kb_m = nullptr;
     const int* kb_n = nullptr;
     const int* ke_n = nullptr;
+    const double* tA = nullptr;
+    double* tC = nullptr;
+    const double* tD = nullptr;
+    int64_t ptA = 0, ptC = 0, ptD = 0;
+    double tbeta = 0.0;
 };
 
 constexpr int GEMM_BM = 64;
diff --git a/diffeqgmrfs.jl_amd/csrc/gemm_f64_dma.hpp b/diffeqgmrfs.jl_amd/csrc/gemm_f64_dma.hpp
--- a/diffeqgmrfs.jl_amd/csrc/gemm_f64_dma.hpp
+++ b/diffeqgmrfs.jl_amd/csrc/gemm_f64_dma.hpp
@@ -60,10 +60,10 @@
     constexpr int A_ST = BM * BK, B_ST = BN * BK, T_ST = TAIL ? BK : 0, ST = A_ST + B_ST + T_ST;
     static_assert(NJ % 2 == 0 || !B_N, "the [k][n] image pairs neighbouring column tiles");
     static_assert(MI % 2 == 0 || !A_T, "the [k][m] image pairs neighbouring row tiles");
-    static_assert(!TAIL || (BM == 64 && BN == 64 && B_N && !A_T), "the tail row: 64 x 64 tiles, B stored [k][n]");
+    static_assert(!TAIL || (BM == 64 && BN == 64 && !A_T), "the tail row: 64 x 64 tiles");
     int bm, bn, z;
     gemm_dma_tile_order<BM, BN>(g, bm, bn, z);
-    const bool tail = TAIL && bm == g.M / BM - 1;
+    const bool tail = TAIL && (g.lower_only == 1 ? bm == bn : bm == g.M / BM - 1);
     const int m0 = bm * BM, n0 = bn * BN;
     if (g.lower_only == 2 && n0 > m0 + BM - 1) return;
     const int zi = z % g.nb1, zp = z / g.nb1;
@@ -115,7 +115,7 @@
             offb[i] = (uint32_t)(((int64_t)(n0 + row) * g.ldb + 2 * ch) * 8);
         }
     }
-    const double* arow = A + (int64_t)g.M * g.lda;
+    const double* arow = g.tC ? g.tA + (int64_t)zp * g.ptA : A + (int64_t)g.M * g.lda;
     auto issue = [&](int kt, int stage) {
         const int k0 = kb + kt * BK;
         const char* abase = reinterpret_cast<const char*>(A_T ? A + (int64_t)k0 * g.lda : A + k0);
@@ -214,8 +214,13 @@
             if constexpr (TAIL) {
                 if (tail) {
                     const v2d b0 = tkg ? b[1][0] : b[0][0], b1 = tkg ? b[1][1] : b[0][1];
-                    tacc.x = fma(ta.x, b0.x, tacc.x); tacc.x = fma(ta.y, b1.x, tacc.x);
-                    tacc.y = fma(ta.x, b0.y, tacc.y); tacc.y = fma(ta.y, b1.y, tacc.y);
+                    if (B_N) {
+                        tacc.x = fma(ta.x, b0.x, tacc.x); tacc.x = fma(ta.y, b1.x, tacc.x);
+                        tacc.y = fma(ta.x, b0.y, tacc.y); tacc.y = fma(ta.y, b1.y, tacc.y);
+                    } else {
+                        tacc.x = fma(ta.x, b0.x, tacc.x); tacc.x = fma(ta.y, b0.y, tacc.x);
+                        tacc.y = fma(ta.x, b1.x, tacc.y); tacc.y = fma(ta.y, b1.y, tacc.y);
+                    }
                 }
             }
             __builtin_amdgcn_sched_barrier(0);
@@ -273,15 +278,23 @@
     if constexpr (TAIL) {
         if (tail) {
             __syncthreads();
-            *reinterpret_cast<v2d*>(gsm + (tkg * 4 + lq) * BN + wn + 2 * li) = tacc;
+            if (B_N) *reinterpret_cast<v2d*>(gsm + (tkg * 4 + lq) * BN + wn + 2 * li) = tacc;
+            else { gsm[(tkg * 4 + lq) * BN + wn + li] = tacc.x; gsm[(tkg * 4 + lq) * BN + wn + 16 + li] = tacc.y; }
             __syncthreads();
             if (w == 0) {
                 double s = 0.0;
 #pragma unroll
                 for (int q = 0; q < 8; ++q) s += gsm[q * BN + lane];
                 double v = alpha * s;
-                if (beta != 0.0) v += beta * Dm[(int64_t)g.M * ldd + n0 + lane];
-                C[(int64_t)g.M * g.ldc + n0 + lane] = v;
+                if (g.tC) {
+                    double* tc = g.tC + (int64_t)zp * g.ptC;
+                    const double* td = g.tD ? g.tD + (int64_t)zp * g.ptD : tc;
+                    if (g.tbeta != 0.0) v += g.tbeta * td[n0 + lane];
+                    tc[n0 + lane] = v;
+                } else {
+                    if (beta != 0.0) v += beta * Dm[(int64_t)g.M * ldd + n0 + lane];
+                    C[(int64_t)g.M * g.ldc + n0 + lane] = v;
+                }
             }
         }
     }
@@ -338,23 +351,36 @@
 }
 
 inline bool gemm_tail_ok(bool a_t, bool b_n, const GemmArgs& g, int batch) {
-    if (a_t || !b_n || g.lower_only || gemm_uses_ll(g, batch) || gemm_dma_shape(false, g, batch) != 1) return false;
+    if (a_t || gemm_uses_ll(g, batch) || gemm_dma_shape(false, g, batch) != 1) return false;
+    if (g.lower_only && g.M != g.N) return false;
+    if (g.tC) {
+        return g.nb1 == 1 && g.tA && ((uintptr_t)g.tA & 15) == 0 && (g.ptA & 1) == 0;
+    }
+    if (!b_n || g.lower_only) return false;
     return (int64_t)(g.M + 1) * g.ldc * 8 < ((int64_t)1 << 32) && (!g.D || (int64_t)(g.M + 1) * g.ldd * 8 < ((int64_t)1 << 32));
 }
 inline bool gemm_try_dma_tail(hipStream_t st, bool a_t, bool b_n, const GemmArgs& g, int batch, hipEvent_t ev_start, hipEvent_t ev_stop,
                               hipError_t* err) {
     if (!gemm_tail_ok(a_t, b_n, g, batch)) return false;
+    const bool tri_grid = g.lower_only && g.M == g.N;
     GemmArgs gs = g;
-    gs.lower_only = 0;
-    const dim3 grid((unsigned)((int64_t)(g.N / 64) * (g.M / 64) * batch)), block(256);
+    gs.lower_only = tri_grid ? 1 : 0;
+    static const bool asc_off = [] { const char* e = getenv("GMRF_GEMM_G2_ORDER"); return e && atoi(e) == 0; }();
+    if (tri_grid && (g.kb_m || g.kb_n) && !asc_off) gs.tri |= DMA_ROWS_ASCENDING;
+    const int64_t nx = g.N / 64, ny = g.M / 64;
+    const dim3 grid((unsigned)((tri_grid ? ny * (ny + 1) / 2 : nx * ny) * batch)), block(256);
     const size_t lds = (size_t)gemm_dma_stages() * (64 + 64 + DMA_BK) * DMA_BK * sizeof(double);
+#define GMRF_DMA_TK(BNAT, ST)                                                                                              \
+    do {                                                                                                                   \
+        if (ev_start) hipExtLaunchKernelGGL((gemm_f64_dma<64, 64, BNAT, ST, false, true>), grid, block, lds, st, ev_start, ev_stop, 0, gs); \
+        else hipLaunchKernelGGL((gemm_f64_dma<64, 64, BNAT, ST, false, true>), grid, block, lds, st, gs);                \
+    } while (0)
     if (gemm_dma_stages() == 3) {
-        if (ev_start) hipExtLaunchKernelGGL((gemm_f64_dma<64, 64, true, 3, false, true>), grid, block, lds, st, ev_start, ev_stop, 0, gs);
-        else hipLaunchKernelGGL((gemm_f64_dma<64, 64, true, 3, false, true>), grid, block, lds, st, gs);
+        if (b_n) GMRF_DMA_TK(true, 3); else GMRF_DMA_TK(false, 3);
     } else {
-        if (ev_start) hipExtLaunchKernelGGL((gemm_f64_dma<64, 64, true, 2, false, true>), grid, block, lds, st, ev_start, ev_stop, 0, gs);
-        else hipLaunchKernelGGL((gemm_f64_dma<64, 64, true, 2, false, true>), grid, block, lds, st, gs);
-    }
+        if (b_n) GMRF_DMA_TK(true, 2); else GMRF_DMA_TK(false, 2);
+    }
+#undef GMRF_DMA_TK
     *err = hipGetLastError();
     return true;
 }
diff --git a/diffeqgmrfs.jl_amd/csrc/gmrf_hip.hip b/diffeqgmrfs.jl_amd/csrc/gmrf_hip.hip
--- a/diffeqgmrfs.jl_amd/csrc/gmrf_hip.hip
+++ b/diffeqgmrfs.jl_amd/csrc/gmrf_hip.hip
@@ -198,6 +198,14 @@
     bool no_fused_posterior = false;
     bool tail_probe = false;
     bool tail_refused = false;
+    const double* frhs = nullptr;
+    const double* fy_for = nullptr;
+    bool fwd_run = false;
+    bool no_factor_fwd = false;
+    double* d_ft = nullptr;
+    double* d_fy = nullptr;
+    int64_t fy_elems = 0;
+    const double* factor_graph_rhs = nullptr;
     unsigned long long* dbg_stamps = nullptr;
     bool fork_graph = false;
     bool no_staircase = false;
@@ -329,13 +337,25 @@
     h->events.clear();
 }
 
+struct GemmTail {
+    const double* A; int64_t pA;
+    double* C; int64_t pC;
+    const double* D; int64_t pD;
+    double beta;
+};
+
 static gmrf_status gemm(gmrf_handle* h, bool a_t, bool b_n, int M, int N, int K, int tri, int lower_only,
                         double alpha, const double* A, int64_t lda, const double* B, int64_t ldb,
                         double beta, double* C, int64_t ldc, int64_t pA, int64_t pB, int64_t pC,
                         int batch = 1, int64_t sA = 0, int64_t sB = 0, int64_t sC = 0, const double* D = nullptr,
                         int64_t ldd = 0, int64_t pD = 0, int pclass = 0, double pwork = -1.0,
-                        const int* kb_m = nullptr, const int* kb_n = nullptr, const int* ke_n = nullptr, bool tail = false) {
+                        const int* kb_m = nullptr, const int* kb_n = nullptr, const int* ke_n = nullptr, bool tail = false,
+                        const GemmTail* gt = nullptr) {
     GemmArgs g;
+    if (gt) {
+        g.tA = gt->A; g.ptA = gt->pA; g.tC = gt->C; g.ptC = gt->pC; g.tD = gt->D; g.ptD = gt->pD; g.tbeta = gt->beta;
+        tail = true;
+    }
     g.kb_m = kb_m; g.kb_n = kb_n; g.ke_n = ke_n;
     g.D = D; g.ldd = ldd; g.pD = pD;
     g.A = A; g.B = B; g.C = C;
@@ -350,7 +370,7 @@
     if (tail) {
         if (!gemm_tail_ok(a_t, b_n, g, batch * (int)h->B)) {
             h->tail_refused = true;
-            return h->tail_probe ? GMRF_OK : bad_shape("internal: a product of the fused sweep does not qualify for the tail-row GEMM");
+            return h->tail_probe ? GMRF_OK : bad_shape("internal: a product does not qualify for the tail-row GEMM");
         }
         if (h->tail_probe) return GMRF_OK;
         flops *= (M + 1.0) / M;
@@ -531,6 +551,7 @@
     free_dev(h->d_mean); h->d_mean = nullptr;
     free_dev(h->d_acc); h->d_acc = nullptr; h->acc_B = 0;
     free_dev(h->d_stage); h->d_stage = nullptr; h->stage_cap = 0;
+    free_dev(h->d_ft); free_dev(h->d_fy); h->d_ft = h->d_fy = nullptr; h->fy_elems = 0; h->fy_for = nullptr;
 }
 
 static gmrf_status set_shape(gmrf_handle* h, int64_t n, int64_t N) {
@@ -1001,7 +1022,7 @@
     return GMRF_OK;
 }
 
-static gmrf_status potrf_block(gmrf_handle* h, double* S, double* L, double* X, double* T, int blk_id) {
+static gmrf_status potrf_block(gmrf_handle* h, double* S, double* L, double* X, double* T, int blk_id, double* fy = nullptr) {
     const int bsp = (int)h->bsp;
     const int64_t ld = bsp;
     const int nt = bsp / 64;
@@ -1052,6 +1073,7 @@
         HIPCHK(hipGetLastError());
         return GMRF_OK;
     }
+    if (fy && (route != ROUTE_PANELS256 || overlap)) return bad_shape("internal: forward solve planned off the 256-column panel route");
     if (route == ROUTE_PANELS256 && !overlap) {
         StepArgs sa;
         sa.S = S; sa.L = L; sa.X = X; sa.ld = ld; sa.nt = nt; sa.cend = nt;
@@ -1089,14 +1111,29 @@
                           sa.pX, pW, sa.pX));
             }
             const int m3 = nt - j - 4;
-            if (m3 <= 0) continue;
+            const int64_t pT = bsp, pY = h->n_pad;
+            if (m3 <= 0) {
+                if (fy) {
+                    SweepArgs sw;
+                    sw.Mat = X + oa * ld + oa; sw.ld = ld; sw.Xin = h->d_ft + oa; sw.ldx = pT; sw.Bin = nullptr; sw.ldb = 0;
+                    sw.Out = fy + oa; sw.ldo = pY; sw.rows = 256; sw.kdim = 256; sw.sub = 0;
+                    sw.pMat = sa.pX; sw.pXin = pT; sw.pBin = 0; sw.pOut = pY;
+                    ProfScope ps(h, 3, 4.0 * 256.0 * 257.0 * nb);
+                    HIPCHK(launch_sweep(h->stream, false, true, 1, sw, (int)h->B));
+                }
+                continue;
+            }
+            const GemmTail tp{h->d_ft + oa, pT, fy + oa, pY, nullptr, 0, 0.0};
+            const GemmTail tu{fy + oa, pY, h->d_ft + oc, pT, nullptr, 0, 1.0};
             const bool in_slot = (j == 0 && h->xsplit == 256 && !h->keep_l);
             double* Lb = in_slot ? X + oc * ld + oa : L + oc * ld + oa;
             const int64_t pLb = in_slot ? sa.pX : sa.pL;
             GCHK(gemm(h, false, false, 64 * m3, 256, 256, TRI_B_UPPER, 0, 1.0, S + oc * ld + oa, ld, X + oa * ld + oa, ld, 0.0, Lb, ld,
-                      sa.pS, sa.pX, pLb, 1, 0, 0, 0, nullptr, 0, 0, 0, 2.0 * t3 * 10.0 * m3 * nb));
+                      sa.pS, sa.pX, pLb, 1, 0, 0, 0, nullptr, 0, 0, 0, 2.0 * t3 * 10.0 * m3 * nb, nullptr, nullptr, nullptr, false,
+                      fy ? &tp : nullptr));
             GCHK(gemm(h, false, false, m3 * 64, m3 * 64, 256, 0, 1, -1.0, Lb, ld, Lb, ld, 1.0, S + oc * ld + oc, ld, pLb, pLb, sa.pS,
-                      1, 0, 0, 0, nullptr, 0, 0, 0, 2.0 * t3 * 4.0 * (m3 * (m3 + 1) / 2) * nb));
+                      1, 0, 0, 0, nullptr, 0, 0, 0, 2.0 * t3 * 4.0 * (m3 * (m3 + 1) / 2) * nb, nullptr, nullptr, nullptr, false,
+                      fy ? &tu : nullptr));
         }
         const int p = h->xsplit;
         GCHK(doubling_levels(h, L, X, T, 256, bsp / 2, -1, p));
@@ -1215,6 +1252,11 @@
         double* L = l_block(h, i);
         double* X = h->d_Linv + i * bstride;
         const int rm_s = (i > 0) ? (int)h->rmax : 0;
+        if (h->fwd_run) {
+            hipLaunchKernelGGL(factor_rhs_block, dim3((unsigned)((bsp + 255) / 256), nb), dim3(256), 0, h->stream, h->frhs, h->n, (int)h->bs,
+                               bsp, i, h->d_ft);
+            HIPCHK(hipGetLastError());
+        }
         static const bool no_tiles_z = [] { const char* e = getenv("GMRF_BXT_TILES"); return e && atoi(e) == 0; }();
         const bool scatter_in_bxt = i > 0 && nb == 1 && h->sparse_b && !h->dense_g1 && h->bxt_plan_ok && !no_tiles_z && h->bxt_nrt == (int)h->rmax / 64
                                     && h->d_dg_rowptr && h->bsp == h->bs && !h->no_scatter_fold;
@@ -1298,9 +1340,10 @@
                           Xp + (int64_t)cm * ld + cm, ld, 0.0, C, ldc, bstride, pX, pC, 1, 0, 0, 0, nullptr, 0, 0, 0, -1.0,
                           h->d_kst, nullptr, nullptr));
             }
+            const GemmTail tg{h->d_fy + (i - 1) * bsp + cm, h->n_pad, h->d_ft, bsp, nullptr, 0, 1.0};
             GCHK(gemm(h, false, false, rm, rm, W, 0, 1, -1.0, C, ldc, C, ldc, scatter_in_bxt ? 1.0 : 0.0, h->d_S, ld, pC, pC,
                       bstride, 1, 0, 0, 0, nullptr, 0, 0, 0, 2.0 * 64.0 * 64.0 * h->g2_tile_k * (double)h->B,
-                      h->d_kst, h->d_kst, nullptr));
+                      h->d_kst, h->d_kst, nullptr, false, h->fwd_run ? &tg : nullptr));
         }
         if (h->diag_count[i] > 0 && !scatter_in_bxt) {
             hipLaunchKernelGGL(scatter_block, dim3((unsigned)((h->diag_count[i] + 255) / 256), nb), dim3(256), 0,
@@ -1315,7 +1358,7 @@
                                h->stream, h->d_S, ld, (int)h->bs, bsp, bstride);
             HIPCHK(hipGetLastError());
         }
-        GCHK(potrf_block(h, h->d_S, L, X, h->d_T, (int)(i + 1)));
+        GCHK(potrf_block(h, h->d_S, L, X, h->d_T, (int)(i + 1), h->fwd_run ? h->d_fy + i * bsp : nullptr));
         if (i == h->tw_blk && h->tw_w)
             GCHK(gemm(h, false, true, bsp, bsp, bsp, 0, 0, 1.0, X, ld, h->tw_hj, ld, 0.0, h->tw_w, ld, 0, 0, 0));
         if (!h->keep_l) {
@@ -1343,9 +1386,49 @@
 
 static std::mutex g_capture_mu;
 
+static gmrf_status factor_fwd_ok(gmrf_handle* h, bool* ok) {
+    *ok = false;
+    if (!h->frhs || h->no_factor_fwd || h->B <= 1 || tw_on(h) || h->tw_blk >= 0 || h->fork_graph || h->rmax <= 0) return GMRF_OK;
+    const int bsp = (int)h->bsp, nt = bsp / 64;
+    if (potrf_route(h) != ROUTE_PANELS256 || bsp % 256 != 0) return GMRF_OK;
+    const int64_t elems = h->B * h->n_pad + h->B * h->bsp;
+    if (!h->d_fy || h->fy_elems < elems) {
+        HIPCHK(hipStreamSynchronize(h->stream));
+        free_dev(h->d_ft); free_dev(h->d_fy); h->d_ft = h->d_fy = nullptr; h->fy_elems = 0; h->fy_for = nullptr;
+        HIPCHK(hipMalloc(&h->d_fy, sizeof(double) * (size_t)(h->B * h->n_pad)));
+        HIPCHK(hipMalloc(&h->d_ft, sizeof(double) * (size_t)(h->B * h->bsp)));
+        h->fy_elems = elems;
+    }
+    const int64_t ld = bsp, bstride = (int64_t)bsp * bsp, pX = stride_pX(h), pL = stride_pL(h), pC = stride_pC(h);
+    const int cm = (int)h->cmin, rm = (int)h->rmax, W = bsp - cm;
+    double* S = h->d_S; double* X = h->d_Linv; double* L = h->d_L;
+    h->tail_probe = true; h->tail_refused = false;
+    gmrf_status st = GMRF_OK;
+    if (h->N > 1) {
+        const GemmTail tg{h->d_fy + cm, h->n_pad, h->d_ft, bsp, nullptr, 0, 1.0};
+        st = gemm(h, false, false, rm, rm, W, 0, 1, -1.0, h->d_C, c_ld(h), h->d_C, c_ld(h), 0.0, S, ld, pC, pC, bstride, 1, 0, 0, 0,
+                  nullptr, 0, 0, 0, -1.0, h->d_kst, h->d_kst, nullptr, false, &tg);
+    }
+    for (int j = 0; j + 4 < nt && st == GMRF_OK; j += 4) {
+        const int64_t oa = (int64_t)j * 64, oc = oa + 256;
+        const int m3 = nt - j - 4;
+        const GemmTail tp{h->d_ft + oa, bsp, h->d_fy + oa, h->n_pad, nullptr, 0, 0.0};
+        const GemmTail tu{h->d_fy + oa, h->n_pad, h->d_ft + oc, bsp, nullptr, 0, 1.0};
+        st = gemm(h, false, false, 64 * m3, 256, 256, TRI_B_UPPER, 0, 1.0, S + oc * ld + oa, ld, X + oa * ld + oa, ld, 0.0, L + oc * ld + oa, ld,
+                  bstride, pX, pL, 1, 0, 0, 0, nullptr, 0, 0, 0, -1.0, nullptr, nullptr, nullptr, false, &tp);
+        if (st == GMRF_OK)
+            st = gemm(h, false, false, m3 * 64, m3 * 64, 256, 0, 1, -1.0, L + oc * ld + oa, ld, L + oc * ld + oa, ld, 1.0, S + oc * ld + oc, ld,
+                      pL, pL, bstride, 1, 0, 0, 0, nullptr, 0, 0, 0, -1.0, nullptr, nullptr, nullptr, false, &tu);
+    }
+    h->tail_probe = false;
+    *ok = st == GMRF_OK && !h->tail_refused;
+    return GMRF_OK;
+}
+
 static gmrf_status run_factor(gmrf_handle* h, int64_t i0, int64_t i1) {
     if (h->eager || h->profiling) { h->stats.persist_route = 0; return factor_blocks_range(h, i0, i1); }
-    if (!h->factor_graph || h->factor_graph_i0 != i0 || h->factor_graph_i1 != i1) {
+    const double* grhs = h->fwd_run ? h->frhs : nullptr;
+    if (!h->factor_graph || h->factor_graph_i0 != i0 || h->factor_graph_i1 != i1 || h->factor_graph_rhs != grhs) {
         std::lock_guard<std::mutex> capture_lock(g_capture_mu);
         if (h->factor_graph) { (void)hipGraphExecDestroy(h->factor_graph); h->factor_graph = nullptr; }
         hipGraph_t graph = nullptr;
@@ -1360,7 +1443,7 @@
         HIPCHK(e);
         HIPCHK(hipGraphInstantiate(&h->factor_graph, graph, nullptr, nullptr, 0));
         (void)hipGraphDestroy(graph);
-        h->factor_graph_i0 = i0; h->factor_graph_i1 = i1;
+        h->factor_graph_i0 = i0; h->factor_graph_i1 = i1; h->factor_graph_rhs = grhs;
     }
     h->xsplit = planned_xsplit(h);
     h->stats.persist_route = h->factor_graph_route;
@@ -1419,9 +1502,17 @@
     GCHK(load_values(h, nzval));
     HIPCHK(hipMemsetAsync(h->d_info, 0, 4 * sizeof(int), h->stream));
     h->info_checked = 0; h->persist_launched = false;
-    GCHK(run_factor(h, 0, h->N));
-    HIPCHK(hipEventRecord(h->ev1, h->stream));
-    gmrf_status s = factor_finish(h, info);
+    h->fy_for = nullptr;
+    bool fwd = false;
+    GCHK(factor_fwd_ok(h, &fwd));
+    h->fwd_run = fwd;
+    gmrf_status s = run_factor(h, 0, h->N);
+    if (s == GMRF_OK) {
+        (void)hipEventRecord(h->ev1, h->stream);
+        s = factor_finish(h, info);
+    }
+    h->fwd_run = false;
+    if (s == GMRF_OK && fwd) h->fy_for = h->frhs;
     float ms = 0.f;
     (void)hipEventElapsedTime(&ms, h->ev0, h->ev1);
     h->stats.factor_ms = ms;
@@ -1827,6 +1918,7 @@
     free_dev(h->d_info); free_dev(h->d_logdet); free_dev(h->d_pflags); free_dev(h->d_kbx); free_dev(h->d_V);
     free_dev(h->d_P); free_dev(h->d_Y); free_dev(h->d_Tp);
     free_dev(h->d_stage); free_dev(h->d_mean); free_dev(h->d_acc);
+    free_dev(h->d_ft); free_dev(h->d_fy);
     free_dev(h->d_sel_src); free_dev(h->d_sel_slot); free_dev(h->d_sig); free_dev(h->d_dv);
     for (auto e : h->ev_pool) (void)hipEventDestroy(e);
     if (h->ev0) (void)hipEventDestroy(h->ev0);
@@ -1885,6 +1977,8 @@
     if (((eager & 65536) != 0) != h->no_sweep_persist) { destroy_graphs(h); h->no_sweep_persist = (eager & 65536) != 0; }
     if (((eager & 131072) != 0) != h->no_scatter_fold) { destroy_graphs(h); h->no_scatter_fold = (eager & 131072) != 0; }
     h->no_fused_posterior = (eager & 262144) != 0;
+    h->no_factor_fwd = (eager & 524288) != 0;
+    if (eager != h->eager_bits) h->fy_for = nullptr;
     h->eager = (eager & 1) != 0;
     h->eager_bits = eager;
     if (h->tw)
@@ -1950,7 +2044,7 @@
     GCHK(load_values(h, nzval));
     HIPCHK(hipMemsetAsync(h->d_info, 0, 4 * sizeof(int), h->stream));
     h->info_checked = 0; h->persist_launched = false; h->stats.persist_route = 0;
-    h->factored = false;
+    h->factored = false; h->fy_for = nullptr;
     return GMRF_OK;
 }
 
@@ -2132,7 +2226,7 @@
     if (seen < 0) { g_last_error = "the packed ranges of this factor carry different (or no) representation tags"; return GMRF_ERR_BAD_SHAPE; }
     const int xs = seen > 0 ? seen - 1 : h->adopt_xsplit;
     if (xs < 0 || xs >= h->bsp || xs % 64) { g_last_error = "bad representation tag in the packed image"; return GMRF_ERR_BAD_SHAPE; }
-    h->factored = true;
+    h->factored = true; h->fy_for = nullptr;
     h->xsplit = xs;
     h->l_valid = l_blocks_valid != 0 && h->keep_l;
     bool all = !h->got_block.empty();
@@ -2372,7 +2466,7 @@
     for (int64_t i = 0; i + 1 < N; ++i) GCHK(put(in + i * be, h->d_C + h->sel * stride_pC(h) + i * c_blk(h), false));
     in += (N - 1) * be;
     for (int64_t i = 0; i < N; ++i) GCHK(put(in + i * be, h->d_Linv + h->sel * stride_pX(h) + i * blk_elems(h), true));
-    h->factored = true; h->l_valid = true;
+    h->factored = true; h->fy_for = nullptr; h->l_valid = true;
     persist_plan(h);
     h->xsplit = 0;
     return GMRF_OK;
@@ -2788,12 +2882,16 @@
     const int kp = pad_k(k);
     GCHK(ensure_panels(h, kp + 1));
     HIPCHK(hipEventRecord(h->ev0, h->stream));
-    GCHK(launch_pack(h, b, h->n, 1, 1));
-    GCHK(run_sweeps(h, GMRF_SOLVE_FORWARD, 1));
+    const bool have_y = h->fy_for && b == h->fy_for;
+    if (!have_y) {
+        GCHK(launch_pack(h, b, h->n, 1, 1));
+        GCHK(run_sweeps(h, GMRF_SOLVE_FORWARD, 1));
+    }
     {
         const int64_t total = (int64_t)(kp + 1) * h->n_pad;
         hipLaunchKernelGGL(fill_normals_panel, dim3((unsigned)((total + 255) / 256), (unsigned)h->B), dim3(256), 0,
-                           h->stream, h->d_P, h->n_pad, (int)h->bs, (int)h->bsp, (int)k, kp, seed, first_id, k, h->d_Y, h->n_pad);
+                           h->stream, h->d_P, h->n_pad, (int)h->bs, (int)h->bsp, (int)k, kp, seed, first_id, k,
+                           have_y ? h->d_fy : h->d_Y, h->n_pad);
         HIPCHK(hipGetLastError());
     }
     GCHK(run_sweeps(h, SWEEP_BACKWARD_TAIL, kp));
@@ -2838,6 +2936,14 @@
     (void)hipEventElapsedTime(&ms, h->ev0, h->ev1);
     h->stats.solve_ms = ms;
     h->stats.sample_ms = 0.0;
+    return GMRF_OK;
+}
+
+gmrf_status gmrf_bt_set_factor_rhs(gmrf_handle* h, const double* b) {
+    if (!h) return bad_shape("null handle");
+    if (b && !is_device_ptr(b)) return bad_shape("the factor's right-hand side must be device memory");
+    h->frhs = b;
+    h->fy_for = nullptr;
     return GMRF_OK;
 }
 
@@ -5011,6 +5117,17 @@
     if (!out || n < 1 || n > 128) return bad_shape("1 .. 128 outputs");
     for (int i = 0; i < n; ++i)
         out[i] = g_persist_stamps[i] ? (g_persist_stamps[i] < 64 ? (double)g_persist_stamps[i] : (double)(g_persist_stamps[i] - g_persist_stamps[0])) : -1.0;
+    return GMRF_OK;
+}
+
+gmrf_status gmrf_test_factor_fwd(gmrf_handle* h, int32_t* state, double* y_out) {
+    if (!h || !state) return bad_shape("null pointer");
+    HIPCHK(hipSetDevice(h->device));
+    *state = (h->fy_for && h->factored && h->fy_for == h->frhs) ? 1 : 0;
+    if (y_out && *state) {
+        GCHK(cols_out(h, h->d_fy, 1, nullptr, y_out, h->n, false));
+        HIPCHK(hipStreamSynchronize(h->stream));
+    }
     return GMRF_OK;
 }
 
diff --git a/diffeqgmrfs.jl_amd/csrc/misc_kernels.hpp b/diffeqgmrfs.jl_amd/csrc/misc_kernels.hpp
--- a/diffeqgmrfs.jl_amd/csrc/misc_kernels.hpp
+++ b/diffeqgmrfs.jl_amd/csrc/misc_kernels.hpp
@@ -59,6 +59,13 @@
         code = (code == 0 || code == c) ? c : -1;
     }
     *seen = code;
+}
+
+__global__ void factor_rhs_block(const double* __restrict__ b, int64_t n, int bs, int bsp, int64_t blk, double* __restrict__ t) {
+    const int r = blockIdx.x * blockDim.x + threadIdx.x;
+    if (r >= bsp) return;
+    const int64_t p = blockIdx.y;
+    t[p * bsp + r] = (r < bs) ? b[p * n + blk * bs + r] : 0.0;
 }
 
 __global__ void pack_panel(const double* __restrict__ src, int64_t ld, double* __restrict__ P,
diff --git a/diffeqgmrfs.jl_amd/posterior.py b/diffeqgmrfs.jl_amd/posterior.py
--- a/diffeqgmrfs.jl_amd/posterior.py
+++ b/diffeqgmrfs.jl_amd/posterior.py
@@ -44,6 +44,8 @@
         self.values_host = np.ascontiguousarray(values, dtype=np.float64).reshape(batch, -1)
         self.nz = torch.from_numpy(self.values_host).to(self.dev)
         self.rhs = torch.from_numpy(np.ascontiguousarray(rhs, dtype=np.float64).reshape(batch, 1, -1)).to(self.dev)
+        if batch > 1:
+            self.F.set_factor_rhs(self.rhs)
         self._stage = {}
         self.bytes_moved = 0
         self._pending = []
diff --git a/include/gmrf_hip.h b/include/gmrf_hip.h
--- a/include/gmrf_hip.h
+++ b/include/gmrf_hip.h
@@ -85,6 +85,8 @@
 gmrf_status gmrf_bt_posterior(gmrf_handle* h, const double* b, uint64_t seed, int64_t first_id, int64_t k,
                               double* mean, double* samples, int64_t ld);
 
+gmrf_status gmrf_bt_set_factor_rhs(gmrf_handle* h, const double* b);
+
 gmrf_status gmrf_bt_normals(gmrf_handle* h, uint64_t seed, int64_t first_id, int64_t k,
                             double* z, int64_t ld);
 
@@ -237,6 +239,7 @@
                                   double* Linv, int32_t* info);
 gmrf_status gmrf_test_persist_stamps(double* out, int32_t n);
 gmrf_status gmrf_test_persist_aborts(gmrf_handle* h, int32_t* n);
+gmrf_status gmrf_test_factor_fwd(gmrf_handle* h, int32_t* state, double* y_out);
 gmrf_status gmrf_test_persist_budget(int32_t cus, int32_t n, const int32_t* demands, int32_t* granted);
 gmrf_status gmrf_test_mfma_f64_rate(int32_t device, double* tflops);
 gmrf_status gmrf_test_clock_probe_start(int32_t device, int32_t n, int32_t sleeps, void** probe);
```

Measured after the change: 53450 solves/s (median of 6 runs). +4.0%, better.
